# wustl-cig/FLAIR

Hardware: AMD Instinct MI355X
Metric: restored frames/sec at 256x256, 16-frame clip, 250-step DDIM (higher is better)
Workload: dtype bf16

## Files before the change

### flair_amd/csrc/api.hip

```cpp
#include <stdarg.h>
#include <stdio.h>

#include "common.h"

static thread_local char g_err[512] = "";

void flair_set_error(const char* fmt, ...) {
    va_list ap;
    va_start(ap, fmt);
    vsnprintf(g_err, sizeof(g_err), fmt, ap);
    va_end(ap);
}

extern "C" const char* flair_last_error(void) { return g_err; }
extern "C" int flair_abi_version(void) { return 11; }

#include <dlfcn.h>

typedef int (*flair_nccl_bcast_fn)(const void*, void*, size_t, int, int, void*, hipStream_t);

extern "C" int flair_bcast_weights(void* blob, size_t bytes, int root, void* rccl_comm, hipStream_t stream) {
    FLAIR_CHECK(blob && bytes > 0 && rccl_comm && root >= 0, "flair_bcast_weights: bad argument (blob, bytes, root, communicator)");
    static flair_nccl_bcast_fn fn = nullptr;
    if (!fn) {
        void* h = nullptr;
        for (const char* name : {"librccl.so", "librccl.so.1"}) {
            h = dlopen(name, RTLD_NOW | RTLD_NOLOAD);
            if (!h) h = dlopen(name, RTLD_NOW | RTLD_GLOBAL);
            if (h) break;
        }
        FLAIR_CHECK(h, "flair_bcast_weights: librccl.so not found (%s)", dlerror());
        fn = reinterpret_cast<flair_nccl_bcast_fn>(dlsym(h, "ncclBroadcast"));
        FLAIR_CHECK(fn, "flair_bcast_weights: ncclBroadcast not found in librccl");
    }
    const size_t chunk = (size_t)512 << 20;
    for (size_t off = 0; off < bytes; off += chunk) {
        const size_t n = bytes - off < chunk ? bytes - off : chunk;
        char* p = reinterpret_cast<char*>(blob) + off;
        const int rc = fn(p, p, n,  1, root, rccl_comm, stream);
        if (rc != 0) {
            flair_set_error("flair_bcast_weights: ncclBroadcast returned %d", rc);
            return FLAIR_ERR_HIP;
        }
    }
    return FLAIR_OK;
}

namespace {
typedef __attribute__((ext_vector_type(8))) __bf16 probe_bf16x8;
typedef __attribute__((ext_vector_type(16))) float probe_f32x16;

__global__ __launch_bounds__(256) void probe_matrix_kernel(float* sink, int iters) {
    probe_f32x16 acc[4];
    for (int i = 0; i < 4; ++i)
        for (int r = 0; r < 16; ++r) acc[i][r] = 0.f;
    probe_bf16x8 a, b;
    for (int e = 0; e < 8; ++e) {
        a[e] = (__bf16)(0.001f * (float)((threadIdx.x + e) & 255));
        b[e] = (__bf16)(0.002f * (float)((threadIdx.x + 2 * e) & 255));
    }
    for (int it = 0; it < iters; ++it) {
#pragma unroll
        for (int u = 0; u < 4; ++u)
#pragma unroll
            for (int i = 0; i < 4; ++i) acc[i] = __builtin_amdgcn_mfma_f32_32x32x16_bf16(a, b, acc[i], 0, 0, 0);
    }
    float s = 0.f;
    for (int i = 0; i < 4; ++i)
        for (int r = 0; r < 16; ++r) s += acc[i][r];
    if (s == 12345.678f) sink[0] = s;
}

__global__ __launch_bounds__(256) void probe_stream_kernel(const uint4* __restrict__ src, uint4* __restrict__ dst, size_t n, int mode) {
    unsigned sum = 0;
    for (size_t i = blockIdx.x * (size_t)blockDim.x + threadIdx.x; i < n; i += (size_t)gridDim.x * blockDim.x) {
        if (mode == 1) {
            dst[i] = make_uint4((unsigned)i, 1u, 2u, 3u);
        } else {
            const uint4 v = src[i];
            if (mode == 2) dst[i] = v;
            else sum ^= v.x ^ v.y ^ v.z ^ v.w;
        }
    }
    if (mode == 0 && sum == 0x12345679u) dst[0] = make_uint4(sum, 0u, 0u, 0u);
}
}

extern "C" int flair_probe_matrix_rate(int iters, int workgroups_per_cu, float* sink, double* flop_out, hipStream_t stream) {
    FLAIR_CHECK(iters > 0 && workgroups_per_cu >= 1 && workgroups_per_cu <= 8 && sink, "flair_probe_matrix_rate: bad argument");
    const int grid = flair_cu_count() * workgroups_per_cu;
    hipLaunchKernelGGL(probe_matrix_kernel, dim3(grid), dim3(256), 0, stream, sink, iters);
    FLAIR_LAUNCH_CHECK();
    if (flop_out) *flop_out = (double)grid * 4  * iters * 16  * (2.0 * 32 * 32 * 16);
    return FLAIR_OK;
}

extern "C" int flair_probe_stream_rate(const void* src, void* dst, size_t bytes, int mode, hipStream_t stream) {
    FLAIR_CHECK(dst && (mode == 1 || src) && bytes >= 16 && mode >= 0 && mode <= 2, "flair_probe_stream_rate: bad argument (mode 0 read, 1 write, 2 copy)");
    FLAIR_CHECK((reinterpret_cast<uintptr_t>(dst) & 15) == 0 && (reinterpret_cast<uintptr_t>(src) & 15) == 0, "flair_probe_stream_rate: 16-byte aligned buffers");
    hipLaunchKernelGGL(probe_stream_kernel, dim3(flair_cu_count() * 8), dim3(256), 0, stream, reinterpret_cast<const uint4*>(src),
                       reinterpret_cast<uint4*>(dst), bytes / 16, mode);
    FLAIR_LAUNCH_CHECK();
    return FLAIR_OK;
}
```

### flair_amd/csrc/conv.hip

```cpp
#include <type_traits>

#include "common.h"

namespace {

struct ConvArgs {
    const void* x[4];
    int segC[4];
    int segLd[4];
    int nseg;
    const void* w;
    const float* bias;
    const void* res0;
    const void* res1;
    int res0Ld, res1Ld;
    void* y;
    int yLd;
    int T, H, W;
    int KT, KH, KW;
    int Cout, CinTot;
    int act;
    float outScale;
    long P;
    int nPixTiles, nCoTiles;
    int tFast;
    unsigned segBytes[4];
    unsigned wBytes;
    float* part;
    int splitK;
    const float* fbias;
    int fbiasLd;
    int stride;
    int tapShift;
    int reflect;
    float actParam;
    int actPeriod;
    int Hin, Win;
    int esz;
};

template <typename E> struct Mma;

template <> struct Mma<bf16_t> {
    static constexpr int BKE = 32;
    static __device__ __forceinline__ int chunk(int i, int half) { return 2 * i + half; }
    static __device__ __forceinline__ void run(const uint4 (&a)[2], const uint4 (&b)[2], f32x16& acc) {
        acc = __builtin_amdgcn_mfma_f32_32x32x16_bf16(__builtin_bit_cast(bf16x8, a[0]),
                                                      __builtin_bit_cast(bf16x8, b[0]), acc, 0, 0, 0);
        acc = __builtin_amdgcn_mfma_f32_32x32x16_bf16(__builtin_bit_cast(bf16x8, a[1]),
                                                      __builtin_bit_cast(bf16x8, b[1]), acc, 0, 0, 0);
    }
    static __device__ __forceinline__ void run1(const uint4& a, const uint4& b, f32x16& acc) {
        acc = __builtin_amdgcn_mfma_f32_32x32x16_bf16(__builtin_bit_cast(bf16x8, a), __builtin_bit_cast(bf16x8, b),
                                                      acc, 0, 0, 0);
    }
    static constexpr int MFMA_PER_HALF = 1;
};

template <> struct Mma<float> {
    static constexpr int BKE = 16;
    static __device__ __forceinline__ int chunk(int i, int half) { return 2 * half + i; }
    static __device__ __forceinline__ void run(const uint4 (&a)[2], const uint4 (&b)[2], f32x16& acc) {
        const float* af = reinterpret_cast<const float*>(a);
        const float* bf = reinterpret_cast<const float*>(b);
#pragma unroll
        for (int s = 0; s < 8; ++s)
            acc = __builtin_amdgcn_mfma_f32_32x32x2f32(af[s], bf[s], acc, 0, 0, 0);
    }
    static __device__ __forceinline__ void run1(const uint4& a, const uint4& b, f32x16& acc) {
        const float* af = reinterpret_cast<const float*>(&a);
        const float* bf = reinterpret_cast<const float*>(&b);
#pragma unroll
        for (int s = 0; s < 4; ++s)
            acc = __builtin_amdgcn_mfma_f32_32x32x2f32(af[s], bf[s], acc, 0, 0, 0);
    }
    static constexpr int MFMA_PER_HALF = 4;
};

__device__ __forceinline__ int lds_off(int row, int chunk) {
    return row * 64 + ((chunk ^ ((row >> 2) & 3)) << 4);
}

__device__ __forceinline__ int staged_row(int id) {
    const int g = id >> 3;
    return (g >> 2) * 8 + (g & 3) + 4 * ((id >> 2) & 1);
}

template <typename E>
__device__ __forceinline__ void store_quad(const ConvArgs& a, long p, int co, float v0, float v1, float v2, float v3) {
    if (co >= a.Cout) return;
    float v[4] = {v0, v1, v2, v3};
    if (a.bias) {
        const float4 b = *reinterpret_cast<const float4*>(a.bias + co);
        v[0] += b.x; v[1] += b.y; v[2] += b.z; v[3] += b.w;
    }
    if (a.fbias) {
        const float* fb = a.fbias + (p / ((long)a.H * a.W)) * a.fbiasLd + co;
        v[0] += fb[0]; v[1] += fb[1]; v[2] += fb[2]; v[3] += fb[3];
    }
    if (a.act == FLAIR_ACT_DCN_OFFSETS) {
        dcn_offset_act<4>(v, co, a.actParam, a.actPeriod);
    } else {
#pragma unroll
        for (int e = 0; e < 4; ++e) v[e] = apply_act(v[e], a.act);
    }
    const E* r0 = reinterpret_cast<const E*>(a.res0);
    const E* r1 = reinterpret_cast<const E*>(a.res1);
    if (r0) {
#pragma unroll
        for (int e = 0; e < 4; ++e) v[e] += ET<E>::ld(r0 + p * a.res0Ld + co + e);
    }
    if (r1) {
#pragma unroll
        for (int e = 0; e < 4; ++e) v[e] += ET<E>::ld(r1 + p * a.res1Ld + co + e);
    }
#pragma unroll
    for (int e = 0; e < 4; ++e) v[e] *= a.outScale;
    E* dst = reinterpret_cast<E*>(a.y) + p * a.yLd + co;
    if constexpr (sizeof(E) == 4) {
        *reinterpret_cast<float4*>(dst) = make_float4(v[0], v[1], v[2], v[3]);
    } else {
        uint2 pk;
        pk.x = pack2bf(v[0], v[1]);
        pk.y = pack2bf(v[2], v[3]);
        *reinterpret_cast<uint2*>(dst) = pk;
    }
}

template <typename E, int ACT, int FC, int FP>
__device__ __forceinline__ void igemm_epilogue(const ConvArgs& a, const f32x16 (&acc)[FC][FP], long pbase, int cobase, int lr, int lh) {
    constexpr unsigned ESZ = sizeof(E);
    constexpr int VEC = ET<E>::VEC, NV = 8 / VEC;
    const float slope = a.act == FLAIR_ACT_NONE ? 1.f : a.act == FLAIR_ACT_RELU ? 0.f : a.act == FLAIR_ACT_LRELU01 ? 0.1f : 0.2f;
    const unsigned yLdB = (unsigned)a.yLd * ESZ, r0LdB = (unsigned)a.res0Ld * ESZ, r1LdB = (unsigned)a.res1Ld * ESZ;
    constexpr unsigned SPAN = FP * 32;
    const __amdgpu_buffer_rsrc_t yd = make_rsrc(reinterpret_cast<char*>(a.y) + ((size_t)pbase * a.yLd + cobase) * ESZ, SPAN * yLdB);
    const __amdgpu_buffer_rsrc_t r0d = make_rsrc(reinterpret_cast<const char*>(a.res0) + (a.res0 ? ((size_t)pbase * a.res0Ld + cobase) * ESZ : 0),
                                                 a.res0 ? SPAN * r0LdB : 0u);
    const __amdgpu_buffer_rsrc_t r1d = make_rsrc(reinterpret_cast<const char*>(a.res1) + (a.res1 ? ((size_t)pbase * a.res1Ld + cobase) * ESZ : 0),
                                                 a.res1 ? SPAN * r1LdB : 0u);
    const int coLeft = a.Cout - cobase;
    const __amdgpu_buffer_rsrc_t bd = make_rsrc(a.bias ? a.bias + cobase : nullptr, a.bias && coLeft > 0 ? (unsigned)coLeft * 4u : 0u);
    const long hw = (long)a.H * a.W;
#pragma unroll
    for (int j = 0; j < FP; ++j) {
        const long p = pbase + j * 32 + lr;
        const bool pvalid = p < a.P;
        const unsigned pl = (unsigned)(j * 32 + lr);
        const float* fbrow = a.fbias ? a.fbias + (pvalid ? p / hw : 0) * a.fbiasLd + cobase : nullptr;
#pragma unroll
        for (int i = 0; i < FC; ++i) {
            uint4 bq[2][2], r0v[2][NV], r1v[2][NV], fq[2][2];
#pragma unroll
            for (int jj = 0; jj < 2; ++jj) {
                const int cw = i * 32 + 16 * jj + 8 * lh;
                const bool ok = pvalid && cw < coLeft;
                bq[jj][0] = buf_load16(bd, 4u * (unsigned)cw);
                bq[jj][1] = buf_load16(bd, 4u * (unsigned)cw + 16u);
#pragma unroll
                for (int q = 0; q < NV; ++q) {
                    r0v[jj][q] = buf_load16(r0d, ok ? pl * r0LdB + (unsigned)(cw + q * VEC) * ESZ : FLAIR_OOB);
                    r1v[jj][q] = buf_load16(r1d, ok ? pl * r1LdB + (unsigned)(cw + q * VEC) * ESZ : FLAIR_OOB);
                }
                fq[jj][0] = fq[jj][1] = make_uint4(0u, 0u, 0u, 0u);
            }
            if (a.fbias) {
#pragma unroll
                for (int jj = 0; jj < 2; ++jj) {
                    const int cw = i * 32 + 16 * jj + 8 * lh;
                    const float* fp = fbrow + (cw < coLeft ? cw : 0);
                    fq[jj][0] = *reinterpret_cast<const uint4*>(fp);
                    fq[jj][1] = *reinterpret_cast<const uint4*>(fp + 4);
                }
            }
#pragma unroll
            for (int jj = 0; jj < 2; ++jj) {
                const f32x16& c = acc[i][j];
                float v[8];
#pragma unroll
                for (int e = 0; e < 4; ++e) {
                    const auto sw2 = __builtin_amdgcn_permlane32_swap(__float_as_uint(c[8 * jj + e]), __float_as_uint(c[8 * jj + 4 + e]), false, false);
                    v[e] = __uint_as_float(sw2[0]);
                    v[4 + e] = __uint_as_float(sw2[1]);
                }
                const int cw = i * 32 + 16 * jj + 8 * lh;
                const bool ok = pvalid && cw < coLeft;
                {
                    const uint4 b0 = bq[jj][0], b1 = bq[jj][1], f0 = fq[jj][0], f1 = fq[jj][1];
                    v[0] += __uint_as_float(b0.x) + __uint_as_float(f0.x); v[1] += __uint_as_float(b0.y) + __uint_as_float(f0.y);
                    v[2] += __uint_as_float(b0.z) + __uint_as_float(f0.z); v[3] += __uint_as_float(b0.w) + __uint_as_float(f0.w);
                    v[4] += __uint_as_float(b1.x) + __uint_as_float(f1.x); v[5] += __uint_as_float(b1.y) + __uint_as_float(f1.y);
                    v[6] += __uint_as_float(b1.z) + __uint_as_float(f1.z); v[7] += __uint_as_float(b1.w) + __uint_as_float(f1.w);
                }
                if constexpr (ACT == 0) {
#pragma unroll
                    for (int e = 0; e < 8; ++e) v[e] = fmaxf(v[e], v[e] * slope);
                } else if constexpr (ACT == 1) {
                    dcn_offset_act<8>(v, cobase + cw, a.actParam, a.actPeriod);
                } else if constexpr (ACT == 2) {
#pragma unroll
                    for (int e = 0; e < 8; ++e) v[e] = silu_f(v[e]);
                } else {
#pragma unroll
                    for (int e = 0; e < 8; ++e) v[e] = 0.5f * v[e] * (1.f + erff(v[e] * 0.70710678118654752f));
                }
#pragma unroll
                for (int q = 0; q < NV; ++q) {
                    float t[VEC];
                    Vec16<E>::load(reinterpret_cast<const E*>(&r0v[jj][q]), t);
#pragma unroll
                    for (int e = 0; e < VEC; ++e) v[q * VEC + e] += t[e];
                    Vec16<E>::load(reinterpret_cast<const E*>(&r1v[jj][q]), t);
#pragma unroll
                    for (int e = 0; e < VEC; ++e) v[q * VEC + e] += t[e];
                }
#pragma unroll
                for (int e = 0; e < 8; ++e) v[e] *= a.outScale;
#pragma unroll
                for (int q = 0; q < NV; ++q) {
                    alignas(16) E out[VEC];
                    Vec16<E>::store(out, v + q * VEC);
                    const uint4 ov = *reinterpret_cast<const uint4*>(out);
                    __builtin_amdgcn_raw_buffer_store_b128(u32x4_t{ov.x, ov.y, ov.z, ov.w}, yd,
                                                           (int)(ok ? pl * yLdB + (unsigned)(cw + q * VEC) * ESZ : FLAIR_OOB), 0, 0);
                }
            }
        }
    }
}

template <typename E, int TH, int RPW, int PF>
__global__ __launch_bounds__(64 * TH / RPW, (2 * 64 * TH / RPW + 255) / 256)
void conv3x3_halo_kernel(ConvArgs a) {
    prefetch_kernargs<sizeof(ConvArgs)>();
    constexpr int BKE = Mma<E>::BKE;
    constexpr int VEC = ET<E>::VEC;
    constexpr int NT = 64 * TH / RPW;
    constexpr int HW_ = 34;
// ... 387 lines not shown
        uint4 fa[2][CF], fb[2][RPW];
        auto load_tap = [&](int set, int tap9) {
            const int kh = tap9 / 3, kw = tap9 % 3;
#pragma unroll
            for (int i = 0; i < CF; ++i)
                fa[set][i] = *reinterpret_cast<const uint4*>(wb0 + (i * 32 * 9 + tap9) * PITCH);
#pragma unroll
            for (int j = 0; j < RPW; ++j)
                fb[set][j] = *reinterpret_cast<const uint4*>(hb + ((kh + j) * HW_ + kw) * PITCH);
        };
        load_tap(0, 0);
        __builtin_amdgcn_sched_group_barrier(0x100, CF + RPW, 0);
#pragma unroll
        for (int tap9 = 0; tap9 < 9; ++tap9) {
            const int set = tap9 & 1;
            if (tap9 < 8) load_tap(set ^ 1, tap9 + 1);
#pragma unroll
            for (int j = 0; j < RPW; ++j)
#pragma unroll
                for (int i = 0; i < CF; ++i) Mma<E>::run1(fa[set][i], fb[set][j], acc[j][i]);
            if (tap9 < 8) __builtin_amdgcn_sched_group_barrier(0x100, CF + RPW, 0);
            __builtin_amdgcn_sched_group_barrier(0x8, CF * RPW * Mma<E>::MFMA_PER_HALF, 0);
        }
    };

    issue();
    write_lds(0);
    if (nch > 1) issue();
    __syncthreads();
    for (int k = 0; k < nch; ++k) {
        compute(k & 1);
        if (k + 1 < nch) {
            write_lds((k + 1) & 1);
            if (k + 2 < nch) issue();
            __syncthreads();
        }
    }

    constexpr int FPITCH = 64 * 4 + 16;
    constexpr int CHUNKS = 64 / VEC;
    constexpr int PARTS = NW / TH;
    constexpr int NIT = 32 * CHUNKS / 64 / PARTS;
    const int orow = wave % TH, part = wave / TH;
    const int h = h0 + orow;
    const long prow = ((long)t * a.H + h) * a.W + w0;
    const int ech = lane % CHUNKS;
    const int eco = co0 + ech * VEC;
    const bool eok = h < a.H && eco < a.Cout;
    uint4 r0v[NIT], r1v[NIT];
#pragma unroll
    for (int k = 0; k < NIT; ++k) {
        const int px = ((k * PARTS + part) * 64 + lane) / CHUNKS;
        const long p = prow + px;
        r0v[k] = r1v[k] = make_uint4(0u, 0u, 0u, 0u);
        if (eok && a.res0) r0v[k] = *reinterpret_cast<const uint4*>(reinterpret_cast<const E*>(a.res0) + p * a.res0Ld + eco);
        if (eok && a.res1) r1v[k] = *reinterpret_cast<const uint4*>(reinterpret_cast<const E*>(a.res1) + p * a.res1Ld + eco);
    }
    __syncthreads();
#pragma unroll
    for (int pass = 0; pass < 2; ++pass) {
        if (kh2 == pass) {
#pragma unroll
            for (int j = 0; j < RPW; ++j) {
                char* tile = smem + (RPW * rp + j) * 32 * FPITCH + lr * FPITCH;
#pragma unroll
                for (int i = 0; i < CF; ++i)
#pragma unroll
                    for (int g = 0; g < 4; ++g) {
                        float4* dst = reinterpret_cast<float4*>(tile + ((cg * CF + i) * 32 + 8 * g + 4 * lh) * 4);
                        float4 v = make_float4(acc[j][i][4 * g], acc[j][i][4 * g + 1], acc[j][i][4 * g + 2],
                                               acc[j][i][4 * g + 3]);
                        if (pass == 1) {
                            const float4 o = *dst;
                            v.x += o.x; v.y += o.y; v.z += o.z; v.w += o.w;
                        }
                        *dst = v;
                    }
            }
        }
        __syncthreads();
    }
    if (!eok) return;
    const float slope = a.act == FLAIR_ACT_NONE ? 1.f : a.act == FLAIR_ACT_RELU ? 0.f : a.act == FLAIR_ACT_LRELU01 ? 0.1f : 0.2f;
    const bool leaky = a.act == FLAIR_ACT_NONE || a.act == FLAIR_ACT_RELU || a.act == FLAIR_ACT_LRELU01 || a.act == FLAIR_ACT_LRELU02;
    const char* tile = smem + orow * 32 * FPITCH;
#pragma unroll
    for (int k = 0; k < NIT; ++k) {
        const int px = ((k * PARTS + part) * 64 + lane) / CHUNKS;
        const long p = prow + px;
        float v[VEC];
        const float* src = reinterpret_cast<const float*>(tile + px * FPITCH) + ech * VEC;
#pragma unroll
        for (int e = 0; e < VEC; e += 4) {
            const float4 q = *reinterpret_cast<const float4*>(src + e);
            v[e] = q.x; v[e + 1] = q.y; v[e + 2] = q.z; v[e + 3] = q.w;
        }
#pragma unroll
        for (int e = 0; e < VEC; ++e) v[e] += biasv[e];
        if (a.fbias) {
            const float* fb = a.fbias + (long)t * a.fbiasLd + eco;
#pragma unroll
            for (int e = 0; e < VEC; ++e) v[e] += fb[e];
        }
        if (leaky) {
#pragma unroll
            for (int e = 0; e < VEC; ++e) v[e] = fmaxf(v[e], v[e] * slope);
        } else if (a.act == FLAIR_ACT_DCN_OFFSETS) {
            dcn_offset_act<VEC>(v, eco, a.actParam, a.actPeriod);
        } else if (a.act == FLAIR_ACT_SILU) {
#pragma unroll
            for (int e = 0; e < VEC; ++e) v[e] = silu_f(v[e]);
        } else {
#pragma unroll
            for (int e = 0; e < VEC; ++e) v[e] = apply_act(v[e], a.act);
        }
        if (a.res0) {
            float r[VEC];
            Vec16<E>::load(reinterpret_cast<const E*>(&r0v[k]), r);
#pragma unroll
            for (int e = 0; e < VEC; ++e) v[e] += r[e];
        }
        if (a.res1) {
            float r[VEC];
            Vec16<E>::load(reinterpret_cast<const E*>(&r1v[k]), r);
#pragma unroll
            for (int e = 0; e < VEC; ++e) v[e] += r[e];
        }
#pragma unroll
        for (int e = 0; e < VEC; ++e) v[e] *= a.outScale;
        Vec16<E>::store(reinterpret_cast<E*>(a.y) + p * a.yLd + eco, v);
    }
}

template <typename E, int TH, int RPW, int CF>
int launch_halo_ks(const ConvArgs& a0, hipStream_t s) {
    ConvArgs a = a0;
    a.nCoTiles = cdiv(a.Cout, 64);
    const int grid = a.T * cdiv(a.H, TH) * (a.W / 32) * a.nCoTiles;
    const size_t lds = 2 * ((size_t)(TH + 2) * 34 * 80 + 64 * 9 * 80);
    static LdsAttrOnce attr;
    {
        const hipError_t e = flair_max_lds_once(attr, reinterpret_cast<const void*>(&conv3x3_halo_ks_kernel<E, TH, RPW, CF>));
        FLAIR_CHECK(e == hipSuccess, "flair_conv_nhwc: hipFuncSetAttribute: %s", hipGetErrorString(e));
    }
    hipLaunchKernelGGL((conv3x3_halo_ks_kernel<E, TH, RPW, CF>), dim3(grid), dim3(256 * TH / RPW / CF), lds, s, a);
    FLAIR_LAUNCH_CHECK();
    return FLAIR_OK;
}

struct DmaTile {
    int t, h0, w0, co0;
};

template <int NW, int RPW, int NSTAGE>
__device__ __forceinline__ void conv3x3_dma_body(const ConvArgs& a, int nTiles, int tilesPerXcd) {
    using E = bf16_t;
    static_assert((RPW == 1 || RPW == 2) && NSTAGE == 2, "the clip-level and one-tile forms (two stages)");
    constexpr int KSTEPS = 2;
    constexpr int TH = NW * RPW, HWP = 34;
    constexpr int HALO_ROWS = (TH + 2) * HWP;
    constexpr int HALO_INSTR = (HALO_ROWS + 15) / 16;
    constexpr int W_INSTR = 64 * 9 / 16;
    constexpr int HALO_BYTES = HALO_INSTR * 1024;
    constexpr int STAGE_BYTES = HALO_BYTES + W_INSTR * 1024;
    constexpr int NSLOT = (HALO_INSTR + W_INSTR + NW - 1) / NW;
    constexpr int BIAS_OFF = NSTAGE * STAGE_BYTES + NW * 1024;
    extern __shared__ __attribute__((aligned(16))) char smem[];

    const int tid = threadIdx.x, lane = tid & 63;
    const int wave = __builtin_amdgcn_readfirstlane(tid >> 6);
    const int lr = lane & 31, lh = lane >> 5;
    const int taps = a.KT * 9, pt = a.KT / 2;
    const int chunksPerTap = a.CinTot / 32;
    const int H = a.H, W = a.W, T = a.T;

    const int xcd = blockIdx.x & 7, slot = blockIdx.x >> 3, slotsPerXcd = gridDim.x >> 3;
    const int tilesW = W / 32, tilesH = H / TH, nCoTiles = a.nCoTiles;
    auto tile_at = [&](int i, DmaTile& tl) -> bool {
        const int inXcd = slot + i * slotsPerXcd;
        const int id = xcd * tilesPerXcd + inXcd;
        if (inXcd >= tilesPerXcd || id >= nTiles) return false;
        int rest = id;
        tl.co0 = (rest % nCoTiles) * 64;
        rest /= nCoTiles;
        if (a.tFast) {
            tl.t = rest % T;
            rest /= T;
            tl.w0 = (rest % tilesW) * 32;
            tl.h0 = (rest / tilesW) * TH;
            return true;
        }
        tl.w0 = (rest % tilesW) * 32;
        rest /= tilesW;
        tl.h0 = (rest % tilesH) * TH;
        tl.t = rest / tilesH;
        return true;
    };

    const int lrow = lane >> 2, lchunk = lane & 3;
    unsigned slotv[NSLOT], hchunk[NSLOT];
#pragma unroll
    for (int i = 0; i < NSLOT; ++i) {
        const int id = wave * NSLOT + i;
        const int c = (id * 16 + lrow) % HWP;
        hchunk[i] = (unsigned)((lchunk ^ ((c >> 2) & 3)) << 4);
    }
    auto setup_tile = [&](const DmaTile& tl) {
#pragma unroll
        for (int i = 0; i < NSLOT; ++i) {
            const int id = wave * NSLOT + i;
            const int R = id * 16 + lrow;
            const int hr = R / HWP, c = R - hr * HWP;
            const int hh = tl.h0 - 1 + hr, ww = tl.w0 - 1 + c;
            const bool okh = R < HALO_ROWS && (unsigned)hh < (unsigned)H && (unsigned)ww < (unsigned)W;
            const unsigned hv = okh ? (unsigned)(hh * W + ww) : 0xffffffffu;
            const int row = R - HALO_INSTR * 16;
            const int tap9 = row >> 6, co = row & 63;
            const bool okw = row >= 0 && row < 576 && tl.co0 + co < a.Cout;
            const unsigned wv = okw ? (unsigned)(((tl.co0 + co) * taps + tap9) * a.CinTot) * 2u + ((lchunk ^ ((co >> 2) & 3)) << 4) : FLAIR_OOB;
            slotv[i] = id >= HALO_INSTR ? wv : hv;
        }
    };

    const u32x4_t wdesc = make_desc(a.w, a.wBytes);
    struct Walk {
        int dt, seg, cb, segOff, j;
    };
    auto dt_at = [&](int t, int j) { return a.tFast ? (j + a.KT * T - t) % a.KT - pt : j - pt; };
    auto walk_first = [&](int t, Walk& wk) {
        wk.j = 0; wk.seg = 0; wk.cb = 0; wk.segOff = 0;
        while (wk.j < a.KT && (unsigned)(t + dt_at(t, wk.j)) >= (unsigned)T) ++wk.j;
        wk.dt = dt_at(t, wk.j);
    };
    auto walk_next = [&](int t, Walk& wk) {
        ++wk.cb;
        if (wk.cb * 32 >= a.segC[wk.seg]) {
            wk.cb = 0;
            wk.segOff += a.segC[wk.seg];
            if (++wk.seg >= a.nseg) {
                wk.seg = 0;
                wk.segOff = 0;
                ++wk.j;
                while (wk.j < a.KT && (unsigned)(t + dt_at(t, wk.j)) >= (unsigned)T) ++wk.j;
                wk.dt = dt_at(t, wk.j);
            }
        }
    };
    auto chunks_of = [&](int t) {
        int n = 0;
        for (int d = -pt; d <= pt; ++d) n += (unsigned)(t + d) < (unsigned)T ? 1 : 0;
        return n * chunksPerTap;
    };
    auto issue = [&](const DmaTile& tl, const Walk& wk, int stage) {
        const unsigned ld = (unsigned)a.segLd[wk.seg] * 2u;
        const char* frame = reinterpret_cast<const char*>(a.x[wk.seg]) + (size_t)(tl.t + wk.dt) * H * W * ld;
        const u32x4_t xdesc = make_desc(frame, a.segBytes[wk.seg]);
        const unsigned cofs = (unsigned)(wk.cb * 64);
        const unsigned kofs = (unsigned)((wk.dt + pt) * 9 * a.CinTot + wk.segOff + wk.cb * 32) * 2u;
        const unsigned sbase = (unsigned)(stage * STAGE_BYTES + wave * NSLOT * 1024);
#pragma unroll
        for (int i = 0; i < NSLOT; ++i) {
            const bool isw = wave * NSLOT + i >= HALO_INSTR;
            const unsigned sv = slotv[i];
            const unsigned offh = sv == 0xffffffffu ? FLAIR_OOB : sv * ld + cofs + hchunk[i];
            const unsigned offw = sv == FLAIR_OOB ? FLAIR_OOB : sv + kofs;
            u32x4_t d;
            d.x = isw ? wdesc.x : xdesc.x;
            d.y = isw ? wdesc.y : xdesc.y;
            d.z = isw ? wdesc.z : xdesc.z;
            d.w = 0x00020000u;
            const bool idle = wave * NSLOT + i >= HALO_INSTR + W_INSTR;
            dma16(d, isw ? offw : offh, idle ? (unsigned)(NSTAGE * STAGE_BYTES + ((wave * NSLOT + i - HALO_INSTR - W_INSTR) % NW) * 1024) : sbase + i * 1024);
        }
    };

    unsigned aoff[KSTEPS], boff[3][KSTEPS];
#pragma unroll
    for (int s_ = 0; s_ < KSTEPS; ++s_) {
        aoff[s_] = (unsigned)(HALO_BYTES + lr * 64 + (((2 * s_ + lh) ^ ((lr >> 2) & 3)) << 4));
#pragma unroll
        for (int kw = 0; kw < 3; ++kw)
            boff[kw][s_] = (unsigned)((RPW * wave * HWP + kw + lr) * 64 + (((2 * s_ + lh) ^ (((kw + lr) >> 2) & 3)) << 4));
    }

    f32x16 acc[RPW][2];
    auto zero_acc = [&]() {
#pragma unroll
        for (int j = 0; j < RPW; ++j)
#pragma unroll
            for (int i = 0; i < 2; ++i)
#pragma unroll
                for (int r = 0; r < 16; ++r) acc[j][i][r] = 0.f;
    };
    auto compute = [&](int stage) {
        const char* sb = smem + stage * STAGE_BYTES;
        uint4 fb[2][RPW + 2][KSTEPS];
        uint4 fa[2][2][KSTEPS];
        auto load_b = [&](int set, int kw) {
#pragma unroll
            for (int h = 0; h < RPW + 2; ++h)
#pragma unroll
                for (int s_ = 0; s_ < KSTEPS; ++s_)
                    fb[set][h][s_] = *reinterpret_cast<const uint4*>(sb + h * (HWP * 64) + boff[kw][s_]);
        };
        auto load_a = [&](int set, int kh, int kw) {
#pragma unroll
            for (int cf = 0; cf < 2; ++cf)
#pragma unroll
                for (int s_ = 0; s_ < KSTEPS; ++s_)
                    fa[set][cf][s_] = *reinterpret_cast<const uint4*>(sb + (kh * 3 + kw) * 4096 + cf * 2048 + aoff[s_]);
        };
        load_b(0, 0);
        load_a(0, 0, 0);
        __builtin_amdgcn_sched_group_barrier(0x100, KSTEPS * (RPW + 2) + 2 * KSTEPS, 0);
#pragma unroll
        for (int step = 0; step < 9; ++step) {
            const int kq = step / 3, kh = step % 3;
            const int nkq = (step + 1) / 3, nkh = (step + 1) % 3;
            if (step < 8) {
                if (nkh == 0) load_b(nkq & 1, nkq);
                load_a((step + 1) & 1, nkh, nkq);
            }
#pragma unroll
            for (int j = 0; j < RPW; ++j)
#pragma unroll
                for (int cf = 0; cf < 2; ++cf) Mma<E>::run(fa[step & 1][cf], fb[kq & 1][j + kh], acc[j][cf]);
            if (step < 8) {
                if (nkh == 0) __builtin_amdgcn_sched_group_barrier(0x100, KSTEPS * (RPW + 2) + 2 * KSTEPS, 0);
                else __builtin_amdgcn_sched_group_barrier(0x100, 2 * KSTEPS, 0);
            }
            __builtin_amdgcn_sched_group_barrier(0x8, 2 * KSTEPS * RPW, 0);
        }
    };
    auto epilogue_as = [&](const DmaTile& tl, int biasSlot, auto actTag, auto resTag) {
        constexpr int ACT = decltype(actTag)::value;
        constexpr bool HASRES = decltype(resTag)::value;
        const float slope = a.act == FLAIR_ACT_NONE ? 1.f : a.act == FLAIR_ACT_RELU ? 0.f : a.act == FLAIR_ACT_LRELU01 ? 0.1f : 0.2f;
        const long p0w = ((long)tl.t * H + tl.h0 + RPW * wave) * W + tl.w0;
        const int cl = 8 * lh;
        const unsigned yLdB = (unsigned)a.yLd * 2u, rLdB = (unsigned)a.res0Ld * 2u;
        const unsigned span = (unsigned)(RPW * W);
        const __amdgpu_buffer_rsrc_t yd = make_rsrc(reinterpret_cast<char*>(a.y) + (p0w * a.yLd + tl.co0) * 2, span * yLdB);
        const __amdgpu_buffer_rsrc_t r0d = make_rsrc(reinterpret_cast<const char*>(a.res0) + (a.res0 ? (p0w * a.res0Ld + tl.co0) * 2 : 0),
                                                     a.res0 ? span * rLdB : 0u);
        const E* r1b = a.res1 ? reinterpret_cast<const E*>(a.res1) + (p0w + lr) * a.res1Ld + tl.co0 + cl : nullptr;
        const float* bl = reinterpret_cast<const float*>(smem + BIAS_OFF + (biasSlot & 1) * 256) + cl;
        const float scale = a.outScale;
        const unsigned yLane = (unsigned)lr * yLdB + 2u * cl, rLane = (unsigned)lr * rLdB + 2u * cl;
        uint4 r0v[2][2][RPW];
        auto res_request = [&](int i) {
#pragma unroll
            for (int jj = 0; jj < 2; ++jj) {
                const int cofs = i * 32 + 16 * jj;
                const bool lane_ok = tl.co0 + cofs + cl < a.Cout;
#pragma unroll
                for (int j = 0; j < RPW; ++j)
                    r0v[i][jj][j] = buf_load16(r0d, lane_ok ? rLane + (unsigned)(j * W) * rLdB + 2u * cofs : FLAIR_OOB);
            }
        };
        if constexpr (HASRES) {
            res_request(0);
            res_request(1);
        }
#pragma unroll
        for (int i = 0; i < 2; ++i) {
#pragma unroll
            for (int jj = 0; jj < 2; ++jj) {
                const int cofs = i * 32 + 16 * jj;
                const bool lane_ok = tl.co0 + cofs + cl < a.Cout;
                float bv[8];
                {
                    const float4 b0 = *reinterpret_cast<const float4*>(bl + cofs);
                    const float4 b1 = *reinterpret_cast<const float4*>(bl + cofs + 4);
                    bv[0] = b0.x; bv[1] = b0.y; bv[2] = b0.z; bv[3] = b0.w; bv[4] = b1.x; bv[5] = b1.y; bv[6] = b1.z; bv[7] = b1.w;
                }
#pragma unroll
                for (int j = 0; j < RPW; ++j) {
                    float v[8];
#pragma unroll
                    for (int e = 0; e < 4; ++e) {
                        const auto sw2 = __builtin_amdgcn_permlane32_swap(__float_as_uint(acc[j][i][8 * jj + e]),
                                                                          __float_as_uint(acc[j][i][8 * jj + 4 + e]), false, false);
                        v[e] = __uint_as_float(sw2[0]) + bv[e];
                        v[4 + e] = __uint_as_float(sw2[1]) + bv[4 + e];
                    }
                    if constexpr (ACT == 0) {
#pragma unroll
                        for (int e = 0; e < 8; ++e) v[e] = fmaxf(v[e], v[e] * slope);
                    } else if constexpr (ACT == 1) {
                        dcn_offset_act_fast<8>(v, tl.co0 + cofs + cl, a.actParam, a.actPeriod, 1.f);
                    } else if constexpr (ACT == 2) {
#pragma unroll
                        for (int e = 0; e < 8; ++e) v[e] *= __builtin_amdgcn_rcpf(1.f + __expf(-v[e]));
                    }
                    if constexpr (HASRES) {
                        float r[8];
                        Vec16<E>::load(reinterpret_cast<const E*>(&r0v[i][jj][j]), r);
#pragma unroll
                        for (int e = 0; e < 8; ++e) v[e] += r[e];
                        if (r1b && lane_ok) {
                            Vec16<E>::load(r1b + (long)j * W * a.res1Ld + cofs, r);
#pragma unroll
                            for (int e = 0; e < 8; ++e) v[e] += r[e];
                        }
                    }
                    if constexpr (ACT != 3) {
#pragma unroll
                        for (int e = 0; e < 8; ++e) v[e] *= scale;
                    }
                    alignas(16) E out[8];
                    Vec16<E>::store(out, v);
                    const uint4 ov = *reinterpret_cast<const uint4*>(out);
                    const unsigned yo = lane_ok ? yLane + (unsigned)(j * W) * yLdB + 2u * cofs : FLAIR_OOB;
                    __builtin_amdgcn_raw_buffer_store_b128(u32x4_t{ov.x, ov.y, ov.z, ov.w}, yd, (int)yo, 0, 0);
                }
            }
        }
    };
    auto epilogue_plain_as = [&](const DmaTile& tl, int biasSlot, auto actTag) {
        constexpr int ACT = decltype(actTag)::value;
        const float slope = a.act == FLAIR_ACT_NONE ? 1.f : a.act == FLAIR_ACT_RELU ? 0.f : a.act == FLAIR_ACT_LRELU01 ? 0.1f : 0.2f;
        const long p0 = ((long)tl.t * H + tl.h0 + RPW * wave) * W + tl.w0 + lr;
        const int cl = 8 * lh;
        E* yb = reinterpret_cast<E*>(a.y) + p0 * a.yLd + tl.co0 + cl;
        const E* r0b = a.res0 ? reinterpret_cast<const E*>(a.res0) + p0 * a.res0Ld + tl.co0 + cl : nullptr;
        const E* r1b = a.res1 ? reinterpret_cast<const E*>(a.res1) + p0 * a.res1Ld + tl.co0 + cl : nullptr;
        const float* bl = reinterpret_cast<const float*>(smem + BIAS_OFF + (biasSlot & 1) * 256) + cl;
        const float scale = a.outScale;
#pragma unroll
        for (int i = 0; i < 2; ++i)
#pragma unroll
            for (int jj = 0; jj < 2; ++jj) {
                const int cofs = i * 32 + 16 * jj;
                if (tl.co0 + cofs >= a.Cout) continue;
                const bool lane_ok = tl.co0 + cofs + cl < a.Cout;
                float bv[8];
                {
                    const float4 b0 = *reinterpret_cast<const float4*>(bl + cofs);
                    const float4 b1 = *reinterpret_cast<const float4*>(bl + cofs + 4);
                    bv[0] = b0.x; bv[1] = b0.y; bv[2] = b0.z; bv[3] = b0.w; bv[4] = b1.x; bv[5] = b1.y; bv[6] = b1.z; bv[7] = b1.w;
                }
#pragma unroll
                for (int j = 0; j < RPW; ++j) {
                    float v[8];
#pragma unroll
                    for (int e = 0; e < 4; ++e) {
                        const auto sw2 = __builtin_amdgcn_permlane32_swap(__float_as_uint(acc[j][i][8 * jj + e]),
                                                                          __float_as_uint(acc[j][i][8 * jj + 4 + e]), false, false);
                        v[e] = __uint_as_float(sw2[0]) + bv[e];
                        v[4 + e] = __uint_as_float(sw2[1]) + bv[4 + e];
                    }
                    if constexpr (ACT == 0) {
#pragma unroll
                        for (int e = 0; e < 8; ++e) v[e] = fmaxf(v[e], v[e] * slope);
                    } else if constexpr (ACT == 1) {
                        dcn_offset_act<8>(v, tl.co0 + cofs + cl, a.actParam, a.actPeriod);
                    } else {
#pragma unroll
                        for (int e = 0; e < 8; ++e) v[e] = silu_f(v[e]);
                    }
                    const long ro = (long)j * W;
                    if (r0b && lane_ok) {
                        float r[8];
                        Vec16<E>::load(r0b + ro * a.res0Ld + cofs, r);
#pragma unroll
                        for (int e = 0; e < 8; ++e) v[e] += r[e];
                    }
                    if (r1b && lane_ok) {
                        float r[8];
                        Vec16<E>::load(r1b + ro * a.res1Ld + cofs, r);
#pragma unroll
                        for (int e = 0; e < 8; ++e) v[e] += r[e];
                    }
#pragma unroll
                    for (int e = 0; e < 8; ++e) v[e] *= scale;
                    if (!lane_ok) continue;
                    Vec16<E>::store(yb + ro * a.yLd + cofs, v);
                }
            }
    };
    auto epilogue = [&](const DmaTile& tl, int biasSlot) {
        const bool res = a.res0 || a.res1;
        auto go = [&](auto actTag) {
            if constexpr (RPW == 1) {
                epilogue_plain_as(tl, biasSlot, actTag);
            } else {
                if (res) epilogue_as(tl, biasSlot, actTag, std::true_type{});
                else epilogue_as(tl, biasSlot, actTag, std::false_type{});
            }
        };
        if (a.act == FLAIR_ACT_DCN_OFFSETS) go(std::integral_constant<int, 1>{});
        else if (a.act == FLAIR_ACT_SILU) go(std::integral_constant<int, 2>{});
        else if (RPW >= 2 && a.act == FLAIR_ACT_NONE && a.outScale == 1.f) go(std::integral_constant<int, 3>{});
        else go(std::integral_constant<int, 0>{});
    };

    DmaTile cur, nxt;
    int iCur = 0, iNxt = 0;
    if (!tile_at(0, cur)) return;
    nxt = cur;
    Walk wk;
    walk_first(nxt.t, wk);
    setup_tile(nxt);
    float4 biasReg = make_float4(0.f, 0.f, 0.f, 0.f);
    bool biasPending = false;
    auto bias_request = [&](const DmaTile& tl) {
        if (tid < 16) {
            const int bco = tl.co0 + 4 * tid;
            biasReg = (a.bias && bco < a.Cout) ? *reinterpret_cast<const float4*>(a.bias + bco) : make_float4(0.f, 0.f, 0.f, 0.f);
            if (a.fbias && bco < a.Cout) {
                const float* fb = a.fbias + (long)tl.t * a.fbiasLd + bco;
                biasReg.x += fb[0]; biasReg.y += fb[1]; biasReg.z += fb[2]; biasReg.w += fb[3];
            }
        }
        biasPending = true;
    };
    auto bias_commit = [&](int slot_) {
        if (tid < 16) *reinterpret_cast<float4*>(smem + BIAS_OFF + (slot_ & 1) * 256 + 16 * tid) = biasReg;
        biasPending = false;
    };
    bias_request(nxt);
    bias_commit(0);
    const bool res0any = a.res0 || a.res1;
    int remIssue = chunks_of(nxt.t);
    int remCompute = remIssue;
    bool more = true;
    int stage = 0;
    issue(nxt, wk, 0);
    walk_next(nxt.t, wk);
    --remIssue;
    asm volatile("s_waitcnt vmcnt(0)" ::: "memory");
    __syncthreads();
    zero_acc();
    while (true) {
        if (more && remIssue == 0) {
            ++iNxt;
            more = tile_at(iNxt, nxt);
            if (more) {
                walk_first(nxt.t, wk);
                setup_tile(nxt);
                remIssue = chunks_of(nxt.t);
                bias_request(nxt);
            }
        }
        if (more) {
            issue(nxt, wk, stage ^ 1);
            walk_next(nxt.t, wk);
            --remIssue;
        }
        compute(stage);
        if (biasPending) bias_commit(iNxt);
        bool storesInFlight = false;
        if (--remCompute == 0) {
            epilogue(cur, iCur);
            storesInFlight = RPW >= 2 ? !a.res1 : cur.co0 + 64 <= a.Cout && !res0any;
            ++iCur;
            if (!tile_at(iCur, cur)) break;
            remCompute = chunks_of(cur.t);
            zero_acc();
        }
        if (storesInFlight) {
            asm volatile("s_waitcnt vmcnt(%0)" ::"n"(4 * RPW) : "memory");
        } else {
            asm volatile("s_waitcnt vmcnt(0)" ::: "memory");
        }
        __syncthreads();
        stage ^= 1;
    }
}

template <int NW, int RPW, int NSTAGE>
__global__ __launch_bounds__(64 * NW, (NW + 3) / 4) void conv3x3_dma_kernel(ConvArgs a, int nTiles, int tilesPerXcd) {
    prefetch_kernargs<sizeof(ConvArgs) + 8>();
    conv3x3_dma_body<NW, RPW, NSTAGE>(a, nTiles, tilesPerXcd);
}

template <int NW, int RPW, int NSTAGE>
int launch_dma(const ConvArgs& a0, hipStream_t s) {
    constexpr int TH = NW * RPW;
    ConvArgs a = a0;
    a.nCoTiles = cdiv(a.Cout, 64);
    a.tFast = a.KT == 3 && a.T > 1;
    const int nTiles = a.T * (a.H / TH) * (a.W / 32) * a.nCoTiles;
    const int nCu = flair_cu_count();
    int grid = nTiles < nCu ? (nTiles + 7) / 8 * 8 : nCu / 8 * 8;
    if (grid < 8) grid = 8;
    const int tilesPerXcd = (nTiles + 7) / 8;
    constexpr int HALO_INSTR = ((TH + 2) * 34 + 15) / 16;
    const size_t lds = NSTAGE * (size_t)(HALO_INSTR + 36) * 1024 + NW * 1024 + 512;
    static LdsAttrOnce attr;
    {
        const hipError_t e = flair_max_lds_once(attr, reinterpret_cast<const void*>(&conv3x3_dma_kernel<NW, RPW, NSTAGE>));
        FLAIR_CHECK(e == hipSuccess, "flair_conv_nhwc: hipFuncSetAttribute: %s", hipGetErrorString(e));
    }
    hipLaunchKernelGGL((conv3x3_dma_kernel<NW, RPW, NSTAGE>), dim3(grid), dim3(64 * NW), lds, s, a, nTiles, tilesPerXcd);

    FLAIR_LAUNCH_CHECK();
    return FLAIR_OK;
}


template <bool HALO3>
__global__ __launch_bounds__(512, 2) void conv_frame_kernel(ConvArgs a) {
    static_assert(HALO3, "halo ring of three, weight ring of two");
    prefetch_kernargs<sizeof(ConvArgs)>();
    using E = bf16_t;
    constexpr int NW = 8, HWP = 34;
    constexpr int HINSTR = 22, HIMG = HINSTR * 1024, WINSTR = 36, SLOT = WINSTR * 1024;
    constexpr int HR = 3, WR = 2;
    constexpr int RING = HR * HIMG, BIAS = RING + WR * SLOT;
    constexpr int NH = (HINSTR + NW - 1) / NW, NWS = (WINSTR + NW - 1) / NW;
    extern __shared__ __attribute__((aligned(16))) char smem[];
    const int tid = threadIdx.x, lane = tid & 63;
    const int wave = __builtin_amdgcn_readfirstlane(tid >> 6);
    const int lr = lane & 31, lh = lane >> 5;
    const int lrow = lane >> 2, lchunk = lane & 3;
    const int tilesW = a.W / 32, perFrame = tilesW * (a.H / 8);
    const int bid = xcd_remap(blockIdx.x, gridDim.x);
    const int t = bid / perFrame, tile = bid - t * perFrame;
    const int h0 = (tile / tilesW) * 8, w0 = (tile % tilesW) * 32;
    const int nS = a.CinTot / 32;

    const u32x4_t wdesc = make_desc(a.w, a.wBytes);
    const u32x4_t bdesc = make_desc(a.bias, a.bias ? (unsigned)a.Cout * 4u : 0u);
    dma16(bdesc, (unsigned)(lane * 16), (unsigned)BIAS);
    unsigned hpix[NH], hpiece[NH];
#pragma unroll
    for (int i = 0; i < NH; ++i) {
        const int k = (wave * NH + i) % HINSTR;
        const int R = k * 16 + lrow;
        const int hr = R / HWP, c = R - hr * HWP;
        const int hh = h0 - 1 + hr, ww = w0 - 1 + c;
        const bool ok = R < 10 * HWP && (unsigned)hh < (unsigned)a.H && (unsigned)ww < (unsigned)a.W;
        hpix[i] = ok ? (unsigned)(hh * a.W + ww) : 0xffffffffu;
        hpiece[i] = (unsigned)((lchunk ^ ((c >> 2) & 3)) << 4);
    }
    unsigned wlane[NWS];
#pragma unroll
    for (int i = 0; i < NWS; ++i) {
        const int id = (wave * NWS + i) % WINSTR;
        const int row = id * 16 + lrow, tap9 = row >> 6, co = row & 63;
        wlane[i] = co < a.Cout ? (unsigned)((co * 9 + tap9) * a.CinTot) * 2u + (unsigned)((lchunk ^ ((co >> 2) & 3)) << 4) : FLAIR_OOB;
    }
    int hseg = 0, hcb = 0;
    auto issue_halo = [&](int slot) {
        const unsigned ld = (unsigned)a.segLd[hseg] * 2u;
        const u32x4_t xdesc = make_desc(reinterpret_cast<const char*>(a.x[hseg]) + (size_t)t * a.H * a.W * ld, a.segBytes[hseg]);
        const unsigned cofs = (unsigned)(hcb * 64);
#pragma unroll
        for (int i = 0; i < NH; ++i) {
            const int k = (wave * NH + i) % HINSTR;
            dma16(xdesc, hpix[i] == 0xffffffffu ? FLAIR_OOB : hpix[i] * ld + cofs + hpiece[i], (unsigned)(slot * HIMG + k * 1024));
        }
        if (++hcb * 32 >= a.segC[hseg]) {
            hcb = 0;
            ++hseg;
        }
    };
    auto issue_w = [&](int s_) {
#pragma unroll
        for (int i = 0; i < NWS; ++i) {
            const int id = (wave * NWS + i) % WINSTR;
            dma16(wdesc, wlane[i] == FLAIR_OOB ? FLAIR_OOB : wlane[i] + (unsigned)(s_ * 64), (unsigned)(RING + (s_ % WR) * SLOT + id * 1024));
        }
    };
    issue_halo(0);
    issue_w(0);
    if (nS > 1) {
        issue_halo(1);
        issue_w(1);
    }
    if (nS > 2) issue_halo(2);

    unsigned aoff[2], boff[3][2];
#pragma unroll
    for (int ks = 0; ks < 2; ++ks) {
        aoff[ks] = (unsigned)(lr * 64 + (((2 * ks + lh) ^ ((lr >> 2) & 3)) << 4));
#pragma unroll
        for (int kw = 0; kw < 3; ++kw)
            boff[kw][ks] = (unsigned)((wave * HWP + kw + lr) * 64 + (((2 * ks + lh) ^ (((kw + lr) >> 2) & 3)) << 4));
    }
    f32x16 acc[2];
    auto compute = [&](int wslot, int hslot) {
        const char* wb = smem + RING + wslot * SLOT;
        const char* xb = smem + hslot * HIMG;
        uint4 fb[2][3][2], fa[2][2][2];
        auto load_b = [&](int set, int kw) {
#pragma unroll
            for (int h = 0; h < 3; ++h)
#pragma unroll
                for (int ks = 0; ks < 2; ++ks) fb[set][h][ks] = *reinterpret_cast<const uint4*>(xb + h * (HWP * 64) + boff[kw][ks]);
        };
        auto load_a = [&](int set, int kh, int kw) {
#pragma unroll
            for (int cf = 0; cf < 2; ++cf)
#pragma unroll
                for (int ks = 0; ks < 2; ++ks) fa[set][cf][ks] = *reinterpret_cast<const uint4*>(wb + (kh * 3 + kw) * 4096 + cf * 2048 + aoff[ks]);
        };
        load_b(0, 0);
        load_a(0, 0, 0);
#pragma unroll
        for (int step = 0; step < 9; ++step) {
            const int kq = step / 3, kh = step % 3;
            const int nkq = (step + 1) / 3, nkh = (step + 1) % 3;
            if (step < 8) {
                if (nkh == 0) load_b(nkq & 1, nkq);
                load_a((step + 1) & 1, nkh, nkq);
            }
#pragma unroll
            for (int cf = 0; cf < 2; ++cf)
#pragma unroll
                for (int ks = 0; ks < 2; ++ks)
                    acc[cf] = __builtin_amdgcn_mfma_f32_32x32x16_bf16(__builtin_bit_cast(bf16x8, fa[step & 1][cf][ks]), __builtin_bit_cast(bf16x8, fb[kq & 1][kh][ks]), acc[cf], 0, 0, 0);
        }
    };

    const long prow = ((long)t * a.H + h0 + wave) * a.W + w0;
    const unsigned yLdB = (unsigned)a.yLd * 2u, r0LdB = (unsigned)a.res0Ld * 2u, r1LdB = (unsigned)a.res1Ld * 2u;
    const __amdgpu_buffer_rsrc_t yd = make_rsrc(reinterpret_cast<char*>(a.y) + prow * a.yLd * 2, (unsigned)a.W * yLdB);
    const __amdgpu_buffer_rsrc_t r0d = make_rsrc(a.res0 ? reinterpret_cast<const char*>(a.res0) + prow * a.res0Ld * 2 : nullptr, a.res0 ? (unsigned)a.W * r0LdB : 0u);
    const __amdgpu_buffer_rsrc_t r1d = make_rsrc(a.res1 ? reinterpret_cast<const char*>(a.res1) + prow * a.res1Ld * 2 : nullptr, a.res1 ? (unsigned)a.W * r1LdB : 0u);
    uint4 r0v[4], r1v[4];
#pragma unroll
    for (int g = 0; g < 4; ++g) r0v[g] = r1v[g] = make_uint4(0u, 0u, 0u, 0u);

    for (int s_ = 0; s_ < nS; ++s_) {
        if (s_ + 1 >= nS) asm volatile("s_waitcnt vmcnt(0)" ::: "memory");
        else if (s_ == 0 && nS > 2) asm volatile("s_waitcnt vmcnt(%0)" ::"n"(2 * NH + NWS) : "memory");
        else if (s_ == 0) asm volatile("s_waitcnt vmcnt(%0)" ::"n"(NH + NWS) : "memory");
        else asm volatile("s_waitcnt vmcnt(%0)" ::"n"(NH) : "memory");
        __builtin_amdgcn_s_barrier();
        if (s_ == 0) {
            const float* sb = reinterpret_cast<const float*>(smem + BIAS);
#pragma unroll
            for (int cf = 0; cf < 2; ++cf)
#pragma unroll
                for (int g = 0; g < 4; ++g) {
                    const float4 bq = *reinterpret_cast<const float4*>(sb + cf * 32 + 8 * g + 4 * lh);
                    acc[cf][4 * g] = bq.x; acc[cf][4 * g + 1] = bq.y; acc[cf][4 * g + 2] = bq.z; acc[cf][4 * g + 3] = bq.w;
                }
        }
        if (s_ >= 1 && s_ + 1 < nS) issue_w(s_ + 1);
        if (s_ >= 1 && s_ + 2 < nS) issue_halo((s_ + 2) % 3);
        if (s_ + 1 == nS) {
            if (a.res0) {
#pragma unroll
                for (int g = 0; g < 4; ++g) r0v[g] = buf_load16(r0d, 16 * g + 8 * lh < a.Cout ? (unsigned)lr * r0LdB + (unsigned)(32 * g + 16 * lh) : FLAIR_OOB);
            }
// ... 231 lines not shown
                for (int i = 0; i < FC; ++i)
#pragma unroll
                    for (int j = 0; j < FP; ++j) Mma<E>::run(af[i], bfr[j], acc[i][j]);
            }
            if (k + 1 < nk) write_lds(cur ^ 1, (u + 1) % PD);
            __syncthreads();
        }
    }

    if (a.splitK > 1) {
#pragma unroll
        for (int j = 0; j < FP; ++j) {
            const long p = p0 + wp * (TP / WP) + j * 32 + lr;
            if (p >= a.P) continue;
#pragma unroll
            for (int i = 0; i < FC; ++i)
#pragma unroll
                for (int g = 0; g < 4; ++g) {
                    const int co = co0 + wc * (TC / WC) + i * 32 + 8 * g + 4 * lh;
                    if (co < a.Cout)
                        *reinterpret_cast<float4*>(a.part + ((long)blockIdx.y * a.P + p) * a.Cout + co) =
                            make_float4(acc[i][j][4 * g], acc[i][j][4 * g + 1], acc[i][j][4 * g + 2],
                                        acc[i][j][4 * g + 3]);
                }
        }
        return;
    }
    if ((a.Cout & 7) == 0 && ((uintptr_t)a.y & 15) == 0 && (a.yLd * (int)sizeof(E)) % 16 == 0 &&
        (!a.res0 || (((uintptr_t)a.res0 & 15) == 0 && (a.res0Ld * (int)sizeof(E)) % 16 == 0)) &&
        (!a.res1 || (((uintptr_t)a.res1 & 15) == 0 && (a.res1Ld * (int)sizeof(E)) % 16 == 0))) {
        auto run = [&](auto actTag) {
            igemm_epilogue<E, decltype(actTag)::value, FC, FP>(a, acc, p0 + wp * (TP / WP), co0 + wc * (TC / WC), lr, lh);
        };
        if (a.act == FLAIR_ACT_DCN_OFFSETS) run(std::integral_constant<int, 1>{});
        else if (a.act == FLAIR_ACT_SILU) run(std::integral_constant<int, 2>{});
        else if (a.act == FLAIR_ACT_GELU) run(std::integral_constant<int, 3>{});
        else run(std::integral_constant<int, 0>{});
        return;
    }
#pragma unroll
    for (int j = 0; j < FP; ++j) {
        const long p = p0 + wp * (TP / WP) + j * 32 + lr;
        if (p >= a.P) continue;
#pragma unroll
        for (int i = 0; i < FC; ++i)
#pragma unroll
            for (int g = 0; g < 4; ++g)
                store_quad<E>(a, p, co0 + wc * (TC / WC) + i * 32 + 8 * g + 4 * lh, acc[i][j][4 * g],
                              acc[i][j][4 * g + 1], acc[i][j][4 * g + 2], acc[i][j][4 * g + 3]);
    }
}

template <typename E>
__global__ void conv_splitk_reduce_kernel(ConvArgs a) {
    const unsigned cq = (unsigned)(a.Cout / 4);
    const unsigned quads = (unsigned)a.P * cq;
    const size_t slice = (size_t)a.P * a.Cout;
    for (unsigned i = blockIdx.x * blockDim.x + threadIdx.x; i < quads; i += gridDim.x * blockDim.x) {
        const unsigned p = i / cq;
        const int co = (int)(i - p * cq) * 4;
        const float* src = a.part + (size_t)p * a.Cout + co;
        float4 s = make_float4(0.f, 0.f, 0.f, 0.f);
        int k = 0;
        for (; k + 4 <= a.splitK; k += 4) {
            float4 v[4];
#pragma unroll
            for (int u = 0; u < 4; ++u) v[u] = *reinterpret_cast<const float4*>(src + (size_t)(k + u) * slice);
#pragma unroll
            for (int u = 0; u < 4; ++u) {
                s.x += v[u].x; s.y += v[u].y; s.z += v[u].z; s.w += v[u].w;
            }
        }
        for (; k < a.splitK; ++k) {
            const float4 v = *reinterpret_cast<const float4*>(src + (size_t)k * slice);
            s.x += v.x; s.y += v.y; s.z += v.z; s.w += v.w;
        }
        store_quad<E>(a, p, co, s.x, s.y, s.z, s.w);
    }
}

template <typename E, int TC, int TP, int WC, int WP, int PD, int KWID>
int launch_pd(const ConvArgs& a0, hipStream_t s) {
    ConvArgs a = a0;
    a.nPixTiles = cdiv(a.P, TP);
    a.nCoTiles = cdiv(a.Cout, TC);
    const int grid = a.nPixTiles * a.nCoTiles;
    const size_t lds = 2 * (TC + TP) * 64 * KWID;
    hipLaunchKernelGGL((conv_igemm_kernel<E, TC, TP, WC, WP, PD, KWID>), dim3(grid, a.splitK), dim3(256), lds, s, a);
    FLAIR_LAUNCH_CHECK();
    if (a.splitK > 1) {
        long g = (a.P * (a.Cout / 4) + 255) / 256;
        if (g > 2048) g = 2048;
        hipLaunchKernelGGL(conv_splitk_reduce_kernel<E>, dim3((int)g), dim3(256), 0, s, a);
        FLAIR_LAUNCH_CHECK();
    }
    return FLAIR_OK;
}

template <typename E, int TC, int TP, int WC, int WP>
int launch(const ConvArgs& a, hipStream_t s) {
    if constexpr (sizeof(E) == 2) {
        bool ok = true;
        for (int i = 0; i < a.nseg; ++i) ok = ok && a.segC[i] % 64 == 0;
        if (ok) return launch_pd<E, TC, TP, WC, WP, 2, 2>(a, s);
    }
    return launch_pd<E, TC, TP, WC, WP, 4, 1>(a, s);
}

int choose_split(const ConvArgs& a, int variant) {
    if (variant > 2) return 1;
    const int maxBlocks = variant == 0 ? 512 : 1024, maxSplit = 16;
    const int tc = variant == 0 ? 128 : 64, tp = variant == 2 ? 64 : 128;
    const int bke = 64 / (a.wBytes && a.CinTot ? (int)(a.wBytes / ((unsigned long long)a.Cout * a.KT * a.KH * a.KW * a.CinTot)) : 2);
    const long nk = (long)a.KT * a.KH * a.KW * (a.CinTot / bke);
    const long tiles = (long)cdiv(a.P, tp) * cdiv(a.Cout, tc);
    if (tiles >= 384 || nk < 32) return 1;
    long s = maxBlocks / tiles;
    if (s > maxSplit) s = maxSplit;
    if (s > nk / 8) s = nk / 8;
    return s < 1 ? 1 : (int)s;
}

int choose_variant(const ConvArgs& a) {
    if (!a.reflect && a.stride == 1 && a.KH == 3 && a.KW == 3 && a.W % 32 == 0 && a.H >= 2) {
        const long per = (long)a.T * (a.W / 32) * cdiv(a.Cout, 64);
        const bool ks = a.Cout % 8 == 0;
        if (a.esz == 2 && ks && a.act != FLAIR_ACT_GELU && a.H % 16 == 0 && per * cdiv(a.H, 8) > 256 && per * (a.H / 16) >= 192) return 8;
        const bool dmaOk = a.esz == 2 && ks && a.act != FLAIR_ACT_GELU;
        if (per * cdiv(a.H, 8) >= 256) return ks && per * cdiv(a.H, 8) <= 256 ? (dmaOk && a.H % 8 == 0 ? 9 : 6) : 3;
        if (per * cdiv(a.H, 4) >= 256) return ks && per * cdiv(a.H, 4) <= 256 ? 7 : 4;
        return 5;
    }
    const long tiles128 = (long)cdiv(a.P, 128) * cdiv(a.Cout, 128);
    if (a.Cout > 64 && tiles128 >= 512) return 0;
    if (a.Cout >= 128 && a.P >= 1024 && tiles128 <= 64 && (long)a.KT * a.KH * a.KW * a.CinTot >= 2304) return 0;
    const long tiles64x128 = (long)cdiv(a.P, 128) * cdiv(a.Cout, 64);
    if (tiles64x128 >= 512) return 1;
    return 2;
}

template <typename E>
int dispatch(const ConvArgs& a0, hipStream_t s) {
    ConvArgs a = a0;
    const int variant = choose_variant(a);
    a.splitK = a.part ? choose_split(a, variant) : 1;
    switch (variant) {
        case 0: return launch<E, 128, 128, 2, 2>(a, s);
        case 1: return launch<E, 64, 128, 1, 4>(a, s);
        case 2: return launch<E, 64, 64, 2, 2>(a, s);
        case 3: return launch_halo<E, 8, 1, 1>(a, s);
        case 4: return launch_halo<E, 4, 1, 1>(a, s);
        case 6: return launch_halo_ks<E, 8, 1, 2>(a, s);
        case 7: return launch_halo_ks<E, 4, 1, 2>(a, s);
        case 8: return launch_dma<8, 2, 2>(a, s);
        case 9:
            if (frame_kernel_ok(a)) return launch_frame(a, s);
            return launch_dma<8, 1, 2>(a, s);
        default: return launch_halo<E, 2, 1, 1>(a, s);
    }
}

}

extern "C" int flair_conv_variant(const flair_conv_params* p);

static void fill_geometry(ConvArgs& a, const flair_conv_params* p) {
    a.stride = p->stride > 1 ? p->stride : 1;
    a.Hin = p->H; a.Win = p->W;
    a.T = p->T; a.KT = p->KT; a.KH = p->KH; a.KW = p->KW; a.Cout = p->Cout;
    a.reflect = p->reflect_pad ? 1 : 0;
    a.act = p->act;
    a.H = (p->H + a.stride - 1) / a.stride;
    a.W = (p->W + a.stride - 1) / a.stride;
    a.P = (long)p->T * a.H * a.W;
    a.CinTot = 0;
    for (int i = 0; i < p->nseg && i < 4; ++i) a.CinTot += p->seg_c[i];
    const int esz = p->dtype == FLAIR_BF16 ? 2 : 4;
    a.esz = esz;
    a.wBytes = (unsigned)((unsigned long long)p->Cout * p->KT * p->KH * p->KW * a.CinTot * esz);
}

extern "C" size_t flair_conv_workspace_bytes(const flair_conv_params* p) {
    if (!p) return 0;
    ConvArgs a{};
    fill_geometry(a, p);
    const int split = choose_split(a, choose_variant(a));
    return split > 1 ? (size_t)split * a.P * a.Cout * sizeof(float) : 0;
}

extern "C" int flair_conv_nhwc(const flair_conv_params* p, const void* const* x, const void* w,
                               const float* bias, const float* frame_bias, const void* res0, const void* res1,
                               void* y, void* workspace, size_t workspace_bytes, hipStream_t stream) {
    FLAIR_CHECK(p && x && w && y, "flair_conv_nhwc: null argument");
    FLAIR_CHECK(p->dtype == FLAIR_F32 || p->dtype == FLAIR_BF16, "flair_conv_nhwc: bad dtype %d", p->dtype);
    FLAIR_CHECK(p->nseg >= 1 && p->nseg <= 4, "flair_conv_nhwc: nseg %d not in 1..4", p->nseg);
    FLAIR_CHECK(p->T > 0 && p->H > 0 && p->W > 0 && p->Cout > 0, "flair_conv_nhwc: empty shape");
    FLAIR_CHECK((p->KT & 1) && (p->KH & 1) && (p->KW & 1), "flair_conv_nhwc: kernel taps must be odd");
    FLAIR_CHECK(p->Cout % 4 == 0, "flair_conv_nhwc: Cout %d must be a multiple of 4", p->Cout);
    const int bke = p->dtype == FLAIR_BF16 ? 32 : 16;
    const int esz = p->dtype == FLAIR_BF16 ? 2 : 4;
    ConvArgs a{};
    a.CinTot = 0;
    for (int i = 0; i < p->nseg; ++i) {
        FLAIR_CHECK(x[i], "flair_conv_nhwc: segment %d is null", i);
        FLAIR_CHECK(p->seg_c[i] > 0 && p->seg_c[i] % bke == 0,
                    "flair_conv_nhwc: segment %d has %d channels; must be a multiple of %d", i, p->seg_c[i], bke);
        FLAIR_CHECK(p->seg_ld[i] >= p->seg_c[i] && (p->seg_ld[i] * esz) % 16 == 0 &&
                        ((uintptr_t)x[i]) % 16 == 0,
                    "flair_conv_nhwc: segment %d stride/alignment", i);
        a.x[i] = x[i];
        a.segC[i] = p->seg_c[i];
        a.segLd[i] = p->seg_ld[i];
        a.CinTot += p->seg_c[i];
        const unsigned long long bytes = (unsigned long long)p->H * p->W * p->seg_ld[i] * esz;
        FLAIR_CHECK(bytes < 0x40000000ull, "flair_conv_nhwc: one frame of segment %d spans %llu bytes (limit 1 GiB)",
                    i, bytes);
        a.segBytes[i] = (unsigned)bytes;
    }
    {
        const unsigned long long wb = (unsigned long long)p->Cout * p->KT * p->KH * p->KW * a.CinTot * esz;
        FLAIR_CHECK(wb < 0x80000000ull, "flair_conv_nhwc: weights span %llu bytes (limit 2 GiB)", wb);
        a.wBytes = (unsigned)wb;
    }
    const int gran = (p->dtype == FLAIR_BF16 && p->Cout % 8 != 0) ? 8 : 16;
    FLAIR_CHECK(p->y_ld >= p->Cout && (p->y_ld * esz) % gran == 0 && ((uintptr_t)y) % 16 == 0,
                "flair_conv_nhwc: output stride/alignment (y_ld = %d: >= Cout = %d, a multiple of %d bytes; y 16-byte aligned)",
                p->y_ld, p->Cout, gran);
    FLAIR_CHECK(!res0 || (p->res_ld[0] >= p->Cout && (p->res_ld[0] * esz) % gran == 0 && ((uintptr_t)res0) % gran == 0),
                "flair_conv_nhwc: res0 stride/alignment (res_ld = %d: >= Cout = %d; stride and pointer multiples of %d bytes)",
                p->res_ld[0], p->Cout, gran);
    FLAIR_CHECK(!res1 || (p->res_ld[1] >= p->Cout && (p->res_ld[1] * esz) % gran == 0 && ((uintptr_t)res1) % gran == 0),
                "flair_conv_nhwc: res1 stride/alignment (res_ld = %d: >= Cout = %d; stride and pointer multiples of %d bytes)",
                p->res_ld[1], p->Cout, gran);
    FLAIR_CHECK(((uintptr_t)w) % 16 == 0, "flair_conv_nhwc: weight alignment");
    FLAIR_CHECK(!bias || ((uintptr_t)bias) % 16 == 0, "flair_conv_nhwc: bias alignment");
    a.nseg = p->nseg;
    a.w = w;
    a.bias = bias;
    a.fbias = frame_bias;
    a.fbiasLd = p->frame_bias_ld;
    FLAIR_CHECK(!frame_bias || p->frame_bias_ld >= p->Cout, "flair_conv_nhwc: frame_bias_ld");
    {
        const unsigned long long hw = (unsigned long long)p->H * p->W * esz;
        FLAIR_CHECK(hw * p->y_ld < 0x40000000ull && (!res0 || hw * p->res_ld[0] < 0x40000000ull) && (!res1 || hw * p->res_ld[1] < 0x40000000ull),
                    "flair_conv_nhwc: one frame of the output / a residual spans more than 1 GiB");
    }
    a.res0 = res0;
    a.res1 = res1;
    a.res0Ld = p->res_ld[0];
    a.res1Ld = p->res_ld[1];
    a.y = y;
    a.yLd = p->y_ld;
    a.act = p->act;
    a.actParam = p->act_param;
    a.actPeriod = p->act_period;
    FLAIR_CHECK(p->act != FLAIR_ACT_DCN_OFFSETS || (p->act_period > 0 && p->act_period % 24 == 0),
                "flair_conv_nhwc: FLAIR_ACT_DCN_OFFSETS needs act_period = 3 * deform_groups (multiple of 24), got %d",
                p->act_period);
    a.outScale = p->out_scale;
    {
        ConvArgs g{};
        fill_geometry(g, p);
        a.stride = g.stride; a.Hin = g.Hin; a.Win = g.Win; a.T = g.T; a.H = g.H; a.W = g.W; a.P = g.P;
        a.KT = g.KT; a.KH = g.KH; a.KW = g.KW; a.Cout = g.Cout; a.esz = g.esz;
    }
    FLAIR_CHECK(a.stride == 1 || a.stride == 2, "flair_conv_nhwc: stride %d unsupported", p->stride);
    FLAIR_CHECK(!p->asym_pad || (a.stride == 2 && a.KH == a.KW && a.KT == 1 && p->H % 2 == 0 && p->W % 2 == 0),
                "flair_conv_nhwc: asym_pad needs a square 2-D stride-2 kernel on even frames");
    a.tapShift = p->asym_pad ? a.KH / 2 : 0;
    FLAIR_CHECK(!p->reflect_pad || (!p->asym_pad && a.KT == 1 && p->H > a.KH / 2 && p->W > a.KW / 2),
                "flair_conv_nhwc: reflect_pad needs a 2-D kernel smaller than the frame");
    a.reflect = p->reflect_pad ? 1 : 0;
    a.part = nullptr;
    a.splitK = 1;

    if (workspace && workspace_bytes >= flair_conv_workspace_bytes(p) && flair_conv_workspace_bytes(p) > 0) {
        FLAIR_CHECK(((uintptr_t)workspace) % 16 == 0, "flair_conv_nhwc: workspace alignment");
        a.part = reinterpret_cast<float*>(workspace);
    }
    if (p->dtype == FLAIR_BF16) return dispatch<bf16_t>(a, stream);
    return dispatch<float>(a, stream);
}

extern "C" int flair_conv_variant(const flair_conv_params* p) {
    if (!p) return -1;
    ConvArgs a{};
    fill_geometry(a, p);
    return choose_variant(a);
}
```

### flair_amd/csrc/gn.hip

```cpp

#include <type_traits>

#include "common.h"

namespace {

struct GnSrc {
    const void* x[2];
    int c[2];
    int ld[2];
};

template <typename E>
__global__ void gn_partial_kernel(GnSrc s, int C, int groups, long pixPerStat, int blocksPerStat, float* part) {
    prefetch_kernargs<sizeof(GnSrc) + 32>();
    constexpr int VEC = ET<E>::VEC;
    extern __shared__ float red[];
    const int cv = C / VEC;
    const int rows = blockDim.x / cv;
    const int slot = threadIdx.x % cv, r = threadIdx.x / cv;
    const int stat = blockIdx.x / blocksPerStat, blk = blockIdx.x % blocksPerStat;
    const long per = (pixPerStat + blocksPerStat - 1) / blocksPerStat;
    const long beg = stat * pixPerStat + (long)blk * per;
    long end = beg + per;
    const long lim = (stat + 1) * pixPerStat;
    if (end > lim) end = lim;

    int c0 = slot * VEC;
    const E* base;
    int ld;
    if (c0 < s.c[0]) {
        base = reinterpret_cast<const E*>(s.x[0]) + c0;
        ld = s.ld[0];
    } else {
        base = reinterpret_cast<const E*>(s.x[1]) + (c0 - s.c[0]);
        ld = s.ld[1];
    }
    float sum[VEC], sq[VEC];
#pragma unroll
    for (int i = 0; i < VEC; ++i) sum[i] = sq[i] = 0.f;
#pragma unroll 4
    for (long p = beg + r; p < end; p += rows) {
        float v[VEC];
        Vec16<E>::load(base + p * ld, v);
#pragma unroll
        for (int i = 0; i < VEC; ++i) {
            sum[i] += v[i];
            sq[i] = fmaf(v[i], v[i], sq[i]);
        }
    }
    float* rs = red;
    float* rq = red + rows * C;
#pragma unroll
    for (int i = 0; i < VEC; ++i) {
        rs[r * C + c0 + i] = sum[i];
        rq[r * C + c0 + i] = sq[i];
    }
    __syncthreads();
    for (int c = threadIdx.x; c < C; c += blockDim.x) {
        float a = 0.f, b = 0.f;
        for (int k = 0; k < rows; ++k) {
            a += rs[k * C + c];
            b += rq[k * C + c];
        }
        rs[c] = a;
        rq[c] = b;
    }
    __syncthreads();
    const int cpg = C / groups;
    for (int g = threadIdx.x; g < groups; g += blockDim.x) {
        float a = 0.f, b = 0.f;
        for (int k = 0; k < cpg; ++k) {
            a += rs[g * cpg + k];
            b += rq[g * cpg + k];
        }
        part[((long)blockIdx.x * 2 + 0) * groups + g] = a;
        part[((long)blockIdx.x * 2 + 1) * groups + g] = b;
    }
}

__global__ void gn_finalize_kernel(const float* part, int groups, int cpg, int blocksPerStat, long pixPerStat,
                                   float eps, float* stats) {
    const int lane = threadIdx.x & 63;
    const int sg = blockIdx.x * (blockDim.x >> 6) + (threadIdx.x >> 6);
    const int stat = sg / groups, g = sg % groups;
    const float* pp = part + ((long)stat * blocksPerStat * 2) * groups + g;
    const long st = 2L * groups;
    double a = 0.0, b = 0.0;
    int i = lane;
    for (; i + 192 < blocksPerStat; i += 256) {
        const float a0 = pp[i * st], b0 = pp[i * st + groups];
        const float a1 = pp[(i + 64) * st], b1 = pp[(i + 64) * st + groups];
        const float a2 = pp[(i + 128) * st], b2 = pp[(i + 128) * st + groups];
        const float a3 = pp[(i + 192) * st], b3 = pp[(i + 192) * st + groups];
        a += ((double)a0 + (double)a1) + ((double)a2 + (double)a3);
        b += ((double)b0 + (double)b1) + ((double)b2 + (double)b3);
    }
    for (; i < blocksPerStat; i += 64) {
        a += (double)pp[i * st];
        b += (double)pp[i * st + groups];
    }
#pragma unroll
    for (int off = 32; off > 0; off >>= 1) {
        a += __shfl_xor(a, off);
        b += __shfl_xor(b, off);
    }
    if (lane == 0) {
        const double cnt = (double)pixPerStat * cpg;
        const double mean = a / cnt;
        double var = b / cnt - mean * mean;
        if (var < 0) var = 0;
        stats[sg * 2 + 0] = (float)mean;
        stats[sg * 2 + 1] = (float)(1.0 / sqrt(var + (double)eps));
    }
}

struct GnApply {
    GnSrc s;
    int C, groups;
    int F, H, W;
    int framesPerStat;
    const float* stats;
    const float* gamma;
    const float* beta;
    const float* film;
    int filmLd;
    int act;
    int resample;
    void* y;  int yLd;
    void* raw; int rawLd;
    int blocksPerFrame;
    int filmVec;
};

template <typename E>
__global__ __launch_bounds__(512) void gn_apply_kernel(GnApply a) {
    prefetch_kernargs<sizeof(GnApply)>();
    constexpr int VEC = ET<E>::VEC;
    const int cv = a.C / VEC;
    const int rows = blockDim.x / cv;
    const int slot = threadIdx.x % cv, r = threadIdx.x / cv;
    const int f = blockIdx.x / a.blocksPerFrame, blk = blockIdx.x % a.blocksPerFrame;
    const int c0 = slot * VEC;
    const E* base;
    int ld;
    if (c0 < a.s.c[0]) {
        base = reinterpret_cast<const E*>(a.s.x[0]) + c0;
        ld = a.s.ld[0];
    } else {
        base = reinterpret_cast<const E*>(a.s.x[1]) + (c0 - a.s.c[0]);
        ld = a.s.ld[1];
    }
    float A[VEC], B[VEC];
    const int cpg = a.C / a.groups;
    const int stat = f / a.framesPerStat;
    {
        float2 st[VEC];
        float gm[VEC], bt[VEC], sc[VEC], sh[VEC];
#pragma unroll
        for (int i = 0; i < VEC; ++i) {
            const int c = c0 + i;
            st[i] = *reinterpret_cast<const float2*>(a.stats + (stat * a.groups + c / cpg) * 2);
            gm[i] = a.gamma[c];
            bt[i] = a.beta[c];
            sc[i] = 0.f;
            sh[i] = 0.f;
        }
        if (a.film) {
#pragma unroll
            for (int i = 0; i < VEC; ++i) {
                sc[i] = a.film[(long)f * a.filmLd + c0 + i];
                sh[i] = a.film[(long)f * a.filmLd + a.C + c0 + i];
            }
        }
#pragma unroll
        for (int i = 0; i < VEC; ++i) {
            float ga = gm[i] * st[i].y;
            float be = bt[i] - st[i].x * ga;
            if (a.film) {
                const float m = 1.f + sc[i];
                ga *= m;
                be = be * m + sh[i];
            }
            A[i] = ga;
            B[i] = be;
        }
    }
    auto run = [&](auto actTag) {
        constexpr int ACTC = decltype(actTag)::value;
        auto act1 = [&](float x) -> float {
            if constexpr (ACTC == 0) return x;
            else if constexpr (ACTC == 1) {
                if constexpr (sizeof(E) == 2) return x * __builtin_amdgcn_rcpf(1.f + __expf(-x));
                else return silu_f(x);
            } else return apply_act(x, a.act);
        };
        E* y = reinterpret_cast<E*>(a.y);
        E* raw = reinterpret_cast<E*>(a.raw);
        const long fin = (long)f * a.H * a.W;
        if (a.resample == 0) {
            const long n = (long)a.H * a.W;
            const long per = (n + a.blocksPerFrame - 1) / a.blocksPerFrame;
            long end = (blk + 1) * per;
            if (end > n) end = n;
            long p = blk * per + r;
            for (; p + 3 * rows < end; p += 4 * rows) {
                uint4 raw4[4];
    #pragma unroll
                for (int u = 0; u < 4; ++u)
                    raw4[u] = *reinterpret_cast<const uint4*>(base + (fin + p + (long)u * rows) * ld);
    #pragma unroll
                for (int u = 0; u < 4; ++u) {
                    float v[VEC];
                    Vec16<E>::load(reinterpret_cast<const E*>(&raw4[u]), v);
    #pragma unroll
                    for (int i = 0; i < VEC; ++i) v[i] = act1(fmaf(v[i], A[i], B[i]));
                    Vec16<E>::store(y + (fin + p + (long)u * rows) * a.yLd + c0, v);
                }
            }
            for (; p < end; p += rows) {
                float v[VEC];
                Vec16<E>::load(base + (fin + p) * ld, v);
    #pragma unroll
                for (int i = 0; i < VEC; ++i) v[i] = act1(fmaf(v[i], A[i], B[i]));
                Vec16<E>::store(y + (fin + p) * a.yLd + c0, v);
            }
        } else if (a.resample == 1) {
            const int Ho = a.H / 2, Wo = a.W / 2;
            const long n = (long)Ho * Wo;
            const long per = (n + a.blocksPerFrame - 1) / a.blocksPerFrame;
            long end = (blk + 1) * per;
            if (end > n) end = n;
            const long fout = (long)f * n;
            for (long p = blk * per + r; p < end; p += rows) {
                const int ho = (int)(p / Wo), wo = (int)(p % Wo);
                float accv[VEC], accr[VEC];
    #pragma unroll
                for (int i = 0; i < VEC; ++i) accv[i] = accr[i] = 0.f;
    #pragma unroll
                for (int q = 0; q < 4; ++q) {
                    const long pi = fin + (long)(2 * ho + (q >> 1)) * a.W + 2 * wo + (q & 1);
                    float v[VEC];
                    Vec16<E>::load(base + pi * ld, v);
    #pragma unroll
                    for (int i = 0; i < VEC; ++i) {
                        accr[i] += v[i];
                        accv[i] += act1(fmaf(v[i], A[i], B[i]));
                    }
                }
    #pragma unroll
                for (int i = 0; i < VEC; ++i) {
                    accv[i] *= 0.25f;
                    accr[i] *= 0.25f;
                }
                Vec16<E>::store(y + (fout + p) * a.yLd + c0, accv);
                if (raw) Vec16<E>::store(raw + (fout + p) * a.rawLd + c0, accr);
            }
        } else {
            const long n = (long)a.H * a.W;
            const long per = (n + a.blocksPerFrame - 1) / a.blocksPerFrame;
            long end = (blk + 1) * per;
            if (end > n) end = n;
            const int Wo = a.W * 2;
            const long fout = (long)f * n * 4;
            for (long p = blk * per + r; p < end; p += rows) {
                const int h = (int)(p / a.W), w = (int)(p % a.W);
// ... 35 lines not shown
    const E* base = reinterpret_cast<const E*>(seg1 ? a.s.x[1] : a.s.x[0]) + (seg1 ? c0 - a.s.c[0] : c0);
    const int ld = seg1 ? a.s.ld[1] : a.s.ld[0];
    uint4* cache = reinterpret_cast<uint4*>(gsm);
    float ga[VEC], be[VEC];
#pragma unroll
    for (int e = 0; e < VEC; e += 4) {
        *reinterpret_cast<float4*>(&ga[e]) = *reinterpret_cast<const float4*>(a.gamma + c0 + e);
        *reinterpret_cast<float4*>(&be[e]) = *reinterpret_cast<const float4*>(a.beta + c0 + e);
    }

    float sum = 0.f, sq = 0.f;
    auto accumulate = [&](const uint4& raw) {
        float v[VEC];
        Vec16<E>::load(reinterpret_cast<const E*>(&raw), v);
#pragma unroll
        for (int e = 0; e < VEC; ++e) {
            sum += v[e];
            sq = fmaf(v[e], v[e], sq);
        }
    };
    long q = threadIdx.x / pp;
    for (; q + (U - 1) * rows < pixPerStat; q += U * rows) {
        uint4 raw[U];
#pragma unroll
        for (int u = 0; u < U; ++u) raw[u] = *reinterpret_cast<const uint4*>(base + (pix0 + q + (long)u * rows) * ld);
#pragma unroll
        for (int u = 0; u < U; ++u) {
            cache[(q + (long)u * rows) * pp + k] = raw[u];
            accumulate(raw[u]);
        }
    }
    for (; q < pixPerStat; q += rows) {
        const uint4 raw = *reinterpret_cast<const uint4*>(base + (pix0 + q) * ld);
        cache[q * pp + k] = raw;
        accumulate(raw);
    }
    double ds = (double)sum, dq = (double)sq;
#pragma unroll
    for (int off = 32; off > 0; off >>= 1) {
        ds += __shfl_xor(ds, off);
        dq += __shfl_xor(dq, off);
    }
    if ((threadIdx.x & 63) == 0) {
        redS[threadIdx.x >> 6] = ds;
        redQ[threadIdx.x >> 6] = dq;
    }
    __syncthreads();
    if (threadIdx.x == 0) {
        double ts = 0, tq = 0;
        for (int w = 0; w < NT / 64; ++w) {
            ts += redS[w];
            tq += redQ[w];
        }
        const double cnt = (double)pixPerStat * cpg;
        const double mean = ts / cnt;
        double var = tq / cnt - mean * mean;
        if (var < 0) var = 0;
        statS[0] = (float)mean;
        statS[1] = (float)(1.0 / sqrt(var + (double)eps));
    }
    __syncthreads();
    const float mean = statS[0], rstd = statS[1];
#pragma unroll
    for (int e = 0; e < VEC; ++e) {
        ga[e] *= rstd;
        be[e] -= mean * ga[e];
    }
    E* y = reinterpret_cast<E*>(a.y);
    const int hw = a.H * a.W;
    auto film_load = [&](long p, float (&sc)[VEC], float (&sh)[VEC]) {
        const float* fr = a.film + (p / hw) * a.filmLd + c0;
#pragma unroll
        for (int e = 0; e < VEC; e += 4) {
            if (a.filmVec) {
                const float4 s4 = *reinterpret_cast<const float4*>(fr + e);
                const float4 h4 = *reinterpret_cast<const float4*>(fr + a.C + e);
                sc[e] = s4.x; sc[e + 1] = s4.y; sc[e + 2] = s4.z; sc[e + 3] = s4.w;
                sh[e] = h4.x; sh[e + 1] = h4.y; sh[e + 2] = h4.z; sh[e + 3] = h4.w;
            } else {
#pragma unroll
                for (int jx = 0; jx < 4; ++jx) {
                    sc[e + jx] = fr[e + jx];
                    sh[e + jx] = fr[a.C + e + jx];
                }
            }
        }
    };
    auto run = [&](auto actTag) {
        constexpr int ACTC = decltype(actTag)::value;
        auto act1 = [&](float x) -> float {
            if constexpr (ACTC == 0) return x;
            else if constexpr (ACTC == 1) {
                if constexpr (sizeof(E) == 2) return x * __builtin_amdgcn_rcpf(1.f + __expf(-x));
                else return silu_f(x);
            } else return apply_act(x, a.act);
        };
        auto finish = [&](const uint4& raw, long p, const float (&sc)[VEC], const float (&sh)[VEC]) {
            float v[VEC];
            Vec16<E>::load(reinterpret_cast<const E*>(&raw), v);
#pragma unroll
            for (int e = 0; e < VEC; ++e) {
                float A = ga[e], B = be[e];
                if (a.film) {
                    const float m = 1.f + sc[e];
                    A *= m;
                    B = B * m + sh[e];
                }
                v[e] = act1(fmaf(v[e], A, B));
            }
            Vec16<E>::store(y + p * a.yLd + c0, v);
        };
        long qq = threadIdx.x / pp;
        for (; qq + rows < pixPerStat; qq += 2 * rows) {
            float sc0[VEC] = {}, sh0[VEC] = {}, sc1[VEC] = {}, sh1[VEC] = {};
            if (a.film) {
                film_load(pix0 + qq, sc0, sh0);
                film_load(pix0 + qq + rows, sc1, sh1);
            }
            finish(cache[qq * pp + k], pix0 + qq, sc0, sh0);
            finish(cache[(qq + rows) * pp + k], pix0 + qq + rows, sc1, sh1);
        }
        for (; qq < pixPerStat; qq += rows) {
            float sc0[VEC] = {}, sh0[VEC] = {};
            if (a.film) film_load(pix0 + qq, sc0, sh0);
            finish(cache[qq * pp + k], pix0 + qq, sc0, sh0);
        }
    };
    if (a.act == FLAIR_ACT_NONE) run(std::integral_constant<int, 0>{});
    else if (a.act == FLAIR_ACT_SILU) run(std::integral_constant<int, 1>{});
    else run(std::integral_constant<int, 2>{});
}

}

static int gn_blocks_per_stat(const flair_gn_params* p) {
    const int vec = p->dtype == FLAIR_BF16 ? 8 : 4;
    const int cv = p->C / vec > 0 ? p->C / vec : 1;
    const int rows = 256 / cv > 0 ? 256 / cv : 1;
    const long pix = (long)p->frames_per_stat * p->H * p->W;
    long bps = (pix + (long)rows * 16 - 1) / ((long)rows * 16);
    constexpr int cap = 512;
    if (bps > cap) bps = cap;
    if (bps < 1) bps = 1;
    return (int)bps;
}

extern "C" size_t flair_groupnorm_workspace_bytes(const flair_gn_params* p) {
    if (!p) return 0;
    const int nstat = p->F / p->frames_per_stat;
    const int bps = gn_blocks_per_stat(p);
    return ((size_t)nstat * bps * 2 * p->groups + (size_t)nstat * p->groups * 2) * sizeof(float);
}

extern "C" int flair_groupnorm_nhwc(const flair_gn_params* p, const void* x0, const void* x1,
                                    const float* gamma, const float* beta, const float* film,
                                    void* y, void* raw, void* workspace, hipStream_t stream) {
    FLAIR_CHECK(p && x0 && gamma && beta && y && workspace, "flair_groupnorm_nhwc: null argument");
    FLAIR_CHECK(p->dtype == FLAIR_F32 || p->dtype == FLAIR_BF16, "flair_groupnorm_nhwc: bad dtype");
    const int vec = p->dtype == FLAIR_BF16 ? 8 : 4;
    const int C = p->C;
    FLAIR_CHECK(C > 0 && C % vec == 0 && C % p->groups == 0, "flair_groupnorm_nhwc: C=%d groups=%d", C, p->groups);
    FLAIR_CHECK(p->c0 > 0 && p->c0 <= C && p->c0 % vec == 0 && (p->c0 == C || x1),
                "flair_groupnorm_nhwc: bad segment split c0=%d", p->c0);
    {
        auto ok = [&](const void* t, int ld, int c) { return ld >= c && ld % vec == 0 && ((uintptr_t)t) % 16 == 0; };
        FLAIR_CHECK(ok(x0, p->ld0, p->c0) && (p->c0 == C || ok(x1, p->ld1, C - p->c0)) && ok(y, p->y_ld, C) &&
                        (!raw || ok(raw, p->raw_ld, C)),
                    "flair_groupnorm_nhwc: strides/alignment (ld0 = %d, ld1 = %d, y_ld = %d, raw_ld = %d: at least the channels "
                    "they hold, multiples of %d elements; pointers 16-byte aligned)", p->ld0, p->ld1, p->y_ld, p->raw_ld, vec);
    }
    FLAIR_CHECK(p->F > 0 && p->frames_per_stat > 0 && p->F % p->frames_per_stat == 0,
                "flair_groupnorm_nhwc: frames %d / frames_per_stat %d", p->F, p->frames_per_stat);
    FLAIR_CHECK(p->resample >= 0 && p->resample <= 2, "flair_groupnorm_nhwc: resample mode");
    FLAIR_CHECK(p->resample != 1 || (p->H % 2 == 0 && p->W % 2 == 0), "flair_groupnorm_nhwc: odd size for pooling");
    const int cv = C / vec;
    FLAIR_CHECK(cv <= 512, "flair_groupnorm_nhwc: C=%d too wide", C);
    const int rows = cv <= 256 ? 256 / cv : 1;
    const int threads = rows * cv;
    const int nstat = p->F / p->frames_per_stat;
    const long pix = (long)p->frames_per_stat * p->H * p->W;
    const int bps = gn_blocks_per_stat(p);
    FLAIR_CHECK(!film || p->film_ld >= 2 * C, "flair_groupnorm_nhwc: film_ld");
    float* part = reinterpret_cast<float*>(workspace);
    float* stats = part + (size_t)nstat * bps * 2 * p->groups;

    GnSrc s;
    s.x[0] = x0; s.x[1] = x1;
    s.c[0] = p->c0; s.c[1] = C - p->c0;
    s.ld[0] = p->ld0; s.ld[1] = p->ld1;
    {
        const int cpg = C / p->groups;
        const int esz = p->dtype == FLAIR_BF16 ? 2 : 4;
        const long groupBytes = pix * cpg * esz;
        if (p->resample == 0 && !raw && cpg % vec == 0 && 1024 % (cpg / vec) == 0 && p->c0 % cpg == 0 && groupBytes <= (128l << 10) &&
            (long)nstat * p->groups >= 16) {
            GnApply a;
            a.s = s;
            a.C = C; a.groups = p->groups;
            a.F = p->F; a.H = p->H; a.W = p->W;
            a.framesPerStat = p->frames_per_stat;
            a.stats = nullptr; a.gamma = gamma; a.beta = beta; a.film = film; a.filmLd = p->film_ld;
            a.act = p->act; a.resample = 0;
            a.y = y; a.yLd = p->y_ld; a.raw = nullptr; a.rawLd = 0; a.blocksPerFrame = 0;
            a.filmVec = film && p->film_ld % 4 == 0 && (reinterpret_cast<uintptr_t>(film) & 15) == 0;
            static LdsAttrOnce attr0, attr1;
            {
                const hipError_t e0 = flair_max_lds_once(attr0, reinterpret_cast<const void*>(&gn_group_kernel<bf16_t>), 128 * 1024);
                const hipError_t e1 = flair_max_lds_once(attr1, reinterpret_cast<const void*>(&gn_group_kernel<float>), 128 * 1024);
                FLAIR_CHECK(e0 == hipSuccess && e1 == hipSuccess, "flair_groupnorm_nhwc: hipFuncSetAttribute failed");
            }
            const int grid = nstat * p->groups;
            if (p->dtype == FLAIR_BF16)
                hipLaunchKernelGGL(gn_group_kernel<bf16_t>, dim3(grid), dim3(1024), (size_t)groupBytes, stream, a, p->eps);
            else
                hipLaunchKernelGGL(gn_group_kernel<float>, dim3(grid), dim3(1024), (size_t)groupBytes, stream, a, p->eps);
            FLAIR_LAUNCH_CHECK();
            return FLAIR_OK;
        }
    }
    const size_t lds = (size_t)2 * rows * C * sizeof(float);
    if (p->dtype == FLAIR_BF16)
        hipLaunchKernelGGL(gn_partial_kernel<bf16_t>, dim3(nstat * bps), dim3(threads), lds, stream, s, C, p->groups, pix, bps,
                           part);
    else
        hipLaunchKernelGGL(gn_partial_kernel<float>, dim3(nstat * bps), dim3(threads), lds, stream, s, C, p->groups, pix, bps,
                           part);
    FLAIR_LAUNCH_CHECK();
    const int sg = nstat * p->groups;
    FLAIR_CHECK(sg % 4 == 0 || sg < 4, "flair_groupnorm_nhwc: groups");
    const int wavesPerBlock = sg >= 4 ? 4 : sg;
    hipLaunchKernelGGL(gn_finalize_kernel, dim3(sg / wavesPerBlock), dim3(64 * wavesPerBlock), 0, stream,
                       part, p->groups, C / p->groups, bps, pix, p->eps, stats);
    FLAIR_LAUNCH_CHECK();

    GnApply a;
    a.s = s;
    a.C = C; a.groups = p->groups;
    a.F = p->F; a.H = p->H; a.W = p->W;
    a.framesPerStat = p->frames_per_stat;
    a.stats = stats; a.gamma = gamma; a.beta = beta; a.film = film; a.filmLd = p->film_ld;
    a.act = p->act; a.resample = p->resample;
    a.y = y; a.yLd = p->y_ld; a.raw = raw; a.rawLd = p->raw_ld;
    const long outPix = p->resample == 1 ? (long)p->H * p->W / 4 : (long)p->H * p->W;
    int bpf = (int)((outPix + (long)rows * 4 - 1) / ((long)rows * 4));
    constexpr int totalBlocks = 1024;

    const int maxBpf = totalBlocks / p->F > 0 ? totalBlocks / p->F : 1;
    if (bpf > maxBpf) bpf = maxBpf;
    if (bpf < 1) bpf = 1;
    a.blocksPerFrame = bpf;
    if (p->dtype == FLAIR_BF16)
        hipLaunchKernelGGL(gn_apply_kernel<bf16_t>, dim3(p->F * bpf), dim3(threads), 0, stream, a);
    else
        hipLaunchKernelGGL(gn_apply_kernel<float>, dim3(p->F * bpf), dim3(threads), 0, stream, a);
    FLAIR_LAUNCH_CHECK();
    return FLAIR_OK;
}
```

### flair_amd/guided_diffusion/unet_new.py

```python
import math

import torch
import torch.nn as nn

from .. import ops
from .nn_new import conv_nd, linear, normalization, zero_module

A = ops


class PlaceHolder(nn.Module):

    def __init__(self, module):
        super().__init__()
        self.wrapped_module = module


LazyReshaper2D = LazyReshaper3D = PlaceHolder


class TemporalWrapper(PlaceHolder):
    """unet_new.py:50-59 (skipped when ``enable_cross_frames`` is False)."""


def _dev(p, device):
    t = p.detach()
    if t.device != device or t.dtype != torch.float32 or not t.is_contiguous():
        t = t.to(device=device, dtype=torch.float32).contiguous()
    return t


class Ctx:

    def __init__(self, dtype, device, T):
        self.dtype, self.device, self.T = dtype, device, T
        self.emb = None
        self.film_all = None
        self.flows = {}
        self.vsrpp_weights = None
        self.enable_cross_frames = True


def _pack(w, segs, dtype, device, cout_pad=None):
    return ops.pack_conv_weight(w.detach().to(device), segs, dtype, cout_pad)


class ResBlock(nn.Module):

    def __init__(self, channels, emb_channels, dropout, out_channels=None, use_conv=False,
                 use_scale_shift_norm=False, dims=2, use_checkpoint=False, up=False, down=False):
        super().__init__()
        if not use_scale_shift_norm:
            raise NotImplementedError("flair_amd: only use_scale_shift_norm=True (the shipped "
                                      "FLAIR configuration) is implemented")
        if use_conv:
            raise NotImplementedError("flair_amd: 3x3 skip convolutions are not used by FLAIR")
        self.channels = channels
        self.out_channels = out_channels or channels
        self.dims, self.up, self.down = dims, up, down
        self.in_layers = nn.Sequential(
            PlaceHolder(normalization(channels)), nn.SiLU(),
            PlaceHolder(conv_nd(dims, channels, self.out_channels, 3, padding=1)))
        self.emb_layers = nn.Sequential(nn.SiLU(), linear(emb_channels, 2 * self.out_channels))
        self.out_layers = nn.Sequential(
            PlaceHolder(normalization(self.out_channels)), nn.SiLU(), nn.Dropout(p=dropout),
            zero_module(PlaceHolder(conv_nd(dims, self.out_channels, self.out_channels, 3, padding=1))))
        if self.out_channels == channels:
            self.skip_connection = nn.Identity()
        else:
            self.skip_connection = PlaceHolder(conv_nd(dims, channels, self.out_channels, 1))
        self.film_off = 0
        self._pk = None

    def pack(self, dtype, device, split=None):
        c, co = self.channels, self.out_channels
        segs = [(s, s) for s in (split or [c])]
        self._pk = dict(
            w1=_pack(self.in_layers[2].wrapped_module.weight, [(c, c)], dtype, device),
            b1=_dev(self.in_layers[2].wrapped_module.bias, device),
            w2=_pack(self.out_layers[3].wrapped_module.weight, [(co, co)], dtype, device),
            b2=_dev(self.out_layers[3].wrapped_module.bias, device),
            g1=_dev(self.in_layers[0].wrapped_module.weight, device),
            be1=_dev(self.in_layers[0].wrapped_module.bias, device),
            g2=_dev(self.out_layers[0].wrapped_module.weight, device),
            be2=_dev(self.out_layers[0].wrapped_module.bias, device))
        if not isinstance(self.skip_connection, nn.Identity):
            self._pk["ws"] = _pack(self.skip_connection.wrapped_module.weight, segs, dtype, device)
            self._pk["bs"] = _dev(self.skip_connection.wrapped_module.bias, device)

    def run(self, ctx, x, x1=None):
        pk = self._pk
        co = self.out_channels
        k = (1, 3, 3) if self.dims == 2 else (3, 3, 3)
        film = ctx.film_all[:, self.film_off:self.film_off + 2 * co]
        eps = self.in_layers[0].wrapped_module.eps
        if self.up or self.down:
            assert x1 is None
            h, x = ops.group_norm(x, pk["g1"], pk["be1"], eps=eps, act=A.ACT_SILU,
                                  resample=2 if self.up else 1, want_raw=True)
        else:
            h = ops.group_norm(x, pk["g1"], pk["be1"], x1=x1, eps=eps, act=A.ACT_SILU)
        h = ops.conv(h, pk["w1"], pk["b1"], co, k)
        h = ops.group_norm(h, pk["g2"], pk["be2"], eps=eps, act=A.ACT_SILU, film=film)
        if "ws" in pk:
            skip = ops.conv([x] if x1 is None else [x, x1], pk["ws"], pk["bs"], co, (1, 1, 1))
        else:
            assert x1 is None
            skip = x
        return ops.conv(h, pk["w2"], pk["b2"], co, k, res0=skip)


QKV_ATTN_WIDTHS = (32, 64, 128)


def qkv_head_width(channels, num_heads):
    d = channels // num_heads if num_heads > 0 and channels % num_heads == 0 else 0
    if d <= 0 or d % 8:
        raise NotImplementedError(f"flair_amd: attention head width {channels}/{num_heads} unsupported "
                                  f"({QKV_ATTN_WIDTHS} and multiples of 64 from 192 to 1024 at any size, other "
                                  "multiples of 8 while width + H*W <= 2048)")
    return d


def temporal_head_width(channels, num_heads):
    d = channels // num_heads if num_heads > 0 and channels % num_heads == 0 else 0
    if d < 8 or d > 256 or d % 8:
        raise NotImplementedError(f"flair_amd: temporal attention head width {channels}/{num_heads} unsupported "
                                  "(multiples of 8 from 8 to 256)")
    return d


class QKVAttentionLegacy(nn.Module):

    def __init__(self, n_heads):
        super().__init__()
        self.n_heads = n_heads


class QKVAttention(QKVAttentionLegacy):
    """unet_new.py:573-605."""


class AttentionBlock(nn.Module):

    bottleneck = False

    def __init__(self, channels, num_heads=1, num_head_channels=-1, use_checkpoint=False,
                 use_new_attention_order=False):
        super().__init__()
        self.channels = channels
        if num_head_channels == -1:
            self.num_heads = num_heads
        else:
            assert channels % num_head_channels == 0
            self.num_heads = channels // num_head_channels
        qkv_head_width(channels, self.num_heads)
        if self.bottleneck:
            self.emb_layers = nn.Sequential(nn.SiLU(), linear(512, 512))
        self.norm = PlaceHolder(normalization(channels))
        self.qkv = conv_nd(1, channels, channels * 3, 1)
        self.attention = (QKVAttention if use_new_attention_order else QKVAttentionLegacy)(self.num_heads)
        self.new_order = use_new_attention_order
        self.proj_out = zero_module(conv_nd(1, channels, channels, 1))
        self.film_off = 0
        self._pk = None

    def pack(self, dtype, device):
        c = self.channels
        self._pk = dict(
            g=_dev(self.norm.wrapped_module.weight, device), be=_dev(self.norm.wrapped_module.bias, device),
            wqkv=_pack(self.qkv.weight.unsqueeze(-1), [(c, c)], dtype, device), bqkv=_dev(self.qkv.bias, device),
            wp=_pack(self.proj_out.weight.unsqueeze(-1), [(c, c)], dtype, device),
            bp=_dev(self.proj_out.bias, device))

    def run(self, ctx, x):
        pk, c = self._pk, self.channels
        n = ops.group_norm(x, pk["g"], pk["be"], eps=self.norm.wrapped_module.eps)
        qkv = ops.conv(n, pk["wqkv"], pk["bqkv"], 3 * c, (1, 1, 1))
        a = ops.qkv_attention(qkv, self.num_heads, new_order=self.new_order)
        if self.bottleneck:
            ops.add_frame_bias(a, ctx.film_all[:, self.film_off:self.film_off + c])
        return ops.conv(a, pk["wp"], pk["bp"], c, (1, 1, 1), res0=x)


class AttentionbottleBlock(AttentionBlock):

    bottleneck = True


class FalshAttn(nn.Module):
    """nn.py:389-394 -- marker only (the window attention kernel replaces flash-attn)."""


class TemporalAttention(nn.Module):

    def __init__(self, channels, num_frames, num_heads=1, num_head_channels=-1, use_checkpoint=False):
        super().__init__()
        self.channels = channels
        if num_head_channels == -1:
            self.num_heads = num_heads
        else:
            assert channels % num_head_channels == 0
            self.num_heads = channels // num_head_channels
        assert num_frames % 2 == 1, "num_frames must be odd"
        self.head_dim = temporal_head_width(channels, self.num_heads)
        self.num_frames = num_frames
        self.q_linear = linear(channels, channels)
        self.k_linear = linear(channels, channels)
        self.v_linear = linear(channels, channels)
        self.attn = FalshAttn()
        self.proj = zero_module(PlaceHolder(conv_nd(2, channels, channels, 1)))
        self.norm = PlaceHolder(normalization(channels))
        self._pk = None

    def pack(self, dtype, device):
        c, f = self.channels, self.num_frames
        offs = torch.arange(f, dtype=torch.float32, device=device) - f // 2
        mid = f // 2
        wq, wk, wv = (_dev(m.weight, device) for m in (self.q_linear, self.k_linear, self.v_linear))
        if torch.device(device).type == "cuda":
            pe = ops.timestep_embedding(offs, c)
            bq = ops.linear(pe[mid:mid + 1].contiguous(), wq, _dev(self.q_linear.bias, device))
            kpos = ops.linear(torch.cat([pe[:mid], pe[mid + 1:]]).contiguous(), wk, None)
        else:
            freqs = torch.exp(-math.log(10000.0) * torch.arange(c // 2, dtype=torch.float32) / (c // 2))
            ang = offs[:, None] * freqs[None]
            pe = torch.cat([torch.cos(ang), torch.sin(ang)], dim=-1)
            bq = pe[mid:mid + 1] @ wq.t() + _dev(self.q_linear.bias, device)
            kpos = torch.cat([pe[:mid], pe[mid + 1:]]) @ wk.t()
        wqkv = torch.cat([wq, wk, wv]).reshape(3 * c, c, 1, 1)
        bqkv = torch.cat([bq.reshape(-1), _dev(self.k_linear.bias, device), _dev(self.v_linear.bias, device)])
        self._pk = dict(
            g=_dev(self.norm.wrapped_module.weight, device), be=_dev(self.norm.wrapped_module.bias, device),
            wqkv=_pack(wqkv, [(c, c)], dtype, device), bqkv=bqkv.contiguous(), kpos=kpos,
            wp=_pack(self.proj.wrapped_module.weight, [(c, c)], dtype, device),
            bp=_dev(self.proj.wrapped_module.bias, device))

    def run(self, ctx, h):
        pk, c = self._pk, self.channels
        n = ops.group_norm(h, pk["g"], pk["be"], eps=self.norm.wrapped_module.eps)
        qkv = ops.conv(n, pk["wqkv"], pk["bqkv"], 3 * c, (1, 1, 1))
        a = ops.temporal_attention(qkv, pk["kpos"], self.num_frames,
                                   round_fp16=(ctx.dtype == torch.float32), head_dim=self.head_dim)
        return ops.conv(a, pk["wp"], pk["bp"], c, (1, 1, 1), res0=h)


class ResidualBlockNoBN(nn.Module):
    def __init__(self, mid_channels):
        super().__init__()
        self.conv1 = nn.Conv2d(mid_channels, mid_channels, 3, 1, 1, bias=True)
        self.conv2 = nn.Conv2d(mid_channels, mid_channels, 3, 1, 1, bias=True)


class ResidualBlocksWithInputConv(nn.Module):

    def __init__(self, in_channels, out_channels=64, num_blocks=1):
        super().__init__()
        if num_blocks != 1:
            raise NotImplementedError("flair_amd: FLAIR uses one residual block per trunk")
        self.main = nn.Sequential(nn.Conv2d(in_channels, out_channels, 3, 1, 1, bias=True),
                                  nn.LeakyReLU(negative_slope=0.1),
                                  nn.Sequential(ResidualBlockNoBN(out_channels)))

    def pack(self, dtype, device, split):
        c = self.main[0].out_channels
        rb = self.main[2][0]
        return dict(w0=_pack(self.main[0].weight, [(s, s) for s in split], dtype, device),
                    b0=_dev(self.main[0].bias, device),
                    w1=_pack(rb.conv1.weight, [(c, c)], dtype, device), b1=_dev(rb.conv1.bias, device),
                    w2=_pack(rb.conv2.weight, [(c, c)], dtype, device), b2=_dev(rb.conv2.bias, device))




def run_trunk(pk, segs, c, *, extra_res=None, out=None, out_scale=1.0):
    k = (1, 3, 3)
    t1 = ops.conv(segs, pk["w0"], pk["b0"], c, k, act=A.ACT_LRELU01)
    if c == 64 and ops.chain_supported(t1, c):
        return ops.conv_chain(t1, pk["w1"], pk["b1"], A.ACT_RELU, pk["w2"], pk["b2"], A.ACT_NONE, c, c,
                              res0=t1, res1=extra_res, out=out, out_scale=out_scale)
    t2 = ops.conv(t1, pk["w1"], pk["b1"], c, k, act=A.ACT_RELU)
    return ops.conv(t2, pk["w2"], pk["b2"], c, k, res0=t1, res1=extra_res, out=out, out_scale=out_scale)


class SecondOrderDeformableAlignment(nn.Module):

    def __init__(self, in_channels, out_channels, kernel_size=3, padding=1, deform_groups=16,
                 max_residue_magnitude=10):
        super().__init__()
        assert kernel_size == 3 and padding == 1
        self.in_channels, self.out_channels = in_channels, out_channels
        self.deform_groups, self.max_residue_magnitude = deform_groups, max_residue_magnitude
        self.weight = nn.Parameter(torch.empty(out_channels, in_channels, 3, 3))
        self.bias = nn.Parameter(torch.zeros(out_channels))
        stdv = 1.0 / math.sqrt(in_channels * 9)
        with torch.no_grad():
            self.weight.uniform_(-stdv, stdv)
        c = out_channels
        self.conv_offset = nn.Sequential(
            nn.Conv2d(3 * c + 4, c, 3, 1, 1), nn.LeakyReLU(negative_slope=0.1),
            nn.Conv2d(c, c, 3, 1, 1), nn.LeakyReLU(negative_slope=0.1),
            nn.Conv2d(c, c, 3, 1, 1), nn.LeakyReLU(negative_slope=0.1),
            nn.Conv2d(c, 27 * deform_groups, 3, 1, 1))
        zero_module(self.conv_offset[-1])

    def pack(self, dtype, device):
        c = self.out_channels
        ka = ops.k_align(dtype)
        co = self.conv_offset
        perm = ops.dcn_raw_permutation(self.deform_groups)
        w6, b6 = co[6].weight.detach()[perm], co[6].bias.detach()[perm]
        return dict(
            w0=_pack(co[0].weight, [(c, c), (c, c), (c, c), (4, ka)], dtype, device), b0=_dev(co[0].bias, device),
            w2=_pack(co[2].weight, [(c, c)], dtype, device), b2=_dev(co[2].bias, device),
            w4=_pack(co[4].weight, [(c, c)], dtype, device), b4=_dev(co[4].bias, device),
            w6=_pack(w6, [(c, c)], dtype, device), b6=_dev(b6, device),
            wd=_pack(self.weight, [(2 * c, 2 * c)], dtype, device), bd=_dev(self.bias, device))


class BasicVSRPP(nn.Module):

    def __init__(self, mid_channels=64, max_residue_magnitude=10, use_checkpoint=False):
        super().__init__()
        self.mid_channels = mid_channels
        self.deform_align = nn.ModuleDict()
        self.backbone = nn.ModuleDict()
        for i, name in enumerate(["backward_1", "forward_1"]):
            self.deform_align[name] = SecondOrderDeformableAlignment(
                2 * mid_channels, mid_channels, 3, padding=1, deform_groups=16,
                max_residue_magnitude=max_residue_magnitude)
            self.backbone[name] = ResidualBlocksWithInputConv((2 + i) * mid_channels, mid_channels, 1)
        self.reconstruction = ResidualBlocksWithInputConv(3 * mid_channels, mid_channels, 1)
        self.conv_last = zero_module(nn.Conv2d(mid_channels, mid_channels, 1, 1))
        self._pk = None

    def pack(self, dtype, device):
        c = self.mid_channels
        self._pk = dict(
            align={n: m.pack(dtype, device) for n, m in self.deform_align.items()},
            trunk={"backward_1": self.backbone["backward_1"].pack(dtype, device, [c, c]),
                   "forward_1": self.backbone["forward_1"].pack(dtype, device, [c, c, c])},
            recon=self.reconstruction.pack(dtype, device, [c, c, c]),
            wl=_pack(self.conv_last.weight, [(c, c)], dtype, device), bl=_dev(self.conv_last.bias, device))

    def _propagate(self, ctx, hidden, flows, name, others, weight, wmaps, dest):
        pk_a, pk_t = self._pk["align"][name], self._pk["trunk"][name]
        T, H, W, c = hidden.shape
        order = list(range(T))
        flow_idx = list(range(-1, T - 1))
        if "backward" in name:
            order = order[::-1]
            flow_idx = order
        zero_c = torch.zeros((1, H, W, c), dtype=ctx.dtype, device=ctx.device)
        ka = ops.k_align(ctx.dtype)
        k3 = (1, 3, 3)
        G = self.deform_align[name].deform_groups
        mag = float(self.deform_align[name].max_residue_magnitude)
        store = ctx.flows.get("_prop") if isinstance(ctx.flows, dict) else None
        key = (name, H, W, ctx.dtype, ka)
        cached = store.get(key) if store is not None else None
        fill = [] if (cached is None and store is not None) else None
        prop, prev2 = zero_c, None
        for i, idx in enumerate(order):
            cur = hidden[idx:idx + 1]
            if i > 0:
                flow_n1 = flows[flow_idx[i]:flow_idx[i] + 1]
                cond_n1 = torch.empty_like(zero_c)
                second = i > 1
                feat_n2 = prev2 if second else zero_c
                cond_n2 = torch.empty_like(zero_c) if second else zero_c
                if cached is not None:
                    flow_n2, flowpad = cached[i - 1]
                    ops.vsrpp_warp2(prop, feat_n2 if second else None, flow_n1, flow_n2, cond_n1, cond_n2 if second else None)
                else:
                    flowpad = torch.zeros((1, H, W, ka), dtype=ctx.dtype, device=ctx.device)
                    flow_n2 = torch.empty_like(flow_n1) if second else None
                    ops.vsrpp_prep(prop, feat_n2 if second else None, flow_n1,
                                   flows[flow_idx[i - 1]:flow_idx[i - 1] + 1] if second else None,
                                   cond_n1, cond_n2 if second else None, flow_n2, flowpad)
                    if fill is not None:
                        fill.append((flow_n2, flowpad))
                o = ops.conv([cond_n1, cur, cond_n2, flowpad], pk_a["w0"], pk_a["b0"], c, k3, act=A.ACT_LRELU01)
                if c == 64 and ops.chain_supported(o, c):
                    o = ops.conv_chain(o, pk_a["w2"], pk_a["b2"], A.ACT_LRELU01, pk_a["w4"], pk_a["b4"],
                                       A.ACT_LRELU01, c, c)
                else:
                    o = ops.conv(o, pk_a["w2"], pk_a["b2"], c, k3, act=A.ACT_LRELU01)
                    o = ops.conv(o, pk_a["w4"], pk_a["b4"], c, k3, act=A.ACT_LRELU01)
                if c == 64 and ops.chain_supported(o, c) and W % 32 == 0:
                    raw = ops.conv_chain(o, None, None, A.ACT_NONE, pk_a["w6"], pk_a["b6"], A.ACT_DCN_OFFSETS, c, 27 * G,
                                         act_param=mag, act_period=3 * G)
                else:
                    raw = ops.conv(o, pk_a["w6"], pk_a["b6"], 27 * G, k3, act=A.ACT_DCN_OFFSETS, act_param=mag,
                                   act_period=3 * G)
                aligned = ops.dcn_align(prop, feat_n2, raw, flow_n1, flow_n2, pk_a["wd"], pk_a["bd"], c,
                                        groups=G, max_mag=mag, raw_activated=True)

            else:
                aligned = zero_c
            segs = [cur] + [o_[idx:idx + 1] for o_ in others] + [aligned]
            new = run_trunk(pk_t, segs, c, extra_res=aligned, out=dest[idx:idx + 1], out_scale=weight)
            if wmaps is not None:
                ops.scale_pixels(new, wmaps[idx])
            prev2, prop = (prop if i > 0 else None), new
        if fill is not None:
            store[key] = fill
        return dest

    def run(self, ctx, hidden):
        T, H, W, c = hidden.shape
        flows_forward, flows_backward = ctx.flows[W]
        weight, wmaps = 1.0, None
        vw = ctx.vsrpp_weights
        if isinstance(vw, (float, int)):
            weight = float(vw)
        elif vw is not None:
            wm = vw.reshape(T, vw.shape[-2], vw.shape[-1], 1).float().contiguous()
            if wm.shape[1] != H or wm.shape[2] != W:
                wm = ops.resize(wm, (H, W), ops.RESIZE_NEAREST)
            wmaps = [wm[i] for i in range(T)]
        bwd = torch.empty_like(hidden)
        fwd = torch.empty_like(hidden)
        self._propagate(ctx, hidden, flows_backward, "backward_1", [], weight, wmaps, bwd)
        ff = flows_forward if flows_forward is not None else flows_backward.flip(0)
        self._propagate(ctx, hidden, ff, "forward_1", [bwd], weight, wmaps, fwd)
        rec = run_trunk(self._pk["recon"], [hidden, bwd, fwd], c)
        return ops.conv(rec, self._pk["wl"], self._pk["bl"], c, (1, 1, 1), res0=hidden)


class _ConvModule(nn.Module):
    def __init__(self, cin, cout):
        super().__init__()
        self.conv = nn.Conv2d(cin, cout, kernel_size=7, stride=1, padding=3)


class SPyNetBasicModule(nn.Module):
    def __init__(self):
        super().__init__()
        ch = [8, 32, 64, 32, 16, 2]
        self.basic_module = nn.Sequential(*[_ConvModule(ch[i], ch[i + 1]) for i in range(5)])


class SPyNet(nn.Module):

    def __init__(self, pretrained=None):
        super().__init__()
        self.basic_module = nn.ModuleList([SPyNetBasicModule() for _ in range(6)])
        self.register_buffer("mean", torch.tensor([0.485, 0.456, 0.406]).view(1, 3, 1, 1))
        self.register_buffer("std", torch.tensor([0.229, 0.224, 0.225]).view(1, 3, 1, 1))
        self._pk = None

    def pack(self, device):
        f32 = torch.float32
        levels = []
        for bm in self.basic_module:
            convs = [m.conv for m in bm.basic_module]
            ws = [_pack(convs[0].weight, [(3, 4), (3, 4), (2, 8)], f32, device)]
            ws += [_pack(convs[j].weight, [(convs[j].in_channels,) * 2], f32, device) for j in (1, 2, 3)]
            ws.append(_pack(convs[4].weight, [(16, 16)], f32, device, cout_pad=4))
            bs = [_dev(convs[j].bias, device) for j in range(4)]
            bs.append(torch.cat([_dev(convs[4].bias, device), torch.zeros(2, device=device)]).contiguous())
            levels.append((ws, bs))
        mean = _dev(self.mean.reshape(-1), device)
        istd = (1.0 / _dev(self.std.reshape(-1), device)).contiguous()
        self._pk = dict(levels=levels, mean=mean, istd=istd)

    def run(self, ref, supp):
        F_, h0, w0, _ = ref.shape
        dev = ref.device
        if F_ == 0:
            return torch.zeros((0, h0, w0, 2), dtype=torch.float32, device=dev)
        h = h0 if h0 % 32 == 0 else 32 * (h0 // 32 + 1)
        w = w0 if w0 % 32 == 0 else 32 * (w0 // 32 + 1)
        if (h, w) != (h0, w0):
            ref = ops.resize(ref, (h, w), ops.RESIZE_BILINEAR, channels=3)
            supp = ops.resize(supp, (h, w), ops.RESIZE_BILINEAR, channels=3)
        sizes = [(h >> (5 - l), w >> (5 - l)) for l in range(6)]
        bufs = [torch.zeros((F_, *sizes[l], 16), dtype=torch.float32, device=dev) for l in range(6)]
        sp = [None] * 6
        ops.cast_channels(ref[..., :3], bufs[5], 0)
        sp[5] = supp
        for l in range(4, -1, -1):
            ops.resize(bufs[l + 1][..., 0:4], sizes[l], ops.RESIZE_AVGPOOL2, channels=3, out=bufs[l][..., 0:4])
            sp[l] = ops.resize(sp[l + 1], sizes[l], ops.RESIZE_AVGPOOL2, channels=3)
        flow = None
        k7 = (1, 7, 7)
        for l in range(6):
            b = bufs[l]
            if l > 0:
                ops.resize(flow, sizes[l], ops.RESIZE_BILINEAR_AC, channels=2, out=b[..., 8:12],
                           scale_c0=2.0, scale_c1=2.0)
            ops.flow_warp(sp[l], b[..., 8:10], border=True, out=b[..., 4:8])
            ws, bs = self._pk["levels"][l]
            y = ops.conv(b, ws[0], bs[0], 32, k7, act=A.ACT_RELU)
            y = ops.conv(y, ws[1], bs[1], 64, k7, act=A.ACT_RELU)
            y = ops.conv(y, ws[2], bs[2], 32, k7, act=A.ACT_RELU)
            y = ops.conv(y, ws[3], bs[3], 16, k7, act=A.ACT_RELU)
            flow = ops.conv(y, ws[4], bs[4], 4, k7, res0=b[..., 8:12])
        out = torch.empty((F_, h0, w0, 2), dtype=torch.float32, device=dev)
        ops.resize(flow, (h0, w0), ops.RESIZE_BILINEAR, channels=2, out=out,
                   scale_c0=float(w0) / float(w), scale_c1=float(h0) / float(h))
        return out


class TimestepEmbedSequential(nn.Sequential):

    def run(self, ctx, h, skip=None):
        for i, layer in enumerate(self):
            inner = layer.wrapped_module if isinstance(layer, PlaceHolder) else layer
            if isinstance(layer, TemporalWrapper) and not ctx.enable_cross_frames:
                continue
            if isinstance(inner, ResBlock):
                h = inner.run(ctx, h, skip if i == 0 else None)
            elif isinstance(inner, (AttentionBlock, TemporalAttention, BasicVSRPP)):
                h = inner.run(ctx, h)
            elif isinstance(inner, nn.Conv2d):
                h = ops.conv(h, inner._pk_w, inner._pk_b, inner.out_channels, (1, 3, 3))
            elif isinstance(inner, nn.Identity):
                pass
            else:
                raise TypeError(f"flair_amd: no executor for {type(inner).__name__}")
        return h


class UNetModel(nn.Module):

    def __init__(self, image_size, in_channels, model_channels, out_channels, num_res_blocks,
                 attention_resolutions, rnn_resolutions, dropout=0, channel_mult=(1, 2, 4, 8),
                 conv_resample=True, dims=2, num_classes=None, use_checkpoint=False, use_fp16=False,
                 num_heads=1, num_head_channels=-1, num_heads_upsample=-1, use_scale_shift_norm=False,
                 resblock_updown=False, use_new_attention_order=False, temporal_block=False):
        super().__init__()
        if dims != 2 or num_classes is not None or not resblock_updown:
            raise NotImplementedError("flair_amd: UNetModel covers the FLAIR video configuration "
                                      "(dims=2, resblock_updown=True, no class conditioning)")
        if num_heads_upsample == -1:
            num_heads_upsample = num_heads
        self.image_size, self.in_channels, self.model_channels = image_size, in_channels, model_channels
        self.out_channels, self.num_res_blocks = out_channels, num_res_blocks
        self.attention_resolutions, self.rnn_resolutions = attention_resolutions, rnn_resolutions
        self.channel_mult = channel_mult
        self.dtype = torch.bfloat16 if use_fp16 else torch.float32
        self.need_flows_res = [image_size // s for s in rnn_resolutions]

        ted = model_channels * 4
        self.time_embed = nn.Sequential(linear(model_channels, ted), nn.SiLU(), linear(ted, ted))
        self.spynet = SPyNet(pretrained=None)

        def res(cin, cout, d=2, **kw):
            return ResBlock(cin, ted, dropout, out_channels=cout, dims=d, use_checkpoint=use_checkpoint,
                            use_scale_shift_norm=use_scale_shift_norm, **kw)

        def level_layers(cin, cout, ds, heads):
            layers = [res(cin, cout)]
            if temporal_block:
                layers.append(TemporalWrapper(res(cout, cout, 3)))
            if ds in attention_resolutions:
                layers.append(AttentionBlock(cout, use_checkpoint=use_checkpoint, num_heads=heads,
                                             num_head_channels=num_head_channels,
                                             use_new_attention_order=use_new_attention_order))
                if temporal_block:
                    layers.append(TemporalWrapper(TemporalAttention(cout, 5, heads, num_head_channels,
                                                                    use_checkpoint)))
            if ds in rnn_resolutions and temporal_block:
                layers.append(TemporalWrapper(BasicVSRPP(mid_channels=cout, use_checkpoint=use_checkpoint)))
            return layers

        ch = input_ch = int(channel_mult[0] * model_channels)
        self.input_blocks = nn.ModuleList(
            [TimestepEmbedSequential(LazyReshaper2D(conv_nd(dims, in_channels, ch, 3, padding=1)))])
        chans, ds = [ch], 1
        for level, mult in enumerate(channel_mult):
            for _ in range(num_res_blocks):
                cout = int(mult * model_channels)
                self.input_blocks.append(TimestepEmbedSequential(*level_layers(ch, cout, ds, num_heads)))
                ch = cout
                chans.append(ch)
            if level != len(channel_mult) - 1:
                self.input_blocks.append(TimestepEmbedSequential(res(ch, ch, down=True)))
                chans.append(ch)
                ds *= 2
        ident = nn.Identity
        self.middle_block = TimestepEmbedSequential(
            res(ch, ch),
            TemporalWrapper(res(ch, ch, 3)) if temporal_block else ident(),
            AttentionbottleBlock(ch, use_checkpoint=use_checkpoint, num_heads=num_heads,
                                 num_head_channels=num_head_channels,
                                 use_new_attention_order=use_new_attention_order),
            TemporalWrapper(TemporalAttention(ch, 5, num_heads, num_head_channels, use_checkpoint))
            if temporal_block else ident(),
            res(ch, ch),
            TemporalWrapper(res(ch, ch, 3)) if temporal_block else ident())
        self._skip_split = []
        self.output_blocks = nn.ModuleList([])
        for level, mult in list(enumerate(channel_mult))[::-1]:
            for i in range(num_res_blocks + 1):
                ich = chans.pop()
                cout = int(model_channels * mult)
                layers = level_layers(ch + ich, cout, ds, num_heads_upsample)
                self._skip_split.append((ch, ich))
                ch = cout
                if level and i == num_res_blocks:
                    layers.append(res(ch, ch, up=True))
                    ds //= 2
                self.output_blocks.append(TimestepEmbedSequential(*layers))
        self.out = nn.Sequential(LazyReshaper3D(normalization(ch)), nn.SiLU(),
                                 zero_module(LazyReshaper2D(conv_nd(dims, input_ch, out_channels, 3, padding=1))))
        self._packed_key = None
        self._flow_cache = {}
        self._graphs = {}
        self.use_hip_graph = False

    def enable_hip_graph(self, flag=True):
        self.use_hip_graph = bool(flag)
        self._graphs = {}
        return self

    def convert_to_fp16(self):
        self.dtype = torch.bfloat16
        self._packed_key = None
        self._graphs = {}

    def convert_to_fp32(self):
        self.dtype = torch.float32
        self._packed_key = None
        self._graphs = {}

    def load_state_dict(self, *args, **kwargs):
        out = super().load_state_dict(*args, **kwargs)
        self._packed_key = None
        self._graphs = {}
        return out

    def reset_flow_cache(self):
        self._flow_cache = {}
        self._flow_gen = getattr(self, "_flow_gen", 0) + 1

    def _res_blocks(self):
        for m in self.modules():
            if isinstance(m, ResBlock):
                yield m

    def _ensure_packed(self, device):
        key = (self.dtype, device)
        if self._packed_key == key:
            return
        dt = self.dtype
        ka = ops.k_align(dt)
        stem = self.input_blocks[0][0].wrapped_module
        stem._pk_w = _pack(stem.weight, [(self.in_channels, ops.pad_channels(self.in_channels, dt))], dt, device)
        stem._pk_b = _dev(stem.bias, device)
        first_out = {id(st[0]): split for st, split in zip(self.output_blocks, self._skip_split)}
        ws, bs, off = [], [], 0
        for m in self.modules():
            if isinstance(m, ResBlock):
                m.pack(dt, device, list(first_out[id(m)]) if id(m) in first_out else None)
            elif isinstance(m, (AttentionBlock, TemporalAttention, BasicVSRPP)):
                m.pack(dt, device)
            else:
                continue
            if isinstance(m, ResBlock) or getattr(m, "bottleneck", False):
                lin = m.emb_layers[1]
                m.film_off = off
                ws.append(_dev(lin.weight, device))
                bs.append(_dev(lin.bias, device))
                off += lin.out_features
        self._emb_w = torch.cat(ws).contiguous()
        self._emb_b = torch.cat(bs).contiguous()
        self.spynet.pack(device)
        self._te = [_dev(p, device) for p in (self.time_embed[0].weight, self.time_embed[0].bias,
                                               self.time_embed[2].weight, self.time_embed[2].bias)]
        head = self.out[2].wrapped_module
        cpad = (self.out_channels + 3) // 4 * 4
        self._head_w = _pack(head.weight, [(head.in_channels,) * 2], dt, device, cout_pad=cpad)
        self._head_b = torch.cat([_dev(head.bias, device),
                                  torch.zeros(cpad - self.out_channels, device=device)]).contiguous()
        self._head_g = _dev(self.out[0].wrapped_module.weight, device)
        self._head_be = _dev(self.out[0].wrapped_module.bias, device)
        self._packed_key = key
        self._flow_cache = {}

    def compute_flow(self, lqs):
        T, _, h, w = lqs.shape
        raw = torch.zeros((T, h, w, 4), dtype=torch.float32, device=lqs.device)
        ops.nchw_to_clip(lqs.contiguous(), raw, 0)
        return self._flows_from_clip(raw)

    def _flows_from_clip(self, raw):
        if raw.shape[0] < 2:
            empty = torch.zeros((0, raw.shape[1], raw.shape[2], 2), dtype=torch.float32, device=raw.device)
            return empty, empty
        pk = self.spynet._pk
        norm = torch.zeros_like(raw)
        ops.affine_channels(raw, 3, 0.5, 0.5, 0.0, 1.0, pk["mean"], pk["istd"], norm)
        a, b = norm[:-1], norm[1:]
        flows_backward = self.spynet.run(a, b)
        flows_forward = self.spynet.run(b, a)
        return flows_forward, flows_backward

    def _flows_for(self, rnn_clip):
        key = (rnn_clip.data_ptr(), rnn_clip._version, tuple(rnn_clip.shape))
        hit = self._flow_cache.get(key)
        if hit is None:
            T, _, h, w = rnn_clip.shape
            raw = torch.zeros((T, h, w, 4), dtype=torch.float32, device=rnn_clip.device)
            ops.nchw_to_clip(rnn_clip.contiguous(), raw, 0)
            flows = {}
            for r in self.need_flows_res:
                src = raw
                if w != r:
                    src = ops.resize(raw, (r, r), ops.RESIZE_BICUBIC, channels=3)
                flows[r] = self._flows_from_clip(src)
            flows["_prop"] = {}
            if len(self._flow_cache) >= 16:
                self._flow_cache.clear()
            hit = (flows, rnn_clip)
            self._flow_cache[key] = hit
        return hit[0]

    def forward(self, x, timesteps, low_res_input=None, num_frames=None, rnn_input=None,
                enable_cross_frames=True, vsrpp_weights=None, **kwargs):
        if not x.is_cuda:
            raise RuntimeError("flair_amd.UNetModel runs on the MI355X only (tensors must be on "
                               "'cuda'); there is no CPU path")
        self._ensure_packed(x.device)
        T = int(num_frames)
        B = x.shape[0] // T
        if rnn_input is None:
            rnn_input = low_res_input
        outs = []
        for b in range(B):
            vw = vsrpp_weights
            if isinstance(vw, torch.Tensor):
                vw = vw[b]
            fn = self._forward_clip_graphed if (self.use_hip_graph and not isinstance(vw, torch.Tensor)
                                                and getattr(self, "_trace", None) is None) else self._forward_clip
            outs.append(fn(x[b * T:(b + 1) * T].float().contiguous(), timesteps[b * T:(b + 1) * T],
                           low_res_input[b].float(), rnn_input[b].float(), enable_cross_frames, vw,
                           **({"clip": b} if fn == self._forward_clip_graphed else {})))
        return outs[0] if B == 1 else torch.cat(outs, dim=0)

    def _forward_clip_graphed(self, x, t, low_res, rnn, enable_cross_frames, vsrpp_weights, clip=0):
        key = (tuple(x.shape), self.dtype, bool(enable_cross_frames), vsrpp_weights, x.device, clip)
        ent = self._graphs.get(key)
        src = (rnn.data_ptr(), rnn._version, low_res.data_ptr(), low_res._version, getattr(self, "_flow_gen", 0))
        if ent is not None and ent["src"] != src:
            del self._graphs[key]
            ent = None
        if ent is None:
            st = dict(x=x.clone(), t=t.clone(), lr=low_res.clone(), rnn=rnn.clone())
            flows = self._flows_for(st["rnn"])
            cur = torch.cuda.current_stream()
            side = torch.cuda.Stream()
            side.wait_stream(cur)
            with torch.cuda.stream(side):
                self._forward_clip(st["x"], st["t"], st["lr"], st["rnn"], enable_cross_frames, vsrpp_weights,
                                   flows=flows)
            cur.wait_stream(side)
            torch.cuda.synchronize()
            graph = torch.cuda.CUDAGraph()
            with torch.cuda.graph(graph, capture_error_mode="thread_local"):
                out = self._forward_clip(st["x"], st["t"], st["lr"], st["rnn"], enable_cross_frames,
                                         vsrpp_weights, flows=flows)
            ent = dict(graph=graph, st=st, out=out, src=src, flows=flows)
            self._graphs[key] = ent
        st = ent["st"]
        st["x"].copy_(x)
        st["t"].copy_(t)
        ent["graph"].replay()
        return ent["out"]

    def _forward_clip(self, x, t, low_res, rnn, enable_cross_frames, vsrpp_weights, flows=None):
        T, _, H, W = x.shape
        dev, dt = x.device, self.dtype
        ctx = Ctx(dt, dev, T)
        ctx.enable_cross_frames = enable_cross_frames
        ctx.vsrpp_weights = vsrpp_weights
        ctx.flows = flows if flows is not None else self._flows_for(rnn)
        temb = ops.timestep_embedding(t.float().contiguous(), self.model_channels)
        e = ops.linear(temb, self._te[0], self._te[1], act_out=A.ACT_SILU)
        ctx.emb = ops.linear(e, self._te[2], self._te[3])
        ctx.film_all = ops.linear(ctx.emb, self._emb_w, self._emb_b, act_in=A.ACT_SILU)
        cin = ops.pad_channels(self.in_channels, dt)
        h = torch.zeros((T, H, W, cin), dtype=dt, device=dev)
        ops.nchw_to_clip(x, h, 0)
        ops.nchw_to_clip(low_res.contiguous(), h, x.shape[1])
        hs = []
        trace = getattr(self, "_trace", None)
        for i, blk in enumerate(self.input_blocks):
            h = blk.run(ctx, h)
            hs.append(h)
            if trace is not None:
                trace.append((f"input_blocks.{i}", h))
        h = self.middle_block.run(ctx, h)
        if trace is not None:
            trace.append(("middle_block", h))
        for i, blk in enumerate(self.output_blocks):
            h = blk.run(ctx, h, hs.pop())
            if trace is not None:
                trace.append((f"output_blocks.{i}", h))
        h = ops.group_norm(h, self._head_g, self._head_be, eps=self.out[0].wrapped_module.eps, act=A.ACT_SILU)
        y = ops.conv(h, self._head_w, self._head_b, self._head_w.shape[0], (1, 3, 3))
        return ops.clip_to_nchw(y, self.out_channels)
```

### flair_amd/ops.py

```python
import ctypes

import torch

from . import _lib
from ._lib import (ACT_DCN_OFFSETS, ACT_GELU, ACT_LRELU01, ACT_LRELU02, ACT_NONE, ACT_RELU, ACT_SILU, ConvParams, check, dtype_code, lib,
                   ptr, stream)

__all__ = ["conv", "conv_chain", "group_norm", "nchw_to_clip", "clip_to_nchw", "timestep_embedding", "linear",
           "qkv_attention", "temporal_attention", "flow_warp", "flow_compose", "resize",
           "dcn_align", "dcn_raw_permutation", "scale_pixels", "predict_xstart", "sampler_update",
           "ACT_NONE", "ACT_RELU", "ACT_LRELU01", "ACT_SILU", "ACT_DCN_OFFSETS", "ACT_LRELU02", "ACT_GELU"]


class GnParams(ctypes.Structure):
    _fields_ = [("dtype", ctypes.c_int), ("C", ctypes.c_int), ("c0", ctypes.c_int),
                ("ld0", ctypes.c_int), ("ld1", ctypes.c_int), ("groups", ctypes.c_int),
                ("F", ctypes.c_int), ("H", ctypes.c_int), ("W", ctypes.c_int),
                ("frames_per_stat", ctypes.c_int), ("eps", ctypes.c_float), ("act", ctypes.c_int),
                ("resample", ctypes.c_int), ("y_ld", ctypes.c_int), ("raw_ld", ctypes.c_int),
                ("film_ld", ctypes.c_int)]


class SamplerCoefs(ctypes.Structure):
    _fields_ = [("gamma", ctypes.c_float), ("w_aux", ctypes.c_float),
                ("sqrt_recip_alphas_cumprod", ctypes.c_float),
                ("sqrt_recipm1_alphas_cumprod", ctypes.c_float),
                ("sqrt_alphas_cumprod_prev", ctypes.c_float),
                ("sqrt_one_minus_alphas_cumprod_prev", ctypes.c_float),
                ("sqrt_one_minus_rho", ctypes.c_float), ("sqrt_rho", ctypes.c_float),
                ("clip_denoised", ctypes.c_int), ("nonzero", ctypes.c_int),
                ("frame_elems", ctypes.c_long), ("frames", ctypes.c_int),
                ("prev_frames", ctypes.c_int)]


class AttnParams(ctypes.Structure):
    _fields_ = [("dtype", ctypes.c_int), ("frames", ctypes.c_int), ("L", ctypes.c_int),
                ("heads", ctypes.c_int), ("head_dim", ctypes.c_int), ("ld", ctypes.c_int),
                ("out_ld", ctypes.c_int), ("q_off", ctypes.c_int), ("k_off", ctypes.c_int),
                ("v_off", ctypes.c_int), ("head_stride", ctypes.c_int), ("scale", ctypes.c_float)]


class TAttnParams(ctypes.Structure):
    _fields_ = [("dtype", ctypes.c_int), ("T", ctypes.c_int), ("H", ctypes.c_int),
                ("W", ctypes.c_int), ("C", ctypes.c_int), ("window", ctypes.c_int),
                ("ld", ctypes.c_int), ("out_ld", ctypes.c_int), ("round_fp16", ctypes.c_int),
                ("scale", ctypes.c_float), ("head_dim", ctypes.c_int)]


class DcnParams(ctypes.Structure):
    _fields_ = [("dtype", ctypes.c_int), ("F", ctypes.c_int), ("H", ctypes.c_int),
                ("W", ctypes.c_int), ("Cin", ctypes.c_int), ("Cout", ctypes.c_int),
                ("G", ctypes.c_int), ("x_ld", ctypes.c_int * 2), ("raw_ld", ctypes.c_int),
                ("y_ld", ctypes.c_int), ("max_residue_magnitude", ctypes.c_float), ("raw_activated", ctypes.c_int)]


def _ld(t):
    assert t.dim() == 4 and t.stride(3) == 1, "clip tensors are (T,H,W,C) with C innermost"
    ld = t.stride(2)
    assert t.stride(1) == ld * t.shape[2] and (t.shape[0] == 1 or t.stride(0) == ld * t.shape[1] * t.shape[2]), \
        "clip tensor must be dense over (T,H,W)"
    return ld


def _f32(t):
    assert t is None or (t.dtype == torch.float32 and t.is_contiguous())
    return t


def k_align(dtype):
    return 32 if dtype == torch.bfloat16 else 16


def pad_channels(c, dtype):
    g = k_align(dtype)
    return (c + g - 1) // g * g


def conv(xs, weight, bias, cout, kernel, *, out=None, act=ACT_NONE, res0=None, res1=None,
         out_scale=1.0, stride=1, frame_bias=None, act_param=0.0, act_period=0, asym_pad=False, reflect_pad=False):
    if isinstance(xs, torch.Tensor):
        xs = [xs]
    x0 = xs[0]
    T, H, W, _ = x0.shape
    p = ConvParams()
    p.dtype = dtype_code(x0)
    p.T, p.H, p.W = T, H, W
    p.KT, p.KH, p.KW = kernel
    p.Cout = cout
    p.nseg = len(xs)
    arr = (ctypes.c_void_p * 4)()
    for i, x in enumerate(xs):
        assert x.dtype == x0.dtype and x.shape[:3] == x0.shape[:3]
        p.seg_c[i] = x.shape[3]
        p.seg_ld[i] = _ld(x)
        arr[i] = x.data_ptr()
    p.stride = stride
    p.asym_pad = int(asym_pad)
    p.reflect_pad = int(reflect_pad)
    p.frame_bias_ld = frame_bias.stride(0) if frame_bias is not None else 0
    if frame_bias is not None:
        assert frame_bias.dtype == torch.float32 and frame_bias.stride(1) == 1 and frame_bias.shape[0] == T
    Ho, Wo = (H + stride - 1) // stride, (W + stride - 1) // stride
    if out is None:
        out = torch.empty((T, Ho, Wo, cout), dtype=x0.dtype, device=x0.device)
    assert tuple(out.shape[:3]) == (T, Ho, Wo) and out.shape[3] >= cout and out.dtype == x0.dtype
    p.y_ld = _ld(out)
    p.res_ld[0] = _ld(res0) if res0 is not None else 0
    p.res_ld[1] = _ld(res1) if res1 is not None else 0
    p.act = act
    p.act_param, p.act_period = act_param, act_period
    p.out_scale = out_scale
    assert weight.dtype == x0.dtype and weight.is_contiguous()
    e0 = _prof_begin()
    wsb = _conv_ws_bytes(p)
    ws = _workspace(wsb, x0.device, "conv") if wsb else None

    def launch(_keep=xs):
        check(lib().flair_conv_nhwc(ctypes.byref(p), arr, ptr(weight), ptr(_f32(bias)), ptr(frame_bias), ptr(res0),
                                    ptr(res1), ptr(out), ptr(ws), ctypes.c_size_t(wsb), stream()), "flair_conv_nhwc")
    launch()
    if e0 is not None:
        cin = sum(x.shape[3] for x in xs)
        taps = kernel[0] * kernel[1] * kernel[2]
        esz = x0.element_size()
        flops = 2.0 * T * Ho * Wo * cout * cin * taps
        nbytes = esz * (cin * T * H * W + cout * T * Ho * Wo * (1 + (res0 is not None) + (res1 is not None))
                        + cout * taps * cin)
        _prof_end(e0, ("conv", lib().flair_conv_variant(ctypes.byref(p))), x0.dtype, flops, nbytes, launch,
                  ("conv", T, H, W, tuple(x.shape[3] for x in xs), cout, tuple(kernel), stride, act,
                   res0 is not None, res1 is not None, frame_bias is not None))
    return out


PROFILE = None


def _prof_begin():
    if PROFILE is None:
        return None
    e0 = torch.cuda.Event(enable_timing=True)
    e0.record()
    return e0


def _prof_end(e0, family, dtype, flops, nbytes, replay=None, sig=None):
    e1 = torch.cuda.Event(enable_timing=True)
    e1.record()
    PROFILE.append((family, str(dtype), float(flops), float(nbytes), e0, e1, replay, sig))


def conv_variant(T, H, W, cins, cout, kernel, dtype=torch.bfloat16, stride=1):
    p = ConvParams()
    p.dtype = 1 if dtype == torch.bfloat16 else 0
    p.T, p.H, p.W = T, H, W
    p.KT, p.KH, p.KW = kernel
    p.Cout = cout
    p.nseg = len(cins)
    for i, c in enumerate(cins):
        p.seg_c[i] = c
        p.seg_ld[i] = c
    p.stride = stride
    p.y_ld = cout
    return lib().flair_conv_variant(ctypes.byref(p))


def _conv_ws_bytes(p):
    f = lib().flair_conv_workspace_bytes
    f.restype = ctypes.c_size_t
    return f(ctypes.byref(p))


def pack_conv_weight(w, seg_channels, dtype, cout_pad=None):
    cout, cin = w.shape[:2]
    taps = 1
    for k in w.shape[2:]:
        taps *= k
    w = w.reshape(cout, cin, taps).permute(0, 2, 1).float()
    parts, o = [], 0
    for real, padded in seg_channels:
        seg = w[:, :, o:o + real]
        if padded > real:
            seg = torch.cat([seg, seg.new_zeros(cout, taps, padded - real)], dim=2)
        parts.append(seg)
        o += real
    assert o == cin, (o, cin)
    w = torch.cat(parts, dim=2)
    if cout_pad is not None and cout_pad > cout:
        w = torch.cat([w, w.new_zeros(cout_pad - cout, taps, w.shape[2])], dim=0)
    return w.to(dtype).contiguous()


class ChainParams(ctypes.Structure):
    _fields_ = [("dtype", ctypes.c_int), ("T", ctypes.c_int), ("H", ctypes.c_int), ("W", ctypes.c_int),
                ("C", ctypes.c_int), ("CoutB", ctypes.c_int), ("nseg", ctypes.c_int),
                ("seg_c", ctypes.c_int * 4), ("seg_ld", ctypes.c_int * 4), ("y_ld", ctypes.c_int),
                ("res_ld", ctypes.c_int * 2), ("actA", ctypes.c_int), ("actB", ctypes.c_int),
                ("out_scale", ctypes.c_float), ("act_param", ctypes.c_float), ("act_period", ctypes.c_int)]


def chain_supported(xs, c_mid):
    x0 = xs[0] if isinstance(xs, (list, tuple)) else xs
    T, H, W, _ = x0.shape
    tiles = T * ((H + 7) // 8) * (W // 32 if W % 32 == 0 and T * ((H + 7) // 8) * (W // 32) >= 192 else W // 8)
    return c_mid in (64, 128) and W % 8 == 0 and tiles <= 512


def conv_chain(xs, wA, bA, actA, wB, bB, actB, c_mid, coutB, *, res0=None, res1=None, out_scale=1.0, out=None,
               act_param=0.0, act_period=0):
    if isinstance(xs, torch.Tensor):
        xs = [xs]
    x0 = xs[0]
    T, H, W, _ = x0.shape
    p = ChainParams()
    p.dtype = dtype_code(x0)
    p.T, p.H, p.W = T, H, W
    p.C, p.CoutB = c_mid, coutB
    p.nseg = len(xs)
    arr = (ctypes.c_void_p * 4)()
    for i, x in enumerate(xs):
        assert x.dtype == x0.dtype and x.shape[:3] == x0.shape[:3]
        p.seg_c[i] = x.shape[3]
        p.seg_ld[i] = _ld(x)
        arr[i] = x.data_ptr()
    if out is None:
        out = torch.empty((T, H, W, coutB), dtype=x0.dtype, device=x0.device)
    assert tuple(out.shape[:3]) == (T, H, W) and out.shape[3] >= coutB and out.dtype == x0.dtype
    p.y_ld = _ld(out)
    p.res_ld[0] = _ld(res0) if res0 is not None else 0
    p.res_ld[1] = _ld(res1) if res1 is not None else 0
    p.actA, p.actB = actA, actB
    p.act_param, p.act_period = act_param, act_period
    p.out_scale = out_scale
    assert wB.dtype == x0.dtype and wB.is_contiguous() and (wA is None or (wA.dtype == x0.dtype and wA.is_contiguous()))
    e0 = _prof_begin()

    def launch(_keep=xs):
        check(lib().flair_conv_chain(ctypes.byref(p), arr, ptr(wA), ptr(_f32(bA)), ptr(wB), ptr(_f32(bB)), ptr(res0),
                                     ptr(res1), ptr(out), stream()), "flair_conv_chain")
    launch()
    if e0 is not None:
        cin = sum(x.shape[3] for x in xs)
        esz = x0.element_size()
        px = T * H * W
        flops = 2.0 * 9 * px * (c_mid * coutB + (cin * c_mid if wA is not None else 0))
        nbytes = esz * (px * (cin + coutB * (1 + (res0 is not None) + (res1 is not None)))
                        + 9 * c_mid * coutB + (9 * cin * c_mid if wA is not None else 0))
        _prof_end(e0, ("chain", 2 if wA is not None else 1, c_mid), x0.dtype, flops, nbytes, launch,
                  ("chain", T, H, W, tuple(x.shape[3] for x in xs), c_mid, coutB, wA is not None, res0 is not None,
                   res1 is not None))
    return out


_gn_ws = {}


def _workspace(nbytes, device, tag="gn"):
    key = (tag, device, torch.cuda.current_stream().cuda_stream)
    buf = _gn_ws.get(key)
    if buf is None or buf.numel() < nbytes:
        buf = torch.empty(max(nbytes, 1 << 20), dtype=torch.uint8, device=device)
        _gn_ws[key] = buf
    return buf


def group_norm(x, gamma, beta, *, x1=None, groups=32, eps=1e-5, act=ACT_NONE, film=None,
               frames_per_stat=None, resample=0, out=None, want_raw=False):
    T, H, W, c0 = x.shape
    C = c0 + (x1.shape[3] if x1 is not None else 0)
    p = GnParams()
    p.dtype = dtype_code(x)
    p.C, p.c0 = C, c0
    p.ld0 = _ld(x)
    p.ld1 = _ld(x1) if x1 is not None else 0
    p.groups = groups
    p.F, p.H, p.W = T, H, W
    p.frames_per_stat = frames_per_stat or T
    p.eps = eps
    p.act = act
    p.resample = resample
    Ho, Wo = (H // 2, W // 2) if resample == 1 else ((H * 2, W * 2) if resample == 2 else (H, W))
    if out is None:
        out = torch.empty((T, Ho, Wo, C), dtype=x.dtype, device=x.device)
    raw = torch.empty((T, Ho, Wo, C), dtype=x.dtype, device=x.device) if want_raw else None
    p.y_ld = _ld(out)
    p.raw_ld = _ld(raw) if raw is not None else 0
    p.film_ld = film.stride(0) if film is not None else 0
    if film is not None:
        assert film.dtype == torch.float32 and film.stride(1) == 1 and film.shape[0] == T
    ws = _workspace(lib_ws_bytes(p), x.device)
    e0 = _prof_begin()

    def launch():
        check(lib().flair_groupnorm_nhwc(ctypes.byref(p), ptr(x), ptr(x1), ptr(_f32(gamma)), ptr(_f32(beta)),
                                         ptr(film), ptr(out), ptr(raw), ptr(ws), stream()),
              "flair_groupnorm_nhwc")
    launch()
    if e0 is not None:
        numel_in, numel_out = T * H * W * C, T * Ho * Wo * C
        _prof_end(e0, ("gn",), x.dtype, 8.0 * numel_in,
                  x.element_size() * (2 * numel_in + numel_out * (2 if want_raw else 1)), launch,
                  ("gn", T, H, W, C, c0, groups, p.frames_per_stat, act, resample, want_raw, film is not None))
    return (out, raw) if want_raw else out


def lib_ws_bytes(p):
    f = lib().flair_groupnorm_workspace_bytes
    f.restype = ctypes.c_size_t
    return f(ctypes.byref(p))


def nchw_to_clip(src, dst, coff=0):
    N, C, H, W = src.shape
    assert src.dtype == torch.float32 and src.is_contiguous()
    check(lib().flair_nchw_f32_to_nhwc(ptr(src), N, C, H, W, ptr(dst), dtype_code(dst), _ld(dst), coff,
                                       stream()), "flair_nchw_f32_to_nhwc")
    return dst


def clip_to_nchw(src, C, coff=0, out=None):
    N, H, W, _ = src.shape
    if out is None:
        out = torch.empty((N, C, H, W), dtype=torch.float32, device=src.device)
    check(lib().flair_nhwc_to_nchw_f32(ptr(src), dtype_code(src), _ld(src), coff, N, C, H, W, ptr(out),
                                       stream()), "flair_nhwc_to_nchw_f32")
    return out


def timestep_embedding(t, dim, max_period=10000.0, out=None, sin_first=False):
    assert t.dtype == torch.float32 and t.is_contiguous()
    N = t.shape[0]
    if out is None:
        out = torch.empty((N, dim), dtype=torch.float32, device=t.device)
    check(lib().flair_timestep_embedding(ptr(t), N, dim, ctypes.c_float(max_period), int(sin_first), ptr(out),
                                         stream()), "flair_timestep_embedding")
    return out


def linear(x, w, b, *, act_in=ACT_NONE, act_out=ACT_NONE, out=None):
    M, K = x.shape
    N = w.shape[0]
    assert x.dtype == torch.float32 and w.dtype == torch.float32 and x.is_contiguous() and w.is_contiguous()
    if out is None:
        out = torch.empty((M, N), dtype=torch.float32, device=x.device)
    check(lib().flair_linear_f32(ptr(x), M, K, ptr(w), ptr(b), N, act_in, act_out, ptr(out), out.stride(0),
                                 stream()), "flair_linear_f32")
    return out


def qkv_attention(qkv, heads, *, new_order=False, out=None):
    F_, H, W, C3 = qkv.shape
    C = C3 // 3
    p = AttnParams()
    p.dtype = dtype_code(qkv)
    p.frames, p.L, p.heads, p.head_dim = F_, H * W, heads, C // heads
    p.ld = _ld(qkv)
    if out is None:
        out = torch.empty((F_, H, W, C), dtype=qkv.dtype, device=qkv.device)
    p.out_ld = _ld(out)
    d = C // heads
    if new_order:
        p.q_off, p.k_off, p.v_off, p.head_stride = 0, C, 2 * C, d
    else:
        p.q_off, p.k_off, p.v_off, p.head_stride = 0, d, 2 * d, 3 * d
    p.scale = 1.0 / (d ** 0.5)
    e0 = _prof_begin()

    def launch():
        check(lib().flair_qkv_attention(ctypes.byref(p), ptr(qkv), ptr(out), stream()), "flair_qkv_attention")
    launch()
    if e0 is not None:
        L = H * W
        _prof_end(e0, ("attn", L), qkv.dtype, 4.0 * F_ * heads * L * L * d, qkv.element_size() * 4.0 * F_ * L * C,
                  launch, ("attn", F_, L, heads, d, new_order))
    return out


def temporal_attention(qkv, kpos, window, *, round_fp16, head_dim=64, out=None):
    T, H, W, C3 = qkv.shape
    C = C3 // 3
    p = TAttnParams()
    p.dtype = dtype_code(qkv)
    p.T, p.H, p.W, p.C, p.window = T, H, W, C, window
    p.ld = _ld(qkv)
    if out is None:
        out = torch.empty((T, H, W, C), dtype=qkv.dtype, device=qkv.device)
    p.out_ld = _ld(out)
    p.round_fp16 = int(round_fp16)
    p.head_dim = head_dim
    p.scale = 1.0 / (head_dim ** 0.5)
    assert kpos.shape == (window - 1, C)
    check(lib().flair_temporal_attention(ctypes.byref(p), ptr(qkv), ptr(_f32(kpos)), ptr(out), stream()),
          "flair_temporal_attention")
    return out


def flow_warp(x, flow, *, border=False, out=None):
    F_, H, W, C = x.shape
    assert flow.dtype == torch.float32 and flow.shape == (F_, H, W, 2)
    if out is None:
        out = torch.empty((F_, H, W, C), dtype=x.dtype, device=x.device)
    check(lib().flair_flow_warp(ptr(x), dtype_code(x), _ld(x), ptr(flow), _ld(flow), F_, H, W, C, int(border),
                                ptr(out), _ld(out), stream()), "flair_flow_warp")
    return out


def flow_compose(f1, f2, out=None):
    F_, H, W, _ = f1.shape
    assert f1.dtype == torch.float32 and f1.is_contiguous() and f2.is_contiguous()
    if out is None:
        out = torch.empty_like(f1)
    check(lib().flair_flow_compose(ptr(f1), ptr(f2), F_, H, W, ptr(out), stream()), "flair_flow_compose")
    return out


RESIZE_BILINEAR, RESIZE_BILINEAR_AC, RESIZE_BICUBIC, RESIZE_AVGPOOL2, RESIZE_NEAREST = 0, 1, 2, 3, 4


def resize(x, size, mode, *, channels=None, out=None, scale_c0=1.0, scale_c1=1.0):
    F_, Hi, Wi, Cx = x.shape
    C = channels or Cx
    Ho, Wo = size
    if out is None:
        out = torch.zeros((F_, Ho, Wo, Cx), dtype=x.dtype, device=x.device)
    check(lib().flair_resize_nhwc(ptr(x), dtype_code(x), _ld(x), F_, Hi, Wi, C, mode, Ho, Wo, ptr(out), _ld(out),
                                  ctypes.c_float(scale_c0), ctypes.c_float(scale_c1), stream()),
          "flair_resize_nhwc")
    return out


def dcn_raw_permutation(groups):
    G = groups
    perm = torch.empty(27 * G, dtype=torch.long)
    for k in range(9):
        for g in range(G):
            for e in range(2):
                perm[3 * G * k + 2 * g + e] = 2 * (g * 9 + k) + e
            perm[3 * G * k + 2 * G + g] = 18 * G + g * 9 + k
    return perm


def dcn_align(x0, x1, raw, flow1, flow2, weight, bias, cout, *, groups=16, max_mag=10.0, out=None, raw_activated=False):
    F_, H, W, ch = x0.shape
    p = DcnParams()
    p.dtype = dtype_code(x0)
    p.F, p.H, p.W = F_, H, W
    p.Cin, p.Cout, p.G = 2 * ch, cout, groups
    p.x_ld[0], p.x_ld[1] = _ld(x0), _ld(x1)
    p.raw_ld = _ld(raw)
    if out is None:
        out = torch.empty((F_, H, W, cout), dtype=x0.dtype, device=x0.device)
    p.y_ld = _ld(out)
    p.max_residue_magnitude = max_mag
    p.raw_activated = int(raw_activated)
    e0 = _prof_begin()
# ... 409 lines not shown
```

### include/flair_hip.h

```cpp
#ifndef FLAIR_HIP_H
#define FLAIR_HIP_H

#include <stddef.h>
#include <stdint.h>

#ifdef __cplusplus
extern "C" {
#endif

#ifndef __HIP_PLATFORM_AMD__
typedef struct ihipStream_t* hipStream_t;
#endif

typedef enum {
    FLAIR_OK = 0,
    FLAIR_ERR_ARG = -1,
    FLAIR_ERR_HIP = -2
} flair_status;

typedef enum { FLAIR_F32 = 0, FLAIR_BF16 = 1 } flair_dtype;

typedef enum {
    FLAIR_ACT_NONE = 0,
    FLAIR_ACT_RELU = 1,
    FLAIR_ACT_LRELU01 = 2,
    FLAIR_ACT_SILU = 3,
    FLAIR_ACT_DCN_OFFSETS = 4,
    FLAIR_ACT_LRELU02 = 5,
    FLAIR_ACT_GELU = 6
} flair_act;

const char* flair_last_error(void);
int flair_abi_version(void);

typedef struct {
    int dtype;
    int T, H, W;
    int KT, KH, KW;
    int Cout;
    int nseg;
    int seg_c[4];
    int seg_ld[4];
    int y_ld;
    int res_ld[2];
    int act;
    float out_scale;
    int frame_bias_ld;
    int stride;
    float act_param;
    int act_period;
    int asym_pad;
    int reflect_pad;
} flair_conv_params;

size_t flair_conv_workspace_bytes(const flair_conv_params* p);
int flair_conv_nhwc(const flair_conv_params* p, const void* const* x, const void* w,
                    const float* bias, const float* frame_bias, const void* res0, const void* res1,
                    void* y, void* workspace, size_t workspace_bytes, hipStream_t stream);
int flair_conv_variant(const flair_conv_params* p);


typedef struct {
    int dtype;
    int T, H, W;
    int C;
    int CoutB;
    int nseg;
    int seg_c[4];
    int seg_ld[4];
    int y_ld;
    int res_ld[2];
    int actA, actB;
    float out_scale;
    float act_param;
    int act_period;
} flair_chain_params;

int flair_conv_chain(const flair_chain_params* p, const void* const* x, const void* wA, const float* biasA,
                     const void* wB, const float* biasB, const void* res0, const void* res1, void* y,
                     hipStream_t stream);


typedef struct {
    int dtype;
    int C, c0;
    int ld0, ld1;
    int groups;
    int F, H, W;
    int frames_per_stat;
    float eps;
    int act;
    int resample;
    int y_ld, raw_ld;
    int film_ld;
} flair_gn_params;

size_t flair_groupnorm_workspace_bytes(const flair_gn_params* p);
int flair_groupnorm_nhwc(const flair_gn_params* p, const void* x0, const void* x1,
                         const float* gamma, const float* beta, const float* film, void* y,
                         void* raw, void* workspace, hipStream_t stream);

int flair_nchw_f32_to_nhwc(const float* src, int N, int C, int H, int W, void* dst, int dtype,
                           int dst_ld, int dst_coff, hipStream_t stream);
int flair_nhwc_to_nchw_f32(const void* src, int dtype, int src_ld, int src_coff, int N, int C,
                           int H, int W, float* dst, hipStream_t stream);

int flair_timestep_embedding(const float* t, int N, int dim, float max_period, int sin_first,
                             float* out, hipStream_t stream);

int flair_linear_f32(const float* x, int M, int K, const float* w, const float* bias, int N,
                     int act_in, int act_out, float* y, int y_ld, hipStream_t stream);

typedef struct {
    float gamma, w_aux;
    float sqrt_recip_alphas_cumprod, sqrt_recipm1_alphas_cumprod;
    float sqrt_alphas_cumprod_prev, sqrt_one_minus_alphas_cumprod_prev;
    float sqrt_one_minus_rho, sqrt_rho;
    int clip_denoised, nonzero;
    long frame_elems;
    int frames, prev_frames;
} flair_sampler_coefs;

int flair_predict_xstart(const float* x, const float* model_out, int N, int C, int Cm, int H, int W,
                         float c_recip, float c_recipm1, int clip, float* x0, hipStream_t stream);
int flair_sampler_update(const flair_sampler_coefs* c, const float* x, float* x0,
                         const float* restored, const float* aux, const float* z,
                         const float* prev_recon, long n, float* x_prev, hipStream_t stream);
int flair_axpby_f32(const float* x, const float* y, float a, float b, float lo, float hi, long n,
                    float* out, hipStream_t stream);
int flair_learned_range_variance(const float* model_out, int N, int C, int H, int W, float min_log,
                                 float max_log, float* variance, float* log_variance,
                                 hipStream_t stream);
int flair_affine_channels_f32(const float* x, int x_ld, int C, long P, float a, float b, float lo,
                              float hi, const float* sub, const float* mul, float* y, int y_ld,
                              hipStream_t stream);
int flair_gated_blend(const void* x, int x_ld, const void* m, int m_ld, const float* gate, int gate_ld,
                      int dtype, int C, int F, long HW, void* y, int y_ld, hipStream_t stream);
int flair_add_act_nhwc(const void* x0, int x0_ld, const void* x1, int x1_ld, int dtype, int C, long P,
                       int act, void* y, int y_ld, hipStream_t stream);
int flair_maxpool3x3s2_nhwc(const void* x, int x_ld, int dtype, int F, int H, int W, int C, void* y,
                            int y_ld, hipStream_t stream);
int flair_dwconv_nhwc(const float* x, int x_ld, int T, int H, int W, int C, int stride, const float* w_dw,
                      const float* b_dw, const float* w_pw, const float* b_pw, int Cout, int act, float* y,
                      int y_ld, hipStream_t stream);
int flair_dwconv7_nhwc(const void* x, int x_ld, int dtype, int T, int H, int W, int C, const float* w,
                       const float* bias, void* y, int y_ld, hipStream_t stream);
int flair_add_frame_bias(void* x, int dtype, int ld, int C, int F, long HW, const float* bias,
                         int bias_ld, hipStream_t stream);
int flair_cast_channels(const float* src, int src_ld, int C, long P, void* dst, int dtype,
                        int dst_ld, int dst_coff, hipStream_t stream);
int flair_scale_pixels(void* x, int dtype, int ld, int C, long P, const float* wmap,
                       hipStream_t stream);

typedef struct {
    int dtype;
    int frames, L, heads, head_dim;
    int ld, out_ld;
    int q_off, k_off, v_off, head_stride;
    float scale;
} flair_attn_params;
int flair_qkv_attention(const flair_attn_params* p, const void* qkv, void* out, hipStream_t stream);

typedef struct {
    int dtype;
    int T, H, W, C, window;
    int ld, out_ld;
    int round_fp16;
    float scale;
    int head_dim;
} flair_tattn_params;
int flair_temporal_attention(const flair_tattn_params* p, const void* qkv, const float* kpos,
                             void* out, hipStream_t stream);

int flair_flow_warp(const void* x, int dtype, int x_ld, const float* flow, int flow_ld, int F,
                    int H, int W, int C, int border, void* y, int y_ld, hipStream_t stream);
int flair_flow_compose(const float* f1, const float* f2, int F, int H, int W, float* out,
                       hipStream_t stream);
int flair_vsrpp_warp2(const void* prop, int prop_ld, const void* feat2, int feat2_ld, const float* flow1,
                      const float* flow2, int dtype, int H, int W, int C, void* cond1, int cond1_ld,
                      void* cond2, int cond2_ld, hipStream_t stream);
int flair_vsrpp_prep(const void* prop, int prop_ld, const void* feat2, int feat2_ld,
                     const float* flow1, const float* flow_prev, int dtype, int H, int W, int C,
                     void* cond1, int cond1_ld, void* cond2, int cond2_ld, float* flow2_out,
                     void* flowpad, int pad_ld, hipStream_t stream);
int flair_resize_nhwc(const void* x, int dtype, int x_ld, int F, int Hi, int Wi, int C, int mode,
                      int Ho, int Wo, void* y, int y_ld, float scale_c0, float scale_c1,
                      hipStream_t stream);

typedef struct {
    int dtype;
    int F, H, W;
    int Cin, Cout, G;
    int x_ld[2];
    int raw_ld, y_ld;
    float max_residue_magnitude;
    int raw_activated;
} flair_dcn_params;
int flair_dcn_align(const flair_dcn_params* p, const void* x0, const void* x1, const void* raw,
                    const float* flow1, const float* flow2, const void* w, const float* bias,
                    void* y, hipStream_t stream);

int flair_depthwise_filter(const float* x, int planes, int Hin, int Win, const float* filt, int kh,
                           int kw, int pad, int out_stride, int out_offset, int stuff,
                           int stuff_offset, int Hout, int Wout, int reflect, float* y,
                           hipStream_t stream);
int flair_jpeg_roundtrip(const float* x, int N, int S, const float* q_luma, const float* q_chroma,
                         const float* dct8, float* workspace, float* y, float* luma_q, float* chroma_q,
                         hipStream_t stream);
int flair_matmul_f32(const float* A, long a_batch_stride, const float* B, long b_batch_stride,
                     float* C, int batch, int M, int N, int K, hipStream_t stream);
int flair_gather_mac_f32(const float* x, long outer, int Lin, long inner, const int* fov,
                         const float* w, int taps, int Lout, float* y, hipStream_t stream);

int flair_layernorm_nhwc(const void* x, int dtype, int x_ld, long rows, int C, const float* gamma,
                         const float* beta, float eps, void* y, int y_ld, const float* pos, int pos_rows,
                         void* y2, int y2_ld, hipStream_t stream);
int flair_attention_wide(const flair_attn_params* p, const void* qkv, void* out, hipStream_t stream);
int flair_argmax_codebook(const void* logits, int dtype, int ld, long rows, int N, const float* codebook, int D,
                          const int* forced_idx, int* idx, void* y, int y_ld, hipStream_t stream);
int flair_vq_nearest_nhwc(const void* z, int dtype, int ld, long rows, int D, const float* codebook, int N,
                          const int* forced_idx, int* idx, void* y, int y_ld, hipStream_t stream);
int flair_adain_nhwc(const void* content, int c_ld, const void* style, int s_ld, int dtype, int frames, int HW,
                     int C, float eps, void* y, int y_ld, hipStream_t stream);
int flair_sft_fuse(const void* dec, const void* scale, const void* shift, float w, int dtype, long n, void* y,
                   hipStream_t stream);

int flair_global_avgpool_nhwc(const void* x, int dtype, int x_ld, int F, int H, int W, int C, float* y, int y_ld,
                              hipStream_t stream);
int flair_channel_gate_nhwc(const void* x, int x_ld, int dtype, int F, long HW, int C, const float* gate, int gate_ld,
                            int gate_is_logit, int add_x, const float* bias, int bias_ld, const void* a, int a_ld,
                            void* y, int y_ld, hipStream_t stream);
int flair_upsample_argmax_nhwc(const void* logits, int dtype, int ld, int F, int h, int w, int N, int H, int W,
                               const float* table, int D, int* idx, float* y, int y_ld, hipStream_t stream);

int flair_warp_affine_cubic(const void* src, int src_is_f64, int N, int C, int Hs, int Ws, const double* minv,
                            int Hd, int Wd, const float* border, int pre, int post, float* dst, hipStream_t stream);
int flair_face_mask_blur(const int* parse_idx, int N, int H, int W, const double* lut, int nlut, const double* kern,
                         int ksize, int repeats, int edge, double div, double* tmp, double* mask, hipStream_t stream);
int flair_face_blend(const float* x0, const float* face, const float* mask, int N, int C, int H, int W, float* out,
                     hipStream_t stream);

int flair_bcast_weights(void* blob, size_t bytes, int root, void* rccl_comm, hipStream_t stream);

int flair_probe_matrix_rate(int iters, int workgroups_per_cu, float* sink, double* flop_out, hipStream_t stream);
int flair_probe_stream_rate(const void* src, void* dst, size_t bytes, int mode, hipStream_t stream);

#ifdef __cplusplus
}
#endif
#endif
```

Before: 0.8838.

## Fuse GroupNorm statistics into the conv epilogue and reuse them in group_norm

The bf16 DMA 3x3 conv kernel gains an optional epilogue that reduces per-channel sum and sum-of-squares of its bf16 output over each tile. It uses lane swizzles and LDS and writes one partial per tile slot. GroupNorm takes these partials and finalizes group mean and rstd in a small kernel, skipping its own read pass over the activation. This adds register and LDS pressure and extra stores to the conv, and requires a new ABI with plumbing in the model.

New measurement: 0.8862 (median of 6 runs). Within noise of the previous version (+0.3%).

```diff
diff --git a/flair_amd/csrc/api.hip b/flair_amd/csrc/api.hip
--- a/flair_amd/csrc/api.hip
+++ b/flair_amd/csrc/api.hip
@@ -13,7 +13,7 @@
 }
 
 extern "C" const char* flair_last_error(void) { return g_err; }
-extern "C" int flair_abi_version(void) { return 11; }
+extern "C" int flair_abi_version(void) { return 12; }
 
 #include <dlfcn.h>
 
diff --git a/flair_amd/csrc/conv.hip b/flair_amd/csrc/conv.hip
--- a/flair_amd/csrc/conv.hip
+++ b/flair_amd/csrc/conv.hip
@@ -37,6 +37,7 @@
     int actPeriod;
     int Hin, Win;
     int esz;
+    float* stat;
 };
 
 template <typename E> struct Mma;
@@ -84,6 +85,16 @@
 __device__ __forceinline__ int staged_row(int id) {
     const int g = id >> 3;
     return (g >> 2) * 8 + (g & 3) + 4 * ((id >> 2) & 1);
+}
+
+template <int N, int BIT>
+__device__ __forceinline__ void stat_halve(float (&h)[8], int lane) {
+    const bool up = lane & BIT;
+#pragma unroll
+    for (int q = 0; q < N; ++q) {
+        const float keep = up ? h[q + N] : h[q], send = up ? h[q] : h[q + N];
+        h[q] = keep + __uint_as_float(__builtin_amdgcn_ds_swizzle(__float_as_uint(send), 0x1f | (BIT << 10)));
+    }
 }
 
 template <typename E>
@@ -777,7 +788,7 @@
     int t, h0, w0, co0;
 };
 
-template <int NW, int RPW, int NSTAGE>
+template <int NW, int RPW, int NSTAGE, bool STATS>
 __device__ __forceinline__ void conv3x3_dma_body(const ConvArgs& a, int nTiles, int tilesPerXcd) {
     using E = bf16_t;
     static_assert((RPW == 1 || RPW == 2) && NSTAGE == 2, "the clip-level and one-tile forms (two stages)");
@@ -789,7 +800,9 @@
     constexpr int HALO_BYTES = HALO_INSTR * 1024;
     constexpr int STAGE_BYTES = HALO_BYTES + W_INSTR * 1024;
     constexpr int NSLOT = (HALO_INSTR + W_INSTR + NW - 1) / NW;
-    constexpr int BIAS_OFF = NSTAGE * STAGE_BYTES + NW * 1024;
+    constexpr int IDLE_BYTES = STATS ? 1024 : NW * 1024;
+    constexpr int STAT_OFF = NSTAGE * STAGE_BYTES + IDLE_BYTES;
+    constexpr int BIAS_OFF = STAT_OFF + (STATS ? 2 * NW * 512 : 0);
     extern __shared__ __attribute__((aligned(16))) char smem[];
 
     const int tid = threadIdx.x, lane = tid & 63;
@@ -831,10 +844,12 @@
         hchunk[i] = (unsigned)((lchunk ^ ((c >> 2) & 3)) << 4);
     }
     auto setup_tile = [&](const DmaTile& tl) {
+        int lrow_ = lrow;
+        if constexpr (STATS) asm volatile("" : "+v"(lrow_));
 #pragma unroll
         for (int i = 0; i < NSLOT; ++i) {
             const int id = wave * NSLOT + i;
-            const int R = id * 16 + lrow;
+            const int R = id * 16 + lrow_;
             const int hr = R / HWP, c = R - hr * HWP;
             const int hh = tl.h0 - 1 + hr, ww = tl.w0 - 1 + c;
             const bool okh = R < HALO_ROWS && (unsigned)hh < (unsigned)H && (unsigned)ww < (unsigned)W;
@@ -895,7 +910,7 @@
             d.z = isw ? wdesc.z : xdesc.z;
             d.w = 0x00020000u;
             const bool idle = wave * NSLOT + i >= HALO_INSTR + W_INSTR;
-            dma16(d, isw ? offw : offh, idle ? (unsigned)(NSTAGE * STAGE_BYTES + ((wave * NSLOT + i - HALO_INSTR - W_INSTR) % NW) * 1024) : sbase + i * 1024);
+            dma16(d, isw ? offw : offh, idle ? (unsigned)(NSTAGE * STAGE_BYTES + ((wave * NSLOT + i - HALO_INSTR - W_INSTR) % (IDLE_BYTES / 1024)) * 1024) : sbase + i * 1024);
         }
     };
 
@@ -989,6 +1004,7 @@
         }
 #pragma unroll
         for (int i = 0; i < 2; ++i) {
+            float sred[2] = {0.f, 0.f};
 #pragma unroll
             for (int jj = 0; jj < 2; ++jj) {
                 const int cofs = i * 32 + 16 * jj;
@@ -999,6 +1015,11 @@
                     const float4 b1 = *reinterpret_cast<const float4*>(bl + cofs + 4);
                     bv[0] = b0.x; bv[1] = b0.y; bv[2] = b0.z; bv[3] = b0.w; bv[4] = b1.x; bv[5] = b1.y; bv[6] = b1.z; bv[7] = b1.w;
                 }
+                float sv[STATS ? 16 : 1];
+                if constexpr (STATS) {
+#pragma unroll
+                    for (int q = 0; q < 16; ++q) sv[q] = 0.f;
+                }
 #pragma unroll
                 for (int j = 0; j < RPW; ++j) {
                     float v[8];
@@ -1038,8 +1059,48 @@
                     const uint4 ov = *reinterpret_cast<const uint4*>(out);
                     const unsigned yo = lane_ok ? yLane + (unsigned)(j * W) * yLdB + 2u * cofs : FLAIR_OOB;
                     __builtin_amdgcn_raw_buffer_store_b128(u32x4_t{ov.x, ov.y, ov.z, ov.w}, yd, (int)yo, 0, 0);
-                }
-            }
+                    if constexpr (STATS) {
+                        float rv[8];
+                        Vec16<E>::load(out, rv);
+#pragma unroll
+                        for (int e = 0; e < 8; ++e) {
+                            sv[e] += rv[e];
+                            sv[8 + e] = fmaf(rv[e], rv[e], sv[8 + e]);
+                        }
+                    }
+                }
+                if constexpr (STATS) {
+                    float h[8];
+#pragma unroll
+                    for (int e = 0; e < 8; ++e) {
+                        const auto sw2 = __builtin_amdgcn_permlane16_swap(__float_as_uint(sv[e]), __float_as_uint(sv[8 + e]), false, false);
+                        h[e] = __uint_as_float(sw2[0]) + __uint_as_float(sw2[1]);
+                    }
+                    stat_halve<4, 8>(h, lr);
+                    stat_halve<2, 4>(h, lr);
+                    stat_halve<1, 2>(h, lr);
+                    sred[jj] = h[0];
+                }
+            }
+            if constexpr (STATS) {
+                float h[8];
+                h[0] = sred[0];
+                h[1] = sred[1];
+                stat_halve<1, 1>(h, lr);
+                const int e_ = ((lr >> 3) & 1) * 4 + ((lr >> 2) & 1) * 2 + ((lr >> 1) & 1);
+                float* sl = reinterpret_cast<float*>(smem + STAT_OFF) + (((biasSlot & 1) * NW + wave) * 2 + ((lr >> 4) & 1)) * 64;
+                sl[i * 32 + 16 * (lr & 1) + 8 * lh + e_] = h[0];
+            }
+        }
+    };
+    auto stat_flush = [&](int slot_, int co0, int par) {
+        if (tid < 128) {
+            const int which = tid >> 6, c = tid & 63;
+            const float* sl = reinterpret_cast<const float*>(smem + STAT_OFF) + ((par & 1) * NW * 2 + which) * 64 + c;
+            float t = 0.f;
+#pragma unroll
+            for (int w_ = 0; w_ < NW; ++w_) t += sl[w_ * 128];
+            if (co0 + c < a.Cout) a.stat[((long)slot_ * 2 + which) * a.Cout + co0 + c] = t;
         }
     };
     auto epilogue_plain_as = [&](const DmaTile& tl, int biasSlot, auto actTag) {
@@ -1151,6 +1212,7 @@
     int remCompute = remIssue;
     bool more = true;
     int stage = 0;
+    int statSlot = -1, statCo0 = 0, statPar = 0;
     issue(nxt, wk, 0);
     walk_next(nxt.t, wk);
     --remIssue;
@@ -1158,6 +1220,12 @@
     __syncthreads();
     zero_acc();
     while (true) {
+        if constexpr (STATS) {
+            if (statSlot >= 0) {
+                stat_flush(statSlot, statCo0, statPar);
+                statSlot = -1;
+            }
+        }
         if (more && remIssue == 0) {
             ++iNxt;
             more = tile_at(iNxt, nxt);
@@ -1178,6 +1246,11 @@
         bool storesInFlight = false;
         if (--remCompute == 0) {
             epilogue(cur, iCur);
+            if constexpr (STATS) {
+                statSlot = (cur.t * tilesH + cur.h0 / TH) * tilesW + cur.w0 / 32;
+                statCo0 = cur.co0;
+                statPar = iCur;
+            }
             storesInFlight = RPW >= 2 ? !a.res1 : cur.co0 + 64 <= a.Cout && !res0any;
             ++iCur;
             if (!tile_at(iCur, cur)) break;
@@ -1192,15 +1265,19 @@
         __syncthreads();
         stage ^= 1;
     }
-}
-
-template <int NW, int RPW, int NSTAGE>
+    if constexpr (STATS) {
+        __syncthreads();
+        stat_flush(statSlot, statCo0, statPar);
+    }
+}
+
+template <int NW, int RPW, int NSTAGE, bool STATS>
 __global__ __launch_bounds__(64 * NW, (NW + 3) / 4) void conv3x3_dma_kernel(ConvArgs a, int nTiles, int tilesPerXcd) {
     prefetch_kernargs<sizeof(ConvArgs) + 8>();
-    conv3x3_dma_body<NW, RPW, NSTAGE>(a, nTiles, tilesPerXcd);
-}
-
-template <int NW, int RPW, int NSTAGE>
+    conv3x3_dma_body<NW, RPW, NSTAGE, STATS>(a, nTiles, tilesPerXcd);
+}
+
+template <int NW, int RPW, int NSTAGE, bool STATS = false>
 int launch_dma(const ConvArgs& a0, hipStream_t s) {
     constexpr int TH = NW * RPW;
     ConvArgs a = a0;
@@ -1212,13 +1289,13 @@
     if (grid < 8) grid = 8;
     const int tilesPerXcd = (nTiles + 7) / 8;
     constexpr int HALO_INSTR = ((TH + 2) * 34 + 15) / 16;
-    const size_t lds = NSTAGE * (size_t)(HALO_INSTR + 36) * 1024 + NW * 1024 + 512;
+    const size_t lds = NSTAGE * (size_t)(HALO_INSTR + 36) * 1024 + (STATS ? 1024 + 2 * NW * 512 : NW * 1024) + 512;
     static LdsAttrOnce attr;
     {
-        const hipError_t e = flair_max_lds_once(attr, reinterpret_cast<const void*>(&conv3x3_dma_kernel<NW, RPW, NSTAGE>));
+        const hipError_t e = flair_max_lds_once(attr, reinterpret_cast<const void*>(&conv3x3_dma_kernel<NW, RPW, NSTAGE, STATS>));
         FLAIR_CHECK(e == hipSuccess, "flair_conv_nhwc: hipFuncSetAttribute: %s", hipGetErrorString(e));
     }
-    hipLaunchKernelGGL((conv3x3_dma_kernel<NW, RPW, NSTAGE>), dim3(grid), dim3(64 * NW), lds, s, a, nTiles, tilesPerXcd);
+    hipLaunchKernelGGL((conv3x3_dma_kernel<NW, RPW, NSTAGE, STATS>), dim3(grid), dim3(64 * NW), lds, s, a, nTiles, tilesPerXcd);
 
     FLAIR_LAUNCH_CHECK();
     return FLAIR_OK;
@@ -1756,7 +1833,7 @@
         case 4: return launch_halo<E, 4, 1, 1>(a, s);
         case 6: return launch_halo_ks<E, 8, 1, 2>(a, s);
         case 7: return launch_halo_ks<E, 4, 1, 2>(a, s);
-        case 8: return launch_dma<8, 2, 2>(a, s);
+        case 8: return a.stat ? launch_dma<8, 2, 2, true>(a, s) : launch_dma<8, 2, 2>(a, s);
         case 9:
             if (frame_kernel_ok(a)) return launch_frame(a, s);
             return launch_dma<8, 1, 2>(a, s);
@@ -1792,9 +1869,20 @@
     return split > 1 ? (size_t)split * a.P * a.Cout * sizeof(float) : 0;
 }
 
-extern "C" int flair_conv_nhwc(const flair_conv_params* p, const void* const* x, const void* w,
-                               const float* bias, const float* frame_bias, const void* res0, const void* res1,
-                               void* y, void* workspace, size_t workspace_bytes, hipStream_t stream) {
+static int stats_slots_per_frame(const ConvArgs& a) {
+    return choose_variant(a) == 8 ? (a.H / 16) * (a.W / 32) : 0;
+}
+
+extern "C" int flair_conv_stats_slots(const flair_conv_params* p) {
+    if (!p) return 0;
+    ConvArgs a{};
+    fill_geometry(a, p);
+    return stats_slots_per_frame(a);
+}
+
+static int conv_entry(const flair_conv_params* p, const void* const* x, const void* w,
+                      const float* bias, const float* frame_bias, const void* res0, const void* res1,
+                      void* y, void* workspace, size_t workspace_bytes, float* stats, size_t stats_bytes, hipStream_t stream) {
     FLAIR_CHECK(p && x && w && y, "flair_conv_nhwc: null argument");
     FLAIR_CHECK(p->dtype == FLAIR_F32 || p->dtype == FLAIR_BF16, "flair_conv_nhwc: bad dtype %d", p->dtype);
     FLAIR_CHECK(p->nseg >= 1 && p->nseg <= 4, "flair_conv_nhwc: nseg %d not in 1..4", p->nseg);
@@ -1882,8 +1970,31 @@
         FLAIR_CHECK(((uintptr_t)workspace) % 16 == 0, "flair_conv_nhwc: workspace alignment");
         a.part = reinterpret_cast<float*>(workspace);
     }
+    if (stats) {
+        const int spf = stats_slots_per_frame(a);
+        FLAIR_CHECK(spf > 0, "flair_conv_nhwc_stats: this geometry's kernel has no statistics epilogue (flair_conv_stats_slots() == 0)");
+        const size_t need = (size_t)a.T * spf * 2 * a.Cout * sizeof(float);
+        FLAIR_CHECK(((uintptr_t)stats) % 16 == 0 && stats_bytes >= need,
+                    "flair_conv_nhwc_stats: statistics buffer (%zu bytes given, %zu needed: T * slots * 2 * Cout f32; 16-byte aligned)",
+                    stats_bytes, need);
+        a.stat = stats;
+    }
     if (p->dtype == FLAIR_BF16) return dispatch<bf16_t>(a, stream);
     return dispatch<float>(a, stream);
+}
+
+extern "C" int flair_conv_nhwc(const flair_conv_params* p, const void* const* x, const void* w,
+                               const float* bias, const float* frame_bias, const void* res0, const void* res1,
+                               void* y, void* workspace, size_t workspace_bytes, hipStream_t stream) {
+    return conv_entry(p, x, w, bias, frame_bias, res0, res1, y, workspace, workspace_bytes, nullptr, 0, stream);
+}
+
+extern "C" int flair_conv_nhwc_stats(const flair_conv_params* p, const void* const* x, const void* w,
+                                     const float* bias, const float* frame_bias, const void* res0, const void* res1,
+                                     void* y, void* workspace, size_t workspace_bytes, float* stats, size_t stats_bytes,
+                                     hipStream_t stream) {
+    FLAIR_CHECK(stats, "flair_conv_nhwc_stats: null statistics buffer");
+    return conv_entry(p, x, w, bias, frame_bias, res0, res1, y, workspace, workspace_bytes, stats, stats_bytes, stream);
 }
 
 extern "C" int flair_conv_variant(const flair_conv_params* p) {
diff --git a/flair_amd/csrc/gn.hip b/flair_amd/csrc/gn.hip
--- a/flair_amd/csrc/gn.hip
+++ b/flair_amd/csrc/gn.hip
@@ -12,7 +12,7 @@
 };
 
 template <typename E>
-__global__ void gn_partial_kernel(GnSrc s, int C, int groups, long pixPerStat, int blocksPerStat, float* part) {
+__global__ void gn_partial_kernel(GnSrc s, int C, int groups, long pixPerStat, int blocksPerStat, float* part, int perChannel) {
     prefetch_kernargs<sizeof(GnSrc) + 32>();
     constexpr int VEC = ET<E>::VEC;
     extern __shared__ float red[];
@@ -65,6 +65,13 @@
         }
         rs[c] = a;
         rq[c] = b;
+    }
+    if (perChannel) {
+        for (int c = threadIdx.x; c < C; c += blockDim.x) {
+            part[((long)blockIdx.x * 2 + 0) * C + c] = rs[c];
+            part[((long)blockIdx.x * 2 + 1) * C + c] = rq[c];
+        }
+        return;
     }
     __syncthreads();
     const int cpg = C / groups;
@@ -112,6 +119,60 @@
         if (var < 0) var = 0;
         stats[sg * 2 + 0] = (float)mean;
         stats[sg * 2 + 1] = (float)(1.0 / sqrt(var + (double)eps));
+    }
+}
+
+struct GnChParts {
+    const float* part[2];
+    int rowsPerStat[2];
+    int c[2];
+};
+
+__global__ __launch_bounds__(512) void gn_finalize_ch_kernel(GnChParts q, int groups, int cpg, long pixPerStat, float eps,
+                                                             float* stats) {
+    __shared__ double redA[8], redB[8];
+    const int stat = blockIdx.x / groups, g = blockIdx.x % groups;
+    double a = 0.0, b = 0.0;
+    for (int k = 0; k < cpg; ++k) {
+        const int c = g * cpg + k;
+        const int sgm = c >= q.c[0] ? 1 : 0;
+        const int cl = sgm ? c - q.c[0] : c;
+        const int rows = q.rowsPerStat[sgm], ld = q.c[sgm];
+        const float* pp = q.part[sgm] + (long)stat * rows * 2 * ld + cl;
+        int i = threadIdx.x;
+        for (; i + 512 < rows; i += 1024) {
+            const float a0 = pp[(long)i * 2 * ld], b0 = pp[(long)i * 2 * ld + ld];
+            const float a1 = pp[(long)(i + 512) * 2 * ld], b1 = pp[(long)(i + 512) * 2 * ld + ld];
+            a += (double)a0 + (double)a1;
+            b += (double)b0 + (double)b1;
+        }
+        for (; i < rows; i += 512) {
+            a += (double)pp[(long)i * 2 * ld];
+            b += (double)pp[(long)i * 2 * ld + ld];
+        }
+    }
+#pragma unroll
+    for (int off = 32; off > 0; off >>= 1) {
+        a += __shfl_xor(a, off);
+        b += __shfl_xor(b, off);
+    }
+    if ((threadIdx.x & 63) == 0) {
+        redA[threadIdx.x >> 6] = a;
+        redB[threadIdx.x >> 6] = b;
+    }
+    __syncthreads();
+    if (threadIdx.x == 0) {
+        double ta = 0.0, tb = 0.0;
+        for (int w = 0; w < 8; ++w) {
+            ta += redA[w];
+            tb += redB[w];
+        }
+        const double cnt = (double)pixPerStat * cpg;
+        const double mean = ta / cnt;
+        double var = tb / cnt - mean * mean;
+        if (var < 0) var = 0;
+        stats[blockIdx.x * 2 + 0] = (float)mean;
+        stats[blockIdx.x * 2 + 1] = (float)(1.0 / sqrt(var + (double)eps));
     }
 }
 
@@ -453,9 +514,20 @@
     return ((size_t)nstat * bps * 2 * p->groups + (size_t)nstat * p->groups * 2) * sizeof(float);
 }
 
-extern "C" int flair_groupnorm_nhwc(const flair_gn_params* p, const void* x0, const void* x1,
-                                    const float* gamma, const float* beta, const float* film,
-                                    void* y, void* raw, void* workspace, hipStream_t stream) {
+extern "C" size_t flair_groupnorm_stats_workspace_bytes(const flair_gn_params* p, const flair_gn_stats* st) {
+    if (!p) return 0;
+    if (!st || (!st->part[0] && !st->part[1])) return flair_groupnorm_workspace_bytes(p);
+    const int nstat = p->F / p->frames_per_stat;
+    const int bps = gn_blocks_per_stat(p);
+    size_t rows = 0;
+    if (!st->part[0]) rows += (size_t)nstat * bps * 2 * p->c0;
+    if (p->c0 < p->C && !st->part[1]) rows += (size_t)nstat * bps * 2 * (p->C - p->c0);
+    return (rows + (size_t)nstat * p->groups * 2) * sizeof(float);
+}
+
+static int gn_entry(const flair_gn_params* p, const void* x0, const void* x1,
+                    const float* gamma, const float* beta, const float* film,
+                    void* y, void* raw, void* workspace, const flair_gn_stats* st, hipStream_t stream) {
     FLAIR_CHECK(p && x0 && gamma && beta && y && workspace, "flair_groupnorm_nhwc: null argument");
     FLAIR_CHECK(p->dtype == FLAIR_F32 || p->dtype == FLAIR_BF16, "flair_groupnorm_nhwc: bad dtype");
     const int vec = p->dtype == FLAIR_BF16 ? 8 : 4;
@@ -519,20 +591,58 @@
             return FLAIR_OK;
         }
     }
-    const size_t lds = (size_t)2 * rows * C * sizeof(float);
-    if (p->dtype == FLAIR_BF16)
-        hipLaunchKernelGGL(gn_partial_kernel<bf16_t>, dim3(nstat * bps), dim3(threads), lds, stream, s, C, p->groups, pix, bps,
-                           part);
-    else
-        hipLaunchKernelGGL(gn_partial_kernel<float>, dim3(nstat * bps), dim3(threads), lds, stream, s, C, p->groups, pix, bps,
-                           part);
-    FLAIR_LAUNCH_CHECK();
     const int sg = nstat * p->groups;
-    FLAIR_CHECK(sg % 4 == 0 || sg < 4, "flair_groupnorm_nhwc: groups");
-    const int wavesPerBlock = sg >= 4 ? 4 : sg;
-    hipLaunchKernelGGL(gn_finalize_kernel, dim3(sg / wavesPerBlock), dim3(64 * wavesPerBlock), 0, stream,
-                       part, p->groups, C / p->groups, bps, pix, p->eps, stats);
-    FLAIR_LAUNCH_CHECK();
+    if (st && (st->part[0] || st->part[1])) {
+        GnChParts q;
+        float* wsp = reinterpret_cast<float*>(workspace);
+        stats = wsp;
+        wsp += (size_t)sg * 2;
+        for (int i = 0; i < 2; ++i) {
+            const int cs = s.c[i];
+            q.part[i] = nullptr; q.rowsPerStat[i] = 0; q.c[i] = cs;
+            if (cs == 0) continue;
+            if (st->part[i]) {
+                const size_t need = (size_t)p->F * st->slots_per_frame[i] * 2 * cs * sizeof(float);
+                FLAIR_CHECK(st->slots_per_frame[i] > 0 && ((uintptr_t)st->part[i]) % 16 == 0 && st->bytes[i] >= need,
+                            "flair_groupnorm_nhwc_stats: partials of segment %d (%zu bytes given, %zu needed: F * slots_per_frame * 2 * "
+                            "channels f32; 16-byte aligned)", i, st->bytes[i], need);
+                q.part[i] = st->part[i];
+                q.rowsPerStat[i] = p->frames_per_stat * st->slots_per_frame[i];
+                continue;
+            }
+            GnSrc s1;
+            s1.x[0] = s.x[i]; s1.x[1] = nullptr;
+            s1.c[0] = cs; s1.c[1] = 0;
+            s1.ld[0] = s.ld[i]; s1.ld[1] = 0;
+            const int cv1 = cs / vec;
+            const int rows1 = cv1 <= 256 ? 256 / cv1 : 1;
+            const size_t lds1 = (size_t)2 * rows1 * cs * sizeof(float);
+            if (p->dtype == FLAIR_BF16)
+                hipLaunchKernelGGL(gn_partial_kernel<bf16_t>, dim3(nstat * bps), dim3(rows1 * cv1), lds1, stream, s1, cs, 1, pix, bps, wsp, 1);
+            else
+                hipLaunchKernelGGL(gn_partial_kernel<float>, dim3(nstat * bps), dim3(rows1 * cv1), lds1, stream, s1, cs, 1, pix, bps, wsp, 1);
+            FLAIR_LAUNCH_CHECK();
+            q.part[i] = wsp;
+            q.rowsPerStat[i] = bps;
+            wsp += (size_t)nstat * bps * 2 * cs;
+        }
+        hipLaunchKernelGGL(gn_finalize_ch_kernel, dim3(sg), dim3(512), 0, stream, q, p->groups, C / p->groups, pix, p->eps, stats);
+        FLAIR_LAUNCH_CHECK();
+    } else {
+        const size_t lds = (size_t)2 * rows * C * sizeof(float);
+        if (p->dtype == FLAIR_BF16)
+            hipLaunchKernelGGL(gn_partial_kernel<bf16_t>, dim3(nstat * bps), dim3(threads), lds, stream, s, C, p->groups, pix, bps,
+                               part, 0);
+        else
+            hipLaunchKernelGGL(gn_partial_kernel<float>, dim3(nstat * bps), dim3(threads), lds, stream, s, C, p->groups, pix, bps,
+                               part, 0);
+        FLAIR_LAUNCH_CHECK();
+        FLAIR_CHECK(sg % 4 == 0 || sg < 4, "flair_groupnorm_nhwc: groups");
+        const int wavesPerBlock = sg >= 4 ? 4 : sg;
+        hipLaunchKernelGGL(gn_finalize_kernel, dim3(sg / wavesPerBlock), dim3(64 * wavesPerBlock), 0, stream,
+                           part, p->groups, C / p->groups, bps, pix, p->eps, stats);
+        FLAIR_LAUNCH_CHECK();
+    }
 
     GnApply a;
     a.s = s;
@@ -557,3 +667,16 @@
     FLAIR_LAUNCH_CHECK();
     return FLAIR_OK;
 }
+
+extern "C" int flair_groupnorm_nhwc(const flair_gn_params* p, const void* x0, const void* x1,
+                                    const float* gamma, const float* beta, const float* film,
+                                    void* y, void* raw, void* workspace, hipStream_t stream) {
+    return gn_entry(p, x0, x1, gamma, beta, film, y, raw, workspace, nullptr, stream);
+}
+
+extern "C" int flair_groupnorm_nhwc_stats(const flair_gn_params* p, const void* x0, const void* x1,
+                                          const float* gamma, const float* beta, const float* film,
+                                          void* y, void* raw, void* workspace, const flair_gn_stats* st, hipStream_t stream) {
+    FLAIR_CHECK(st, "flair_groupnorm_nhwc_stats: null statistics descriptor");
+    return gn_entry(p, x0, x1, gamma, beta, film, y, raw, workspace, st, stream);
+}
diff --git a/flair_amd/guided_diffusion/unet_new.py b/flair_amd/guided_diffusion/unet_new.py
--- a/flair_amd/guided_diffusion/unet_new.py
+++ b/flair_amd/guided_diffusion/unet_new.py
@@ -39,6 +39,19 @@
         self.flows = {}
         self.vsrpp_weights = None
         self.enable_cross_frames = True
+        self.gn_stats_reuse = False
+
+
+def _conv_s(ctx, *args, **kw):
+    if not ctx.gn_stats_reuse:
+        return ops.conv(*args, **kw)
+    y, st = ops.conv(*args, want_stats=True, **kw)
+    y.gn_stats = st
+    return y
+
+
+def _stats_of(ctx, t):
+    return getattr(t, "gn_stats", None) if (ctx.gn_stats_reuse and t is not None) else None
 
 
 def _pack(w, segs, dtype, device, cout_pad=None):
@@ -97,17 +110,18 @@
         if self.up or self.down:
             assert x1 is None
             h, x = ops.group_norm(x, pk["g1"], pk["be1"], eps=eps, act=A.ACT_SILU,
-                                  resample=2 if self.up else 1, want_raw=True)
+                                  resample=2 if self.up else 1, want_raw=True, stats=_stats_of(ctx, x))
         else:
-            h = ops.group_norm(x, pk["g1"], pk["be1"], x1=x1, eps=eps, act=A.ACT_SILU)
-        h = ops.conv(h, pk["w1"], pk["b1"], co, k)
-        h = ops.group_norm(h, pk["g2"], pk["be2"], eps=eps, act=A.ACT_SILU, film=film)
+            h = ops.group_norm(x, pk["g1"], pk["be1"], x1=x1, eps=eps, act=A.ACT_SILU,
+                               stats=_stats_of(ctx, x), stats1=_stats_of(ctx, x1))
+        h = _conv_s(ctx, h, pk["w1"], pk["b1"], co, k)
+        h = ops.group_norm(h, pk["g2"], pk["be2"], eps=eps, act=A.ACT_SILU, film=film, stats=_stats_of(ctx, h))
         if "ws" in pk:
             skip = ops.conv([x] if x1 is None else [x, x1], pk["ws"], pk["bs"], co, (1, 1, 1))
         else:
             assert x1 is None
             skip = x
-        return ops.conv(h, pk["w2"], pk["b2"], co, k, res0=skip)
+        return _conv_s(ctx, h, pk["w2"], pk["b2"], co, k, res0=skip)
 
 
 QKV_ATTN_WIDTHS = (32, 64, 128)
@@ -175,12 +189,12 @@
 
     def run(self, ctx, x):
         pk, c = self._pk, self.channels
-        n = ops.group_norm(x, pk["g"], pk["be"], eps=self.norm.wrapped_module.eps)
+        n = ops.group_norm(x, pk["g"], pk["be"], eps=self.norm.wrapped_module.eps, stats=_stats_of(ctx, x))
         qkv = ops.conv(n, pk["wqkv"], pk["bqkv"], 3 * c, (1, 1, 1))
         a = ops.qkv_attention(qkv, self.num_heads, new_order=self.new_order)
         if self.bottleneck:
             ops.add_frame_bias(a, ctx.film_all[:, self.film_off:self.film_off + c])
-        return ops.conv(a, pk["wp"], pk["bp"], c, (1, 1, 1), res0=x)
+        return _conv_s(ctx, a, pk["wp"], pk["bp"], c, (1, 1, 1), res0=x)
 
 
 class AttentionbottleBlock(AttentionBlock):
@@ -238,11 +252,11 @@
 
     def run(self, ctx, h):
         pk, c = self._pk, self.channels
-        n = ops.group_norm(h, pk["g"], pk["be"], eps=self.norm.wrapped_module.eps)
+        n = ops.group_norm(h, pk["g"], pk["be"], eps=self.norm.wrapped_module.eps, stats=_stats_of(ctx, h))
         qkv = ops.conv(n, pk["wqkv"], pk["bqkv"], 3 * c, (1, 1, 1))
         a = ops.temporal_attention(qkv, pk["kpos"], self.num_frames,
                                    round_fp16=(ctx.dtype == torch.float32), head_dim=self.head_dim)
-        return ops.conv(a, pk["wp"], pk["bp"], c, (1, 1, 1), res0=h)
+        return _conv_s(ctx, a, pk["wp"], pk["bp"], c, (1, 1, 1), res0=h)
 
 
 class ResidualBlockNoBN(nn.Module):
@@ -425,7 +439,7 @@
         ff = flows_forward if flows_forward is not None else flows_backward.flip(0)
         self._propagate(ctx, hidden, ff, "forward_1", [bwd], weight, wmaps, fwd)
         rec = run_trunk(self._pk["recon"], [hidden, bwd, fwd], c)
-        return ops.conv(rec, self._pk["wl"], self._pk["bl"], c, (1, 1, 1), res0=hidden)
+        return _conv_s(ctx, rec, self._pk["wl"], self._pk["bl"], c, (1, 1, 1), res0=hidden)
 
 
 class _ConvModule(nn.Module):
@@ -515,7 +529,7 @@
             elif isinstance(inner, (AttentionBlock, TemporalAttention, BasicVSRPP)):
                 h = inner.run(ctx, h)
             elif isinstance(inner, nn.Conv2d):
-                h = ops.conv(h, inner._pk_w, inner._pk_b, inner.out_channels, (1, 3, 3))
+                h = _conv_s(ctx, h, inner._pk_w, inner._pk_b, inner.out_channels, (1, 3, 3))
             elif isinstance(inner, nn.Identity):
                 pass
             else:
@@ -741,7 +755,8 @@
         return outs[0] if B == 1 else torch.cat(outs, dim=0)
 
     def _forward_clip_graphed(self, x, t, low_res, rnn, enable_cross_frames, vsrpp_weights, clip=0):
-        key = (tuple(x.shape), self.dtype, bool(enable_cross_frames), vsrpp_weights, x.device, clip)
+        key = (tuple(x.shape), self.dtype, bool(enable_cross_frames), vsrpp_weights, x.device, clip,
+               bool(getattr(self, "gn_stats_reuse", True)))
         ent = self._graphs.get(key)
         src = (rnn.data_ptr(), rnn._version, low_res.data_ptr(), low_res._version, getattr(self, "_flow_gen", 0))
         if ent is not None and ent["src"] != src:
@@ -775,6 +790,7 @@
         dev, dt = x.device, self.dtype
         ctx = Ctx(dt, dev, T)
         ctx.enable_cross_frames = enable_cross_frames
+        ctx.gn_stats_reuse = bool(getattr(self, "gn_stats_reuse", True))
         ctx.vsrpp_weights = vsrpp_weights
         ctx.flows = flows if flows is not None else self._flows_for(rnn)
         temb = ops.timestep_embedding(t.float().contiguous(), self.model_channels)
@@ -799,6 +815,7 @@
             h = blk.run(ctx, h, hs.pop())
             if trace is not None:
                 trace.append((f"output_blocks.{i}", h))
-        h = ops.group_norm(h, self._head_g, self._head_be, eps=self.out[0].wrapped_module.eps, act=A.ACT_SILU)
+        h = ops.group_norm(h, self._head_g, self._head_be, eps=self.out[0].wrapped_module.eps, act=A.ACT_SILU,
+                           stats=_stats_of(ctx, h))
         y = ops.conv(h, self._head_w, self._head_b, self._head_w.shape[0], (1, 3, 3))
         return ops.clip_to_nchw(y, self.out_channels)
diff --git a/flair_amd/ops.py b/flair_amd/ops.py
--- a/flair_amd/ops.py
+++ b/flair_amd/ops.py
@@ -19,6 +19,10 @@
                 ("frames_per_stat", ctypes.c_int), ("eps", ctypes.c_float), ("act", ctypes.c_int),
                 ("resample", ctypes.c_int), ("y_ld", ctypes.c_int), ("raw_ld", ctypes.c_int),
                 ("film_ld", ctypes.c_int)]
+
+
+class GnStats(ctypes.Structure):
+    _fields_ = [("part", ctypes.c_void_p * 2), ("slots_per_frame", ctypes.c_int * 2), ("bytes", ctypes.c_size_t * 2)]
 
 
 class SamplerCoefs(ctypes.Structure):
@@ -77,7 +81,8 @@
 
 
 def conv(xs, weight, bias, cout, kernel, *, out=None, act=ACT_NONE, res0=None, res1=None,
-         out_scale=1.0, stride=1, frame_bias=None, act_param=0.0, act_period=0, asym_pad=False, reflect_pad=False):
+         out_scale=1.0, stride=1, frame_bias=None, act_param=0.0, act_period=0, asym_pad=False, reflect_pad=False,
+         want_stats=False):
     if isinstance(xs, torch.Tensor):
         xs = [xs]
     x0 = xs[0]
@@ -114,10 +119,20 @@
     e0 = _prof_begin()
     wsb = _conv_ws_bytes(p)
     ws = _workspace(wsb, x0.device, "conv") if wsb else None
+    stats = None
+    if want_stats:
+        slots = lib().flair_conv_stats_slots(ctypes.byref(p))
+        if slots > 0:
+            stats = torch.empty((T, slots, 2, cout), dtype=torch.float32, device=x0.device)
 
     def launch(_keep=xs):
-        check(lib().flair_conv_nhwc(ctypes.byref(p), arr, ptr(weight), ptr(_f32(bias)), ptr(frame_bias), ptr(res0),
-                                    ptr(res1), ptr(out), ptr(ws), ctypes.c_size_t(wsb), stream()), "flair_conv_nhwc")
+        if stats is None:
+            check(lib().flair_conv_nhwc(ctypes.byref(p), arr, ptr(weight), ptr(_f32(bias)), ptr(frame_bias), ptr(res0),
+                                        ptr(res1), ptr(out), ptr(ws), ctypes.c_size_t(wsb), stream()), "flair_conv_nhwc")
+        else:
+            check(lib().flair_conv_nhwc_stats(ctypes.byref(p), arr, ptr(weight), ptr(_f32(bias)), ptr(frame_bias), ptr(res0),
+                                              ptr(res1), ptr(out), ptr(ws), ctypes.c_size_t(wsb), ptr(stats),
+                                              ctypes.c_size_t(stats.numel() * 4), stream()), "flair_conv_nhwc_stats")
     launch()
     if e0 is not None:
         cin = sum(x.shape[3] for x in xs)
@@ -128,8 +143,8 @@
                         + cout * taps * cin)
         _prof_end(e0, ("conv", lib().flair_conv_variant(ctypes.byref(p))), x0.dtype, flops, nbytes, launch,
                   ("conv", T, H, W, tuple(x.shape[3] for x in xs), cout, tuple(kernel), stride, act,
-                   res0 is not None, res1 is not None, frame_bias is not None))
-    return out
+                   res0 is not None, res1 is not None, frame_bias is not None, stats is not None))
+    return (out, stats) if want_stats else out
 
 
 PROFILE = None
@@ -264,7 +279,7 @@
 
 
 def group_norm(x, gamma, beta, *, x1=None, groups=32, eps=1e-5, act=ACT_NONE, film=None,
-               frames_per_stat=None, resample=0, out=None, want_raw=False):
+               frames_per_stat=None, resample=0, out=None, want_raw=False, stats=None, stats1=None):
     T, H, W, c0 = x.shape
     C = c0 + (x1.shape[3] if x1 is not None else 0)
     p = GnParams()
@@ -287,19 +302,40 @@
     p.film_ld = film.stride(0) if film is not None else 0
     if film is not None:
         assert film.dtype == torch.float32 and film.stride(1) == 1 and film.shape[0] == T
-    ws = _workspace(lib_ws_bytes(p), x.device)
+    st = None
+    if stats is not None or (stats1 is not None and x1 is not None):
+        st = GnStats()
+        for i, (seg, part) in enumerate(((x, stats), (x1, stats1))):
+            if seg is None or part is None:
+                continue
+            assert part.dtype == torch.float32 and part.is_contiguous() and part.dim() == 4 and part.shape[0] == T \
+                and part.shape[2] == 2 and part.shape[3] == seg.shape[3], "stats: the (T, slots, 2, C) partials of this segment"
+            st.part[i] = part.data_ptr()
+            st.slots_per_frame[i] = part.shape[1]
+            st.bytes[i] = part.numel() * 4
+        f = lib().flair_groupnorm_stats_workspace_bytes
+        f.restype = ctypes.c_size_t
+        ws = _workspace(f(ctypes.byref(p), ctypes.byref(st)), x.device)
+    else:
+        ws = _workspace(lib_ws_bytes(p), x.device)
     e0 = _prof_begin()
 
-    def launch():
-        check(lib().flair_groupnorm_nhwc(ctypes.byref(p), ptr(x), ptr(x1), ptr(_f32(gamma)), ptr(_f32(beta)),
-                                         ptr(film), ptr(out), ptr(raw), ptr(ws), stream()),
-              "flair_groupnorm_nhwc")
+    def launch(_keep=(stats, stats1)):
+        if st is None:
+            check(lib().flair_groupnorm_nhwc(ctypes.byref(p), ptr(x), ptr(x1), ptr(_f32(gamma)), ptr(_f32(beta)),
+                                             ptr(film), ptr(out), ptr(raw), ptr(ws), stream()),
+                  "flair_groupnorm_nhwc")
+        else:
+            check(lib().flair_groupnorm_nhwc_stats(ctypes.byref(p), ptr(x), ptr(x1), ptr(_f32(gamma)), ptr(_f32(beta)),
+                                                   ptr(film), ptr(out), ptr(raw), ptr(ws), ctypes.byref(st), stream()),
+                  "flair_groupnorm_nhwc_stats")
     launch()
     if e0 is not None:
         numel_in, numel_out = T * H * W * C, T * Ho * Wo * C
         _prof_end(e0, ("gn",), x.dtype, 8.0 * numel_in,
                   x.element_size() * (2 * numel_in + numel_out * (2 if want_raw else 1)), launch,
-                  ("gn", T, H, W, C, c0, groups, p.frames_per_stat, act, resample, want_raw, film is not None))
+                  ("gn", T, H, W, C, c0, groups, p.frames_per_stat, act, resample, want_raw, film is not None,
+                   st is not None and bool(st.part[0]), st is not None and bool(st.part[1])))
     return (out, raw) if want_raw else out
 
 
diff --git a/include/flair_hip.h b/include/flair_hip.h
--- a/include/flair_hip.h
+++ b/include/flair_hip.h
@@ -59,6 +59,12 @@
                     void* y, void* workspace, size_t workspace_bytes, hipStream_t stream);
 int flair_conv_variant(const flair_conv_params* p);
 
+int flair_conv_stats_slots(const flair_conv_params* p);
+int flair_conv_nhwc_stats(const flair_conv_params* p, const void* const* x, const void* w,
+                          const float* bias, const float* frame_bias, const void* res0, const void* res1,
+                          void* y, void* workspace, size_t workspace_bytes, float* stats, size_t stats_bytes,
+                          hipStream_t stream);
+
 
 typedef struct {
     int dtype;
@@ -99,6 +105,17 @@
 int flair_groupnorm_nhwc(const flair_gn_params* p, const void* x0, const void* x1,
                          const float* gamma, const float* beta, const float* film, void* y,
                          void* raw, void* workspace, hipStream_t stream);
+
+typedef struct {
+    const float* part[2];
+    int slots_per_frame[2];
+    size_t bytes[2];
+} flair_gn_stats;
+
+size_t flair_groupnorm_stats_workspace_bytes(const flair_gn_params* p, const flair_gn_stats* st);
+int flair_groupnorm_nhwc_stats(const flair_gn_params* p, const void* x0, const void* x1,
+                               const float* gamma, const float* beta, const float* film, void* y,
+                               void* raw, void* workspace, const flair_gn_stats* st, hipStream_t stream);
 
 int flair_nchw_f32_to_nhwc(const float* src, int N, int C, int H, int W, void* dst, int dtype,
                            int dst_ld, int dst_coff, hipStream_t stream);
```
